# wvangansbeke/LaneDetection_End2End

Hardware: AMD Instinct MI355X
Metric: images/sec fwd+bwd, 256x512 2-lane bs32 (higher is better)
Workload: dtype f32; 1 GPU; BEV ERFNet + fused WLS fit + Area loss, 2 lanes, 256x512, batch 32 per GPU, fp32, train mode (BN batch stats, Dropout2d on), fwd+bwd, optimizer excluded; global_batch=32, parallelism=dp1, grad_allreduce=none

## Files before the change

lanedetection_end2end_amd/_lib.py:

```python
import ctypes
import os
from ctypes import c_char_p, c_double, c_int, c_long, c_size_t, c_void_p

import torch

_HERE = os.path.dirname(os.path.abspath(__file__))
LIB_PATH = os.path.join(_HERE, "liblanefit_hip.so")
_lib = None


class LaneFitLibraryError(RuntimeError):
    pass


def _declare(lib):
    P, I, L, D = c_void_p, c_int, c_long, c_double
    sig = {
        "lf_abi_version": (c_int, []),
        "lf_last_error": (c_char_p, []),
        "lf_wls_workspace_bytes": (c_size_t, [I, I, I]),
        "lf_wls_fwd": (I, [P, P, L, I, I, I, I, I, I, D, D, I, I, P, P, P, P, P, P]),
        "lf_wls_bwd": (I, [P, P, L, I, I, I, I, I, I, D, I, P, P, P, P, P]),
        "lf_gels_workspace_bytes": (c_size_t, [I, I]),
        "lf_gels_fwd": (I, [P, P, I, L, I, P, P, P, P, P]),
# ... 51 lines not shown
        "lf_adam_step": (I, [P, P, I, ctypes.c_float, ctypes.c_float, ctypes.c_float, ctypes.c_float, ctypes.c_float,
                             I, ctypes.c_float, P]),
        "lf_sgd_step": (I, [P, P, I, ctypes.c_float, ctypes.c_float, ctypes.c_float, ctypes.c_float, P]),
        "lf_rmsprop_step": (I, [P, P, I, ctypes.c_float, ctypes.c_float, ctypes.c_float, ctypes.c_float, ctypes.c_float,
                                ctypes.c_float, P]),
        "lf_conv1d_scratch_floats": (L, [I, I, I, I]),
        "lf_conv1d_fwd": (I, [P, P, P, P, I, I, I, I, I, I, I, P, P]),
        "lf_conv1d_bwd_data": (I, [P, P, P, P, I, I, I, I, I, I, P, P]),
        "lf_conv1d_bwd_weight": (I, [P, P, P, P, I, I, I, I, I, I, P, P]),
        "lf_erfnet_num_layers": (I, [P]),
        "lf_erfnet_range_workspace_bytes": (c_size_t, [P, I, I]),
        "lf_erfnet_layer_io": (I, [P, I, P]),
        "lf_erfnet_forward_range": (I, [P, I, I, I, P, P, P, P, P, I, P, P, c_size_t, P]),
        "lf_erfnet_backward_range": (I, [P, I, I, I, P, P, P, P, P, I, P, P, c_size_t, P]),
        "lf_linear_fwd": (I, [P, P, P, P, I, I, I, I, P]),
        "lf_linear_bwd": (I, [P, P, P, P, P, P, P, I, I, I, I, P]),
        "lf_seg_maps": (I, [P, P, P, I, I, I, I, I, I, P]),
        "lf_erfnet_set_precision": (I, [P, I]),
        "lf_erfnet_profile": (I, [P, I]),
        "lf_erfnet_profile_read": (I, [P, P, c_char_p]),
        "lf_erfnet_infer_workspace_bytes": (c_size_t, [P, I]),
        "lf_erfnet_infer_encoder_offset": (L, [P]),
        "lf_erfnet_infer": (I, [P, P, P, P, P, I, P, P, c_size_t, P]),
        "lf_erfnet_infer_range_workspace_bytes": (c_size_t, [P, I, I, I]),
        "lf_erfnet_infer_range": (I, [P, I, I, I, P, P, P, P, P, P, c_size_t, P]),
        "lf_convchain_infer_workspace_bytes": (c_size_t, [P, I]),
        "lf_convchain_infer": (I, [P, P, P, P, P, ctypes.c_float, P, P, c_size_t, P]),
        "lf_head_fit": (I, [P, I, P, P, P, L, I, I, I, I, I, I, D, D, I, I, P, P, P, P, P, P]),
        "lf_lane_infer_workspace_bytes": (c_size_t, [P, I, I, I]),
        "lf_lane_infer": (I, [P, P, P, P, P, P, L, I, I, D, D, I, I, P, P, P, P, c_size_t, P]),
        "lf_theta_grid": (I, [P, L, P, P, I, I, I, P, P]),
        "lf_theta_grid_bwd_workspace_bytes": (c_size_t, [I]),
        "lf_theta_grid_bwd": (I, [P, L, P, P, P, I, I, I, P, P, P]),
        "lf_wls_fwd_theta": (I, [P, P, L, P, P, I, I, I, I, I, I, D, D, I, I, P, P, P, P, P, P]),
        "lf_wls_bwd_theta_workspace_bytes": (c_size_t, [I, I]),
        "lf_wls_bwd_theta": (I, [P, P, L, P, P, I, I, I, I, I, I, D, I, P, P, P, P, P, P, P]),
        "lf_wls_bwd_grid": (I, [P, P, L, I, I, I, I, I, I, D, I, P, P, P, P, P]),
        "lf_lane_eval": (I, [P, P, P, P, P, P, L, P, I, I, I, I, I, D, D, P, P, P, P, P, P]),
        "lf_lane_decode_bev": (I, [P, I, P, P, P, P, L, P, P, I, D, P, P, I, I, I, I, I, I, I, I, I, I, P, P, P]),
        "lf_step_loss_workspace_bytes": (c_size_t, []),
        "lf_step_loss": (I, [I, I, I, I, I, I, I, P, L, I, P, P, L, I, P, P, P, P, P, P, P, I, D, D, P, P, P, P, P, P]),
        "lf_step_loss_bwd": (I, [P, I, L, L, P, P, P]),
        "lf_seg_step_workspace_bytes": (c_size_t, [I, I, I, I, I, I]),
        "lf_seg_step": (I, [P, P, P, P, L, P, I, I, I, I, I, I, I, D, D, I, P, P, P, P, P, P, P, P]),
        "lf_seg_step_bwd": (I, [P, L, P, P]),
        "lf_label_batch_bp": (I, [P, P, P, P, P, P, P, L, P, P, I, I, P, P, P, P, P, P, P, P, P]),
        "lf_label_batch_bev": (I, [P, P, P, P, P, L, P, P, I, P, P, P, P, P, P, P]),
        "lf_grad_norm_workspace_bytes": (c_size_t, [I]),
        "lf_grad_sumsq": (I, [P, P, I, I, P, P]),
        "lf_grad_norm_finish": (I, [P, I, ctypes.c_float, ctypes.c_float, P, P]),
        "lf_grad_scale_inplace": (I, [P, P, I, ctypes.c_float, P, P]),
        "lf_adam_step_clipped": (I, [P, P, I, ctypes.c_float, ctypes.c_float, ctypes.c_float, ctypes.c_float, ctypes.c_float,
                                     I, ctypes.c_float, P, P]),
        "lf_sgd_step_clipped": (I, [P, P, I, ctypes.c_float, ctypes.c_float, ctypes.c_float, ctypes.c_float, P, P]),
        "lf_rmsprop_step_clipped": (I, [P, P, I, ctypes.c_float, ctypes.c_float, ctypes.c_float, ctypes.c_float, ctypes.c_float,
                                        ctypes.c_float, P, P]),
        "lf_head_fit_seg": (I, [P, I, P, P, P, L, P, I, I, I, I, I, I, I, D, D, I, P, P, P, P, P, P]),
        "lf_lane_infer_seg_workspace_bytes": (c_size_t, [P, I, I, I]),
        "lf_lane_infer_seg": (I, [P, P, P, P, P, P, L, P, I, I, I, D, D, I, P, P, P, P, c_size_t, P]),
        "lf_stem_bwd_data": (I, [P, P, P, I, I, I, I, I, P, P]),
        "lf_erfnet_backward_input": (I, [P, P, P, P, P, P, P, I, I, P, P, c_size_t, P]),
        "lf_erfnet_infer_fold": (I, [P, P, P, P, P, c_size_t, P]),
        "lf_lane_infer_folded": (I, [P, P, P, P, P, P, L, I, I, D, D, I, I, P, P, P, P, c_size_t, I, P]),
        "lf_lane_infer_seg_folded": (I, [P, P, P, P, P, P, L, P, I, I, I, D, D, I, P, P, P, P, c_size_t, I, P]),
    }
    dbg = {
        "lf_debug_set_split_any_size": (None, [I]),
        "lf_debug_set_bf16_lds": (None, [I]),
        "lf_debug_set_bf16_no_partial_fast": (None, [I]),
        "lf_debug_stride2_epi": (I, [I, I, P, P, P, P, I, P, P, P, P, I, I, I, I, I, P, P]),
        "lf_debug_stride2_wgrad_scratch_floats": (L, [I, I, I, I, I, I, I]),
        "lf_debug_stride2_wgrad": (I, [I, I, P, P, P, P, I, I, I, I, I, P, P]),
        "lf_debug_stem_wgrad_scratch_floats": (L, [I, I, I, I]),
        "lf_debug_stem_wgrad": (I, [I, P, P, P, P, I, I, I, I, P, P]),
        "lf_debug_head_wgrad_scratch_floats": (L, [I, I, I, I]),
        "lf_debug_head_wgrad": (I, [I, P, P, P, P, I, I, I, I, P, P]),
        "lf_debug_set_ops_precision": (None, [I]),
        "lf_debug_conv1d_fwd_phases": (I, [P, P, P, P, I, I, I, I, I, I, P, P, P]),
        "lf_debug_conv1d_wgrad_phases": (I, [P, P, I, I, I, I, I, I, P, P, P]),
        "lf_debug_conv1d_fwd_pro": (I, [P, P, P, P, P, P, I, I, I, I, I, I, P, P]),
        "lf_debug_set_wgrad_ro": (None, [I, I, I]),
        "lf_debug_set_fp32_stream": (None, [I, I]),
        "lf_debug_set_bwd16_fused": (None, [I]),
        "lf_debug_set_fwd_pair": (None, [I, I]),
        "lf_debug_conv1d_fwd_pair": (I, [P, P, P, P, P, P, P, P, P, P, I, I, I, I, I, P, P]),
        "lf_debug_conv1d_bwd_pair_scratch_floats": (L, [I, I, I, I]),
        "lf_debug_conv1d_bwd_pair": (I, [P, P, P, I, P, P, P, P, P, P, P, P, P, P, I, I, I, I, I, I, P, P]),
        "lf_debug_conv1d_bwd_data_epi3": (I, [P, P, P, P, P, P, P, I, I, I, I, I, I, P, P]),
        "lf_debug_conv1d_epi": (I, [P, P, P, P, I, I, P, P, P, P, P, P, I, I, I, I, I, I, P, P]),
        "lf_debug_conv1d_wgrad_pro": (I, [P, P, P, P, P, P, I, I, I, I, I, I, P, P]),
        "lf_debug_bias_residual_launches": (L, []),
        "lf_debug_partial_fast_launches": (L, []),
        "lf_debug_bf16_ring_launches": (L, []),
        "lf_debug_set_bf16_max_workgroups": (None, [I]),
        "lf_debug_set_thin": (None, [I, I]),
        "lf_debug_thin_launches": (L, []),
        "lf_debug_fold_pack_launches": (L, []),
        "lf_debug_bn_finalize_fwd": (I, [P, I, I, I, I, I, I, L] * 2 + [I, D, P, P, P, P, ctypes.c_float, ctypes.c_float, I, P, P, P, P, P]),
        "lf_debug_bn_bwd_finalize": (I, [P, I, I, I, I, I, I, L] * 2 + [I, D, P, P, P, P, P, P, I, P]),
        "lf_debug_bn_act": (I, [P, P, P, P, P, P, L, I, L, I, P]),
        "lf_debug_bn_bwd_reduce": (I, [P, P, P, P, P, P, P, I, L, I, L, I, P]),
        "lf_debug_bn_bwd_apply": (I, [P, P, P, P, P, P, P, P, P, P, P, L, I, L, I, P]),
        "lf_debug_pool_concat_fwd": (I, [P, I, I, I, I, P, I, I, P, I, I, P]),
        "lf_debug_pool_affine_fwd": (I, [P, I, I, I, I, P, I, I, P, P, I, P]),
        "lf_debug_pool_bwd": (I, [P, P, I, I, I, I, I, I, P, I, P]),
        "lf_debug_stem_fwd": (I, [P, I, I, I, I, P, P, P, P, P, P, I, I, P]),
        "lf_debug_head_fwd": (I, [P, P, P, P, I, I, I, I, I, P]),
        "lf_debug_head_bwd_data": (I, [P, P, P, I, I, I, I, I, P]),
        "lf_debug_convchain_offset": (L, [P, I, I]),
    }
    for table in (sig, dbg):
        for name, (res, args) in table.items():
            fn = getattr(lib, name)
            fn.restype = res
            fn.argtypes = args
    return sig


def exported_symbols():
    return list(_declare(load()).keys()) + list(_extra_symbols)


_extra_symbols = ["lf_debug_set_thin", "lf_debug_thin_launches", "lf_debug_fold_pack_launches"]


def load():
    global _lib
    if _lib is None:
        if not os.path.exists(LIB_PATH):
            raise LaneFitLibraryError(
                "%s not found: build it with `python -m lanedetection_end2end_amd.build` "
                "(there is no fallback path)" % LIB_PATH)
        lib = ctypes.CDLL(LIB_PATH)
        _declare(lib)
        _lib = lib
    return _lib


def check(rc, what):
    if rc != 0:
        raise LaneFitLibraryError("%s failed: %s" % (what, load().lf_last_error().decode()))


def ptr(t, rows=False):
    if t is None:
        return None
    if not t.is_cuda:
        raise LaneFitLibraryError("lanefit ops need tensors on the MI355X (got a %s tensor); "
                                  "there is no CPU path" % t.device)
    if rows:
        assert t.dim() == 2 and t.stride(1) == 1, "internal: tensor rows must be contiguous"
    else:
        assert t.is_contiguous(), "internal: tensor must be contiguous"
    return c_void_p(t.data_ptr())


def stream():
    return c_void_p(torch.cuda.current_stream().cuda_stream)


class DeferredRead:

    def __init__(self, t):
        if t.is_cuda:
            self.host = torch.empty(t.shape, dtype=t.dtype, pin_memory=True)
            self.host.copy_(t, non_blocking=True)
            self.event = torch.cuda.Event()
            self.event.record()
        else:
            self.host = t.detach().clone()
            self.event = None

    def ready(self):
        return self.event is None or self.event.query()

    def get(self):
        if self.event is not None:
            self.event.synchronize()
        return self.host
```

lanedetection_end2end_amd/csrc/lf_bwd16.hip:

```cpp
#include "lf_conv_dev.h"
#include "lf_conv_epi.h"

namespace {

constexpr int B16_TILE = 1024;
template <int EPIC> struct B16Cfg {
    static constexpr bool ST_ADD = (EPIC & LF_EPI_ADD) != 0;
    static constexpr bool AUX_IS_X = (EPIC & LF_EPI_MASKBN) != 0;
    static constexpr bool ST_AUX = (EPIC & LF_EPI_STATS_XHAT) != 0 && !AUX_IS_X;
    static constexpr bool SUMS = (EPIC & LF_EPI_STATS_XHAT) != 0;
    static constexpr int T_ADD = 6, T_AUX = ST_AUX ? 6 + (ST_ADD ? 1 : 0) : 4;
    static constexpr int NTILE = 6 + (ST_ADD ? 1 : 0) + (ST_AUX ? 1 : 0);
    static constexpr int STAGES = NTILE == 6 ? 3 : 2;
    static constexpr int STAGE = NTILE * B16_TILE, WAVE_LDS = STAGES * STAGE;
    static_assert(WG_WAVES * WAVE_LDS + 1024 <= 80 * 1024, "two workgroups per CU");
    static_assert(WAVE_LDS >= 13 * 64 * 4, "the ring also stages the wave's weight-gradient sums");
};

typedef __attribute__((address_space(3))) float* lds_f32_p;
typedef __attribute__((address_space(3))) f32x4* lds_f32x4_p;
typedef __attribute__((address_space(3))) unsigned char* lds_u8_p;

template <bool PRO, int EPIC>
__global__ __launch_bounds__(256, 2) void tapbwd16_kernel(const LfTapGeom g, const LfWgradArgs wa, const LfTapArgs a, const long pps,
                                                          const int write_bias, const int wave_rows) {
    using Cfg = B16Cfg<EPIC>;
    constexpr int NTAPS = 3, NT = 1, epi = EPIC;
    constexpr bool S16 = false, HOISTV = true;
    const int lane = threadIdx.x & 63, wave = __builtin_amdgcn_readfirstlane((int)(threadIdx.x >> 6));
    const int pl = lane & 15, kq = lane >> 4;
    const long npix_l = (long)g.N * g.Hl * g.Wl;
    const unsigned npix = (unsigned)npix_l, bx = blockIdx.x;
    const int cob = 0;
    const long sub = (long)blockIdx.x * WG_WAVES + wave;
    const long p_begin = sub * pps;
    long p_end = p_begin + pps;
    if (p_end > npix_l) p_end = npix_l;
    const int niter = p_end > p_begin ? (int)((p_end - p_begin + 15) / 16) : 0;
    f32x4 acc[NTAPS];
#pragma unroll
    for (int t = 0; t < NTAPS; ++t) acc[t] = zero4();
    float bsum = 0.f;
    const unsigned tbytes = (unsigned)min((long)g.N * g.Hs * g.Ws * g.s_pix * 4, (long)LF_OOB);
    const i32x4s rx = make_rsrc_words(wa.x, tbytes), rg = make_rsrc_words(wa.g, tbytes),
                 radd = make_rsrc_words(a.add_src, Cfg::ST_ADD ? tbytes : 0u), raux = make_rsrc_words(a.aux, Cfg::ST_AUX ? tbytes : 0u);
    lds_u8_p const ring = (lds_u8_p)lf_tap_lds + wave * Cfg::WAVE_LDS;
    const unsigned lds0 = (unsigned)(size_t)ring;
    const int tdh0 = g.tdh[0], tdh1 = g.tdh[1], tdh2 = g.tdh[2], tdw0 = g.tdw[0], tdw1 = g.tdw[1], tdw2 = g.tdw[2];
    long p_ld = p_begin;
    int pj_, pi_, pn_;
    row1_coords(g, niter ? (unsigned)p_begin : 0u, pn_, pi_, pj_);
    int cj = pj_, ci = pi_, cn = pn_;
    const int px = lane >> 2, chunk = lane & 3;
    int slot_ld = 0;
    auto issue = [&]() __attribute__((always_inline)) {
        const bool ok = p_ld < p_end;
        const int j = pj_ + px;
        const unsigned dst = lds0 + (unsigned)(slot_ld * Cfg::STAGE);
#pragma unroll
        for (int t = 0; t < NTAPS; ++t) {
            const int dh = t == 0 ? tdh0 : t == 1 ? tdh1 : tdh2, dw = t == 0 ? tdw0 : t == 1 ? tdw1 : tdw2;
            const int sy = pi_ + dh, sx = j + dw;
            const bool in = ok && sy >= 0 && sy < g.Hs && sx >= 0 && sx < g.Ws;
            const unsigned o = in ? (unsigned)((((pn_ * g.Hs + sy) * g.Ws + sx) * g.s_pix + g.s_choff + chunk * 4) * 4) : LF_OOB;
            lds_dma16(rg, dst + (unsigned)(t * B16_TILE), o, 0u);
            lds_dma16(rx, dst + (unsigned)((3 + t) * B16_TILE), o, 0u);
        }
        if constexpr (Cfg::ST_ADD || Cfg::ST_AUX) {
            const unsigned o = ok ? (unsigned)((((pn_ * g.Hs + pi_) * g.Ws + j) * g.s_pix + g.s_choff + chunk * 4) * 4) : LF_OOB;
            if constexpr (Cfg::ST_ADD) lds_dma16(radd, dst + (unsigned)(Cfg::T_ADD * B16_TILE), o, 0u);
            if constexpr (Cfg::ST_AUX) lds_dma16(raux, dst + (unsigned)(Cfg::T_AUX * B16_TILE), o, 0u);
        }
        slot_ld = slot_ld == Cfg::STAGES - 1 ? 0 : slot_ld + 1;
        p_ld += 16;
        pj_ += 16;
        if (pj_ >= g.Wl) { pj_ = 0; if (++pi_ >= g.Hl) { pi_ = 0; ++pn_; } }
    };
    f32x4 w3[NTAPS];
    {
        const __amdgpu_buffer_rsrc_t rwl = make_rsrc(a.wp, (unsigned)(NTAPS * 16 * 16 * 4));
#pragma unroll
        for (int t = 0; t < NTAPS; ++t) w3[t] = ldb4(rwl, (unsigned)(kq * 16 + pl) * 16u, (unsigned)(t * 16 * 64));
    }
    float psc = 1.f, psh = 0.f;
    if constexpr (PRO) { psc = wa.pro_sc[pl]; psh = wa.pro_sh[pl]; }
#undef LF_EPI_ACC
#define LF_EPI_ACC(n, m) dacc
#undef LF_EPI_LDADD
#define LF_EPI_LDADD(o) (*(lds_f32x4_p)(epi_lane + Cfg::T_ADD * B16_TILE))
#undef LF_EPI_LDMSK
#define LF_EPI_LDMSK(o) (*(lds_f32x4_p)(epi_lane + 4 * B16_TILE))
#undef LF_EPI_LDAUX
#define LF_EPI_LDAUX(o) (*(lds_f32x4_p)(epi_lane + Cfg::T_AUX * B16_TILE))
#undef LF_EPI_HOIST_ALL
#define LF_EPI_HOIST_ALL true
#undef LF_EPI_ROW1
#define LF_EPI_ROW1 true
    LF_EPI_HEAD
    (void)r_add; (void)r_msk; (void)r_aux;
    if constexpr ((EPIC & LF_EPI_MASKBN) != 0) asm volatile("" ::"v"(hv[0][0]), "v"(hv[0][1]) : "memory");
    asm volatile("s_waitcnt vmcnt(0)" ::"v"(w3[0]), "v"(w3[1]), "v"(w3[2]), "v"(psc), "v"(psh) : "memory");
#pragma unroll
    for (int q = 0; q < Cfg::STAGES - 1; ++q) issue();
    int slot_c = 0;
    f32x4 row1 = zero4(), row2 = zero4();
    for (int it = 0; it < niter; ++it) {
        asm volatile("s_waitcnt lgkmcnt(0)" ::: "memory");
        issue();
        wait_vm_lgkm0<Cfg::NTILE * (Cfg::STAGES - 1)>();
        lds_u8_p const st = ring + slot_c * Cfg::STAGE;
        slot_c = slot_c == Cfg::STAGES - 1 ? 0 : slot_c + 1;
        lds_u8_p const epi_lane = st + pl * 64 + kq * 16;
        {
            lds_f32_p const frag = (lds_f32_p)(st + kq * 64 + pl * 4);
            float gv[4], xv[NTAPS][4];
#pragma unroll
            for (int u = 0; u < 4; ++u) {
                gv[u] = frag[(1 * B16_TILE + u * 256) / 4];
#pragma unroll
                for (int t = 0; t < NTAPS; ++t) xv[t][u] = frag[((3 + t) * B16_TILE + u * 256) / 4];
            }
            if constexpr (PRO) {
#pragma unroll
                for (int t = 0; t < NTAPS; ++t) {
                    const int dh = t == 0 ? tdh0 : t == 1 ? tdh1 : tdh2, dw = t == 0 ? tdw0 : t == 1 ? tdw1 : tdw2;
                    const bool rowok = (unsigned)(ci + dh) < (unsigned)g.Hs;
                    const int c0 = cj + dw;
                    const bool edge = c0 < 0 || c0 + 15 >= g.Ws;
#pragma unroll
                    for (int u = 0; u < 4; ++u) {
                        float v = fmaxf(xv[t][u] * psc + psh, 0.f);
                        if (edge) v = (unsigned)(c0 + 4 * u + kq) < (unsigned)g.Ws ? v : 0.f;
                        xv[t][u] = rowok ? v : 0.f;
                    }
                }
            }
#pragma unroll
            for (int u = 0; u < 4; ++u) {
#pragma unroll
                for (int t = 0; t < NTAPS; ++t) acc[t] = __builtin_amdgcn_mfma_f32_16x16x4f32(xv[t][u], gv[u], acc[t], 0, 0, 0);
                bsum += gv[u];
            }
        }
        f32x4 dacc;
#pragma unroll
        for (int t = 0; t < NTAPS; ++t) {
            const f32x4 x3 = *(lds_f32x4_p)(epi_lane + t * B16_TILE);
            f32x4 part;
#pragma unroll
            for (int s4 = 0; s4 < 4; ++s4) part = __builtin_amdgcn_mfma_f32_16x16x4f32(w3[t][s4], x3[s4], s4 ? part : zero4(), 0, 0, 0);
            dacc = t ? dacc + part : part;
        }
        {
            const int pn[1] = {cn}, pi[1] = {ci}, pj[1] = {cj + pl};
            const bool pv[1] = {true};
            LF_EPI_TILE(0)
        }
        if constexpr (Cfg::SUMS) {
            if (wave_rows && ((it & 3) == 3 || it == niter - 1)) {
                f32x4 q1, q2;
                q1.x = sum16(s1[0].x); q1.y = sum16(s1[0].y); q1.z = sum16(s1[0].z); q1.w = sum16(s1[0].w);
                q2.x = sum16(s2[0].x); q2.y = sum16(s2[0].y); q2.z = sum16(s2[0].z); q2.w = sum16(s2[0].w);
                const bool first = (it & 15) < 4;
                row1 = first ? q1 : row1 + q1;
                row2 = first ? q2 : row2 + q2;
                s1[0] = zero4(); s2[0] = zero4();
                if (((it & 15) == 15 || it == niter - 1) && pl == 0) {
                    const long row = (p_begin >> 8) + (it >> 4);
#pragma unroll
                    for (int e = 0; e < 4; ++e) {
                        a.stats[(long)(kq * 4 + e) * a.stats_ld + row] = row1[e];
                        a.stats[(long)(g.Cd + kq * 4 + e) * a.stats_ld + row] = row2[e];
                    }
                }
            }
        }
        cj += 16;
        if (cj >= g.Wl) { cj = 0; if (++ci >= g.Hl) { ci = 0; ++cn; } }
    }
    asm volatile("s_waitcnt vmcnt(0)" ::: "memory");
    if (!wave_rows) {
        const int pn[1] = {0};
        LF_EPI_TAIL
    }
#undef LF_EPI_ACC
#define LF_EPI_ACC(n, m) acc[n][m]
#undef LF_EPI_LDADD
#define LF_EPI_LDADD(o) epi_ld<S16>(r_add, o)
#undef LF_EPI_LDMSK
#define LF_EPI_LDMSK(o) epi_ld<S16>(r_msk, o)
#undef LF_EPI_LDAUX
#define LF_EPI_LDAUX(o) epi_ld<S16>(r_aux, o)
#undef LF_EPI_HOIST_ALL
#define LF_EPI_HOIST_ALL false
#undef LF_EPI_ROW1
#define LF_EPI_ROW1 false
    float* const red = reinterpret_cast<float*>(lf_tap_lds);
    constexpr int RW = Cfg::WAVE_LDS / 4;
    if (wave > 0) {
#pragma unroll
        for (int t = 0; t < NTAPS; ++t)
#pragma unroll
            for (int e = 0; e < 4; ++e) red[wave * RW + (t * 4 + e) * 64 + lane] = acc[t][e];
    }
    red[wave * RW + 12 * 64 + lane] = bsum;
    __syncthreads();
    if (wave == 0) {
#pragma unroll
        for (int t = 0; t < NTAPS; ++t) {
            float* out = wa.partial + ((long)blockIdx.x * NTAPS + t) * g.Cs * g.Cd;
#pragma unroll
            for (int e = 0; e < 4; ++e) {
                float v = acc[t][e];
#pragma unroll
                for (int w = 1; w < WG_WAVES; ++w) v += red[w * RW + (t * 4 + e) * 64 + lane];
                out[(long)(4 * kq + e) * g.Cd + pl] = v;
            }
        }
        if (write_bias && wa.bias_partial) {
            float v = red[12 * 64 + lane] + red[RW + 12 * 64 + lane] + red[2 * RW + 12 * 64 + lane] + red[3 * RW + 12 * 64 + lane];
            v += __shfl_xor(v, 16, 64);
            v += __shfl_xor(v, 32, 64);
            if (kq == 0) wa.bias_partial[(long)blockIdx.x * g.Cd + pl] = v;
        }
    }
}

std::atomic<int> g_bwd16_mode{1};
enum { B16_MASK = 1, B16_MASKBN = 2, B16_EPI3 = 4, B16_ADD = 8 };
constexpr int g_bwd16_routed = B16_MASK | B16_MASKBN | B16_EPI3 | B16_ADD;

int form_of(int pro, int epi) {
    if (pro == LF_PRO_NONE && epi == LF_EPI_MASK) return B16_MASK;
    if (pro == LF_PRO_BNRELU && epi == (LF_EPI_MASKBN | LF_EPI_STATS_XHAT)) return B16_MASKBN;
    if (pro == LF_PRO_NONE && epi == (LF_EPI_ADD | LF_EPI_MASK | LF_EPI_STATS_XHAT)) return B16_EPI3;
    if (pro == LF_PRO_NONE && epi == LF_EPI_ADD) return B16_ADD;
    return 0;
}
template <typename F>
auto with_form(int form, F&& f) {
    switch (form) {
        case B16_MASK: return f(tapbwd16_kernel<false, LF_EPI_MASK>, B16Cfg<LF_EPI_MASK>{});
        case B16_MASKBN: return f(tapbwd16_kernel<true, LF_EPI_MASKBN | LF_EPI_STATS_XHAT>, B16Cfg<LF_EPI_MASKBN | LF_EPI_STATS_XHAT>{});
        case B16_EPI3: return f(tapbwd16_kernel<false, LF_EPI_ADD | LF_EPI_MASK | LF_EPI_STATS_XHAT>, B16Cfg<LF_EPI_ADD | LF_EPI_MASK | LF_EPI_STATS_XHAT>{});
        default: return f(tapbwd16_kernel<false, LF_EPI_ADD>, B16Cfg<LF_EPI_ADD>{});
    }
}

}

void lf_tapbwd16_set(int mode) { g_bwd16_mode = mode < 0 ? 0 : mode; }
bool lf_tapbwd16_routed(int pro, int epi) {
    const int mode = g_bwd16_mode.load();
    const int forms = mode == 0 ? 0 : mode == 1 ? g_bwd16_routed : mode >> 1;
    return (forms & form_of(pro, epi)) != 0;
}

bool lf_tapbwd16_ok(const LfTapGeom& gf, const LfTapGeom& gd, const LfWgradArgs& w, const LfTapArgs& a, int pro, int epi) {
    const int form = form_of(pro, epi);
    if (!form) return false;
    const LfTapGeom& g = gf;
    bool same = gf.N == gd.N && gf.Hl == gd.Hl && gf.Wl == gd.Wl && gf.Hs == gd.Hs && gf.Ws == gd.Ws && gf.s_pix == gd.s_pix && gf.s_choff == gd.s_choff &&
                gf.ssh == gd.ssh && gf.ssw == gd.ssw && gf.Hd == gd.Hd && gf.Wd == gd.Wd && gf.d_pix == gd.d_pix && gf.d_choff == gd.d_choff &&
                gf.dsh == gd.dsh && gf.dsw == gd.dsw && gf.dah == gd.dah && gf.daw == gd.daw && gf.Cs == gd.Cs && gf.Cd == gd.Cd && gf.ntaps == gd.ntaps;
    for (int t = 0; same && t < 3 && t < gf.ntaps; ++t) same = gf.tdh[t] == gd.tdh[t] && gf.tdw[t] == gd.tdw[t];
    if (!same) return false;
    if (!(g.Cs == 16 && g.Cd == 16 && g.ntaps == 3 && g.ssh == 1 && g.ssw == 1 && g.dsh == 1 && g.dsw == 1 && g.dah == 0 && g.daw == 0 &&
          g.Hs == g.Hl && g.Hd == g.Hl && g.Ws == g.Wl && g.Wd == g.Wl && g.s_pix == 16 && g.d_pix == 16 && g.s_choff == 0 && g.d_choff == 0 &&
          g.tdh[1] == 0 && g.tdw[1] == 0))
        return false;
    if (g.N < 1 || g.Hl < 1 || g.Wl < 64 || g.Wl % 64 != 0) return false;
    const long npix = (long)g.N * g.Hl * g.Wl;
    if (npix * 64 >= (long)LF_OOB) return false;
    if (lf_tapgemm_bf16_lds() < 3) return false;
    if (w.s16 || a.s16 || a.wp16 || w.dbg || a.dbg || a.bias || a.dm) return false;
    if (!w.x || !w.g || !w.partial || !w.bias_partial || !a.wp || !a.dst || a.src != w.g) return false;
    if (a.dst == w.x || a.dst == w.g) return false;
    if ((pro == LF_PRO_BNRELU) != (w.pro_sc != nullptr) || (w.pro_sc != nullptr) != (w.pro_sh != nullptr)) return false;
    if ((epi & LF_EPI_MASK) && a.mask_src != w.x) return false;
    if ((epi & LF_EPI_MASKBN) && (a.aux != w.x || !a.msc || !a.msh)) return false;
    if ((epi & LF_EPI_ADD) && (!a.add_src || a.add_src == a.dst)) return false;
    if ((epi & LF_EPI_STATS_XHAT) && (!a.aux || a.aux == a.dst || !a.stats)) return false;
    if (epi & LF_EPI_STATS_XHAT) {
        const long pps = lf_tapwgrad_wave_pixels(g);
        if (!(pps % 256 == 0 || pps == 64 || (lf_tapwgrad_splits(g) == 1 && npix <= 256))) return false;
        if (a.stats_ld < lf_tapgemm_stat_rows(g)) return false;
    }
    return with_form(form, [&](auto kern, auto cfg) {
        return allow_big_lds(reinterpret_cast<const void*>(kern), 128 * 1024);
    });
}

int lf_tapbwd16_launch(const LfTapGeom& gf, const LfTapGeom& gd, const LfWgradArgs& w, const LfTapArgs& a, int pro, int epi, hipStream_t st) {
    LF_REQUIRE(lf_tapbwd16_ok(gf, gd, w, a, pro, epi), "tapbwd16: the fused kernel does not take this launch (pro %d, epi %d, %d x %d x %d x %d -> %d)",
               pro, epi, gf.N, gf.Hl, gf.Wl, gf.Cs, gf.Cd);
    const long pps = lf_tapwgrad_wave_pixels(gf);
    const int gx = lf_tapwgrad_splits(gf);
    const int wave_rows = pps % 256 == 0;
    with_form(form_of(pro, epi), [&](auto kern, auto cfg) {
        hipLaunchKernelGGL(kern, dim3(gx), dim3(256), (size_t)WG_WAVES * decltype(cfg)::WAVE_LDS, st, gf, w, a, pps, 1, wave_rows);
        return true;
    });
    LF_CHECK_LAUNCH("tapbwd16");
    return 0;
}
```

lanedetection_end2end_amd/csrc/lf_conv.h:

```cpp
#pragma once
#include <atomic>

#include "lf_common.h"

#define LF_MAX_TAPS 9
struct TapIdx { int v[LF_MAX_TAPS]; };

struct LfTapGeom {
    int N, Hl, Wl;
    int Hs, Ws, s_pix, s_choff;
    int ssh, ssw;
    int Hd, Wd, d_pix, d_choff;
    int dsh, dsw, dah, daw;
    int Cs, Cd;
    int ntaps;
    int tdh[LF_MAX_TAPS], tdw[LF_MAX_TAPS];
};

enum { LF_PRO_NONE = 0, LF_PRO_BNRELU = 1 };
enum {
    LF_EPI_RELU = 1,
    LF_EPI_MASK = 2,
    LF_EPI_ADD = 4,
    LF_EPI_STATS_SQ = 8,
    LF_EPI_MASKBN = 16,
    LF_EPI_STATS_XHAT = 32,
    LF_EPI_BIAS = 64
};

struct LfTapArgs {
    const float* src;
    const float* wp;
    int s16;
    const void* wp16;
    int split;
    const void* wp48;
    const float* bias;
    float* dst;
    const float* pro_sc;
    const float* pro_sh;
    const float* mask_src;
    const float* add_src;
    const float* aux;
    const float* msc;
    const float* msh;
    const float* asc;
    const float* ash;
    const float* dm;
    float* stats;
    int stats_ld;
    unsigned long long* dbg;
    int thin;
};

void lf_tapgemm_set_split_any_size(int v);
void lf_tapgemm_set_fp32_stream(int mode, int max_workgroups);
void lf_tapgemm_set_thin(int mode, int nt);
long lf_tapgemm_thin_launches();
int lf_tapgemm_stat_rows(const LfTapGeom& g);
int lf_tapgemm_stat_rows_for(const LfTapGeom& g, const LfTapArgs& a);
int lf_tapgemm_launch(const LfTapGeom& g, const LfTapArgs& a, int pro, int epi, hipStream_t st);
int lf_tapgemm_launch_unordered(const LfTapGeom& g, const LfTapArgs& a, int pro, int epi, hipStream_t st);
bool lf_tapgemm_split_ok(const LfTapGeom& g);
long lf_tapgemm_bias_residual_launches();
extern std::atomic<long> g_bres_launches;

bool lf_tappair_ok(const LfTapGeom& ga, const LfTapGeom& gb, const LfTapArgs& aa, const LfTapArgs& ab, int pro, int epi_a, int epi_b);
int lf_tappair_launch(const LfTapGeom& ga, const LfTapGeom& gb, const LfTapArgs& aa, const LfTapArgs& ab, int pro, hipStream_t st);
void lf_tappair_set(int mode, int max_workgroups);
bool lf_tappair_routed(int C, int pro);

int lf_tapgemm_bf16_route(const LfTapGeom& g, const LfTapArgs& a, int pro, int epi, int epis, long npix, int nt, dim3 grid, hipStream_t st);
void lf_tapgemm_set_bf16_lds(int v);
int lf_tapgemm_bf16_lds();
void lf_tapgemm_set_bf16_no_partial_fast(int v);
long lf_tapgemm_partial_fast_launches();
long lf_tapgemm_bf16_ring_launches();
void lf_tapgemm_set_bf16_max_workgroups(int v);

struct LfWgradArgs {
    const float* x;
    const float* g;
    const float* pro_sc;
    const float* pro_sh;
    int s16;
    int split;
    float* partial;
    float* bias_partial;
    unsigned long long* dbg = nullptr;
};
int lf_tapwgrad_splits(const LfTapGeom& g);
int lf_tapwgrad_splits_bound(const LfTapGeom& g, int s16);
long lf_tapwgrad_wave_pixels(const LfTapGeom& g);
int lf_tapwgrad_splits_for(const LfTapGeom& g, const LfWgradArgs& a, int pro);
int lf_tapwgrad_launch(const LfTapGeom& g, const LfWgradArgs& a, int pro, hipStream_t st);

bool lf_tapbwd16_ok(const LfTapGeom& gf, const LfTapGeom& gd, const LfWgradArgs& w, const LfTapArgs& a, int pro, int epi);
int lf_tapbwd16_launch(const LfTapGeom& gf, const LfTapGeom& gd, const LfWgradArgs& w, const LfTapArgs& a, int pro, int epi, hipStream_t st);
void lf_tapbwd16_set(int mode);
bool lf_tapbwd16_routed(int pro, int epi);

bool lf_tapwgrad_ro_ok(const LfTapGeom& g, int s16);
int lf_tapwgrad_ro_rows_bound(const LfTapGeom& g);
int lf_tapwgrad_ro_rows(const LfTapGeom& g);
int lf_tapwgrad_ro_launch(const LfTapGeom& g, const LfWgradArgs& a, int pro, hipStream_t st);
void lf_tapwgrad_ro_set(int mode, int cap64, int cap128);

int lf_wgrad_reduce_launch(const float* partial, int splits, int ntaps, int Cs, int Cd, float* grad, long sk, long sn,
                           const int* tapidx_host, const float* bias_rows, int n_bias_rows, float* bias_grad,
                           int bias_accumulate, hipStream_t st);
#define LF_REDUCE_BATCH 32
struct LfReduceJob {
    const float* partial; float* grad; const float* bias_rows; float* bias_grad;
    long sk, sn;
    int splits, ntaps, Cs, Cd, n_bias_rows;
    int tapidx[LF_MAX_TAPS];
};
int lf_wgrad_reduce_batch_launch(const LfReduceJob* jobs_host, int njobs, hipStream_t st);
int lf_rows_reduce_launch(const float* rows, int nrows, int C, float* dst, int accumulate, hipStream_t st);

struct LfPackEntry {
    long src_off;
    long dst_off;
    int Kc, Nc, ntaps;
    long sk, sn;
    int tapidx[LF_MAX_TAPS];
    int param;
    long dst16_off;
};
int lf_pack_weights_launch(const LfPackEntry* entries_dev, int nentries, const float* const* params_dev, float* arena,
                           hipStream_t st);
long lf_pack_bf16_elems(int Kc, int Nc, int ntaps);
int lf_pack_weights_split_launch(const LfPackEntry* entries_dev, int nentries, const float* const* params_dev, void* arena48,
                                 hipStream_t st);

struct LfFoldEntry {
    LfPackEntry pk;
    int ch_off, C;
    const float* gamma;
    const float* beta;
    const float* mean;
    const float* var;
    const float* bias;
    long out_off;
};
int lf_fold_pack_launch(const LfFoldEntry* entries_dev, int nentries, const float* const* params_dev, float eps, float* vec, float* arena,
                        void* arena16, void* arena48, hipStream_t st);
long lf_fold_pack_launches();
int lf_pack_weights_bf16_launch(const LfPackEntry* entries_dev, int nentries, const float* const* params_dev, void* arena16,
                                hipStream_t st);
```

lanedetection_end2end_amd/csrc/lf_debug.h:

```cpp
#pragma once
#ifdef __cplusplus
extern "C" {
#endif
void lf_debug_set_split_any_size(int v);
void lf_debug_set_bf16_lds(int v);
void lf_debug_set_bf16_no_partial_fast(int v);
long lf_debug_partial_fast_launches(void);
long lf_debug_bf16_ring_launches(void);
void lf_debug_set_bf16_max_workgroups(int v);
void lf_debug_set_ops_precision(int mode);
int lf_debug_conv1d_fwd_phases(const float* x, const float* w, const float* bias, float* y, int N, int H, int W, int C,
                               int axis, int dilation, float* scratch, unsigned long long* dbg, void* stream);
int lf_debug_conv1d_fwd_pro(const float* x, const float* w, const float* bias, const float* sc, const float* sh, float* y, int N, int H,
                            int W, int C, int axis, int dilation, float* scratch, void* stream);
void lf_debug_set_wgrad_ro(int mode, int cap64, int cap128);
void lf_debug_set_fp32_stream(int mode, int max_workgroups);
void lf_debug_set_fwd_pair(int mode, int max_workgroups);
int lf_debug_conv1d_fwd_pair(const float* x, const float* wa, const float* ba, const float* wb, const float* bb, const float* sc,
                             const float* sh, float* t, float* y, float* stats, int N, int H, int W, int C, int dilation, float* scratch,
                             void* stream);
void lf_debug_set_bwd16_fused(int mode);
long lf_debug_conv1d_bwd_pair_scratch_floats(int N, int H, int W, int C);
int lf_debug_conv1d_bwd_pair(const float* x, const float* gy, const float* w, int epi, const float* add_src, const float* aux,
                             const float* msc, const float* msh, const float* pro_sc, const float* pro_sh, float* gx, float* gw, float* gb,
                             float* stats, int N, int H, int W, int C, int axis, int dilation, float* scratch, void* stream);
int lf_debug_conv1d_wgrad_pro(const float* x, const float* gy, const float* sc, const float* sh, float* gw, float* gb, int N, int H, int W,
                              int C, int axis, int dilation, float* scratch, void* stream);
int lf_debug_conv1d_bwd_data_epi3(const float* gy, const float* w, const float* mask_src, const float* add_src, const float* aux,
                                  float* gx, float* stats, int N, int H, int W, int C, int axis, int dilation, float* scratch, void* stream);
int lf_debug_conv1d_epi(const float* src, const float* w, const float* bias, float* dst, int transposed, int epi, const float* mask_src,
                        const float* add_src, const float* aux, const float* msc, const float* msh, float* stats, int N, int H, int W, int C,
                        int axis, int dilation, float* scratch, void* stream);
int lf_debug_stride2_epi(int kind, int phase, const float* src, const float* w, const float* bias, float* dst, int epi, const float* mask_src,
                         const float* add_src, const float* aux, float* stats, int N, int H, int W, int Cin, int Cout, float* scratch,
                         void* stream);
long lf_debug_stride2_wgrad_scratch_floats(int kind, int reduce, int N, int H, int W, int Cin, int Cout);
int lf_debug_stride2_wgrad(int kind, int reduce, const float* x, const float* g, float* gw, float* gb, int N, int H, int W, int Cin,
                           int Cout, float* scratch, void* stream);
long lf_debug_stem_wgrad_scratch_floats(int N, int Cin, int H, int W);
int lf_debug_stem_wgrad(int reduce, const float* img, const float* gcat, float* gw, float* gb, int N, int Cin, int H, int W, float* scratch,
                        void* stream);
long lf_debug_head_wgrad_scratch_floats(int N, int h, int w, int K);
int lf_debug_head_wgrad(int reduce, const float* x, const float* gout, float* gw, float* gb, int N, int h, int w, int K, float* scratch,
                        void* stream);
int lf_debug_bn_finalize_fwd(const float* rows0, int nrows0, int ld0, int C0, int ch_off0, int tile_pix0, int seg_rows0, long seg_pix0,
                             const float* rows1, int nrows1, int ld1, int C1, int ch_off1, int tile_pix1, int seg_rows1, long seg_pix1,
                             int C, double count, const float* gamma, const float* beta, float* running_mean, float* running_var,
                             float momentum, float eps, int training, float* scale, float* shift, float* asc, float* ash, void* stream);
int lf_debug_bn_bwd_finalize(const float* rows0, int nrows0, int ld0, int C0, int ch_off0, int tile_pix0, int seg_rows0, long seg_pix0,
                             const float* rows1, int nrows1, int ld1, int C1, int ch_off1, int tile_pix1, int seg_rows1, long seg_pix1,
                             int C, double count, const float* asc, const float* ash, float* c1, float* c2, float* ggamma, float* gbeta,
                             int training, void* stream);
int lf_debug_bn_act(const float* x, const float* sc, const float* sh, const float* dm, const float* res, float* y, long npix, int C,
                    long pix_per_image, int s16, void* stream);
int lf_debug_bn_bwd_reduce(const float* g, const float* y, const float* t, const float* asc, const float* ash, const float* dm, float* rows,
                           int ld, long npix, int C, long pix_per_image, int s16, void* stream);
int lf_debug_bn_bwd_apply(const float* g, const float* y, const float* t, const float* asc, const float* ash, const float* gamma,
                          const float* c1, const float* c2, const float* dm, float* g_t, float* g_z, long npix, int C, long pix_per_image,
                          int s16, void* stream);
int lf_debug_pool_concat_fwd(const float* x, int N, int H, int W, int Cin, float* cat, int cat_pix, int choff, float* rows, int ld, int s16,
                             void* stream);
int lf_debug_pool_affine_fwd(const float* x, int N, int H, int W, int Cin, float* cat, int cat_pix, int choff, const float* sc, const float* sh,
                             int s16, void* stream);
int lf_debug_pool_bwd(const float* x, const float* gcat, int N, int H, int W, int Cin, int cat_pix, int choff, float* gx, int s16, void* stream);
int lf_debug_stem_fwd(const float* img, int N, int Cin, int H, int W, const float* w, const float* b, const float* sc, const float* sh, float* cat,
                      float* rows, int ld, int s16, void* stream);
int lf_debug_head_fwd(const float* x, const float* w, const float* b, float* out, int N, int h, int w_, int K, int s16, void* stream);
int lf_debug_head_bwd_data(const float* gout, const float* w, float* gx, int N, int h, int w_, int K, int s16, void* stream);
long lf_debug_bias_residual_launches(void);
void lf_debug_set_thin(int mode, int nt);
long lf_debug_thin_launches(void);
long lf_debug_fold_pack_launches(void);
int lf_debug_conv1d_wgrad_phases(const float* x, const float* gy, int N, int H, int W, int C, int axis, int dilation,
                                 float* scratch, unsigned long long* dbg, void* stream);
struct lf_convchain_plan;
long lf_debug_convchain_offset(const struct lf_convchain_plan* plan, int block, int which);
#ifdef __cplusplus
}
#endif
```

lanedetection_end2end_amd/csrc/lf_eltwise.h:

```cpp
#pragma once
#include "lf_common.h"

struct LfStatPart {
    const float* rows; int nrows; int C; int ch_off; int ld;
    int tile_pix = 0; int seg_rows = 0; long seg_pix = 0;
};
inline int lf_stat_ld(int nrows) { return (nrows + 3) / 4 * 4; }
inline LfStatPart lf_stat_part_tiles(const float* rows, int nrows, int ld, int C, int ch_off, int seg_rows, long seg_pix, int tile_pix = 256) {
    LfStatPart p = {rows, nrows, C, ch_off, ld};
    p.tile_pix = tile_pix; p.seg_rows = seg_rows; p.seg_pix = seg_pix;
    return p;
}

int lf_bn_finalize_fwd(const LfStatPart* parts, int nparts, int C, double count, const float* gamma, const float* beta,
                       float* running_mean, float* running_var, float momentum, float eps, int training,
                       float* scale, float* shift, float* asc , float* ash , hipStream_t st);
int lf_bn_act(const float* x, const float* sc, const float* sh, const float* dm, const float* res, float* y,
              long npix, int C, long pix_per_image, int s16, hipStream_t st);
int lf_bn_bwd_reduce_rows(long npix);
int lf_bn_bwd_reduce(const float* g, const float* y, const float* t, const float* asc, const float* ash, const float* dm,
                     float* rows, int ld, long npix, int C, long pix_per_image, int s16, hipStream_t st);
int lf_bn_bwd_finalize(const LfStatPart* parts, int nparts, int C, double count, const float* asc, const float* ash, float* c1,
                       float* c2, float* ggamma, float* gbeta, int training, hipStream_t st);
int lf_bn_bwd_apply(const float* g, const float* y, const float* t, const float* asc, const float* ash, const float* gamma,
                    const float* c1, const float* c2, const float* dm, float* g_t, float* g_z, long npix, int C,
                    long pix_per_image, int s16, hipStream_t st);

int lf_pool_rows(long npix_out);
int lf_pool_concat_fwd(const float* x, int N, int H, int W, int Cin, float* cat, int cat_pix, int choff, float* rows, int ld,
                       int s16, hipStream_t st);
int lf_pool_affine_fwd(const float* x, int N, int H, int W, int Cin, float* cat, int cat_pix, int choff, const float* sc,
                       const float* sh, int s16, hipStream_t st);
int lf_pool_bwd(const float* x, const float* gcat, int N, int H, int W, int Cin, int cat_pix, int choff, float* gx,
                int s16, hipStream_t st);

int lf_stem_rows(int N, int H, int W);
int lf_stem_fwd(const float* img, int N, int Cin, int H, int W, const float* w, const float* b, float* cat, float* rows, int ld,
                int s16, hipStream_t st);
int lf_stem_fwd_infer(const float* img, int N, int Cin, int H, int W, const float* w, const float* b, const float* sc, const float* sh,
                      float* cat, int s16, hipStream_t st);
int lf_stem_wgrad_rows(int N, int H, int W);
int lf_stem_wgrad(const float* img, const float* gcat, int N, int Cin, int H, int W, float* wrows, float* brows,
                  int s16, hipStream_t st);

int lf_head_fwd(const float* x, const float* w, const float* b, float* out, int N, int h, int w_, int K, int s16,
                hipStream_t st);
int lf_head_bwd_data(const float* gout, const float* w, float* gx, int N, int h, int w_, int K, int s16, hipStream_t st);
int lf_head_wgrad_rows(int N, int h, int w_);
int lf_head_wgrad(const float* x, const float* gout, float* wrows, float* brows, int N, int h, int w_, int K,
                  int s16, hipStream_t st);
```

lanedetection_end2end_amd/csrc/lf_eltwise.hip:

```cpp
#include "lf_eltwise.h"
#include "lf_types.h"
#include "lf_plan.h"

typedef float f32x4 __attribute__((ext_vector_type(4)));

namespace {

__device__ __forceinline__ f32x4 ld4(const float* p) { return *reinterpret_cast<const f32x4*>(p); }
__device__ __forceinline__ void st4(float* p, f32x4 v) { *reinterpret_cast<f32x4*>(p) = v; }
__device__ __forceinline__ f32x4 z4() { f32x4 z = {0.f, 0.f, 0.f, 0.f}; return z; }
__device__ __forceinline__ f32x4 relu4(f32x4 v) {
    v.x = fmaxf(v.x, 0.f); v.y = fmaxf(v.y, 0.f); v.z = fmaxf(v.z, 0.f); v.w = fmaxf(v.w, 0.f); return v;
}
__device__ __forceinline__ f32x4 pos4(f32x4 v, f32x4 m) {
    v.x = m.x > 0.f ? v.x : 0.f; v.y = m.y > 0.f ? v.y : 0.f; v.z = m.z > 0.f ? v.z : 0.f; v.w = m.w > 0.f ? v.w : 0.f; return v;
}

template <int NQ>
__device__ __forceinline__ void block_reduce_quads(f32x4 (&a1)[NQ], f32x4 (&a2)[NQ], int U, float (*sm)[8 * NQ]) {
    const int tid = threadIdx.x;
#pragma unroll
    for (int q = 0; q < NQ; ++q) {
        sm[tid][8 * q + 0] = a1[q].x; sm[tid][8 * q + 1] = a1[q].y; sm[tid][8 * q + 2] = a1[q].z; sm[tid][8 * q + 3] = a1[q].w;
        sm[tid][8 * q + 4] = a2[q].x; sm[tid][8 * q + 5] = a2[q].y; sm[tid][8 * q + 6] = a2[q].z; sm[tid][8 * q + 7] = a2[q].w;
// ... 49 lines not shown
                    s1 += v ? av : 0.0;
                    s2 += v ? (double)b[u][e] + av * av * inv : 0.0;
                }
        }
    }
    constexpr int NWV = FIN_THREADS / 64;
    __shared__ double sm[NWV][2];
#pragma unroll
    for (int o = 32; o > 0; o >>= 1) { s1 += __shfl_xor(s1, o, 64); s2 += __shfl_xor(s2, o, 64); }
    const int w = threadIdx.x >> 6;
    if ((threadIdx.x & 63) == 0) { sm[w][0] = s1; sm[w][1] = s2; }
    __syncthreads();
    double t1 = 0.0, t2 = 0.0;
#pragma unroll
    for (int k = 0; k < NWV; ++k) { t1 += sm[k][0]; t2 += sm[k][1]; }
    s1 = t1; s2 = t2;
}

__global__ __launch_bounds__(FIN_THREADS) void bn_finalize_fwd_kernel(StatParts sp, int C, double count,
                                                            const float* __restrict__ gamma, const float* __restrict__ beta,
                                                            float* __restrict__ rmean, float* __restrict__ rvar,
                                                            float momentum, float eps, int training,
                                                            float* __restrict__ scale, float* __restrict__ shift,
                                                            float* __restrict__ asc, float* __restrict__ ash) {
    const int c = blockIdx.x;
    double s1 = 0.0, s2 = 0.0;
    if (training) stat_channel_sums(sp, c, s1, s2);
    if (threadIdx.x == 0 && c < C) {
        double mean, var;
        if (training) {
            mean = s1 / count;
            var = s2 / count - mean * mean;
            if (var < 0.0) var = 0.0;
            rmean[c] = (float)((1.0 - momentum) * (double)rmean[c] + momentum * mean);
            const double unb = count > 1.0 ? var * count / (count - 1.0) : var;
            rvar[c] = (float)((1.0 - momentum) * (double)rvar[c] + momentum * unb);
        } else {
            mean = (double)rmean[c];
            var = (double)rvar[c];
        }
        const double rstd = 1.0 / sqrt(var + (double)eps);
        const double sc = (double)gamma[c] * rstd;
        scale[c] = (float)sc;
        shift[c] = (float)((double)beta[c] - mean * sc);
        asc[c] = (float)rstd;
        ash[c] = (float)(-mean * rstd);
    }
}

template <typename T, int NQ>
__global__ __launch_bounds__(256) void bn_act_kernel(const T* __restrict__ x, const float* __restrict__ sc,
                                                    const float* __restrict__ sh, const float* __restrict__ dm,
                                                    const T* __restrict__ res, T* __restrict__ y, long units,
                                                    int U, long pix_per_image) {
    constexpr int V = 4 * NQ;
    const int C = U * V;
    for (long u = (long)blockIdx.x * 256 + threadIdx.x; u < units; u += (long)gridDim.x * 256) {
        const int c = (int)(u % U) * V;
        f32x4 v[NQ];
        lf_ldq<T, NQ>(x + u * V, v);
#pragma unroll
        for (int q = 0; q < NQ; ++q) v[q] = v[q] * ld4(sc + c + 4 * q) + ld4(sh + c + 4 * q);
        if (dm) {
            const float* d = dm + ((u / U) / pix_per_image) * C + c;
#pragma unroll
            for (int q = 0; q < NQ; ++q) v[q] *= ld4(d + 4 * q);
        }
        if (res) {
            f32x4 r[NQ];
            lf_ldq<T, NQ>(res + u * V, r);
#pragma unroll
            for (int q = 0; q < NQ; ++q) v[q] += r[q];
        }
#pragma unroll
        for (int q = 0; q < NQ; ++q) v[q] = relu4(v[q]);
        lf_stq<T, NQ>(y + u * V, v);
    }
}

template <typename T, int NQ>
__global__ __launch_bounds__(256) void bn_bwd_reduce_kernel(const T* __restrict__ g, const T* __restrict__ y,
                                                           const T* __restrict__ t, const float* __restrict__ asc,
                                                           const float* __restrict__ ash, const float* __restrict__ dm,
                                                           float* __restrict__ rows, int ld, long npix, int U, long pix_per_image) {
    constexpr int V = 4 * NQ;
    const int C = U * V, ppi = 256 / U;
    const int cq = threadIdx.x % U, pr = threadIdx.x / U;
    const int c = cq * V;
    (void)asc; (void)ash;
    f32x4 a1[NQ], a2[NQ];
#pragma unroll
    for (int q = 0; q < NQ; ++q) { a1[q] = z4(); a2[q] = z4(); }
    const long per_block = ((npix + gridDim.x - 1) / gridDim.x + ppi - 1) / ppi * ppi;
    const long p0 = (long)blockIdx.x * per_block;
    long p1 = p0 + per_block;
    if (p1 > npix) p1 = npix;
    for (long p = p0 + pr; p < p1; p += ppi) {
        const long off = p * C + c;
        f32x4 gm[NQ], tv[NQ];
        lf_ldq<T, NQ>(g + off, gm);
        lf_ldq<T, NQ>(t + off, tv);
        if (y) {
            f32x4 yv[NQ];
            lf_ldq<T, NQ>(y + off, yv);
#pragma unroll
            for (int q = 0; q < NQ; ++q) gm[q] = pos4(gm[q], yv[q]);
        }
        if (dm) {
            const float* d = dm + (p / pix_per_image) * C + c;
#pragma unroll
            for (int q = 0; q < NQ; ++q) gm[q] *= ld4(d + 4 * q);
        }
#pragma unroll
        for (int q = 0; q < NQ; ++q) {
            a1[q] += gm[q];
            a2[q] += gm[q] * tv[q];
        }
    }
    __shared__ float sm[256][8 * NQ];
    block_reduce_quads<NQ>(a1, a2, U, sm);
    if (threadIdx.x < U) {
#pragma unroll
        for (int q = 0; q < NQ; ++q)
#pragma unroll
            for (int e = 0; e < 4; ++e) {
                rows[(long)(c + 4 * q + e) * ld + blockIdx.x] = a1[q][e];
                rows[((long)C + c + 4 * q + e) * ld + blockIdx.x] = a2[q][e];
            }
    }
}

__global__ __launch_bounds__(FIN_THREADS) void bn_bwd_finalize_kernel(StatParts sp, int C, double mean_scale, const float* __restrict__ asc,
                                                            const float* __restrict__ ash, float* __restrict__ c1,
                                                            float* __restrict__ c2, float* __restrict__ ggamma,
                                                            float* __restrict__ gbeta) {
    const int c = blockIdx.x;
    double t1, t2;
    stat_channel_sums(sp, c, t1, t2);
    if (threadIdx.x == 0 && c < C) {
        const double rstd = (double)asc[c], mr = (double)ash[c];
        t2 = rstd * t2 + mr * t1;
        c1[c] = (float)(t1 * mean_scale);
        c2[c] = (float)(t2 * mean_scale);
        ggamma[c] = (float)t2;
        gbeta[c] = (float)t1;
    }
}

template <typename T, int NQ>
__global__ __launch_bounds__(256) void bn_bwd_apply_kernel(const T* __restrict__ g, const T* __restrict__ y,
                                                          const T* __restrict__ t, const float* __restrict__ asc,
                                                          const float* __restrict__ ash, const float* __restrict__ gamma,
                                                          const float* __restrict__ c1, const float* __restrict__ c2,
                                                          const float* __restrict__ dm, T* __restrict__ g_t,
                                                          T* __restrict__ g_z, long units, int U, long pix_per_image) {
    constexpr int V = 4 * NQ;
    const int C = U * V;
    for (long u = (long)blockIdx.x * 256 + threadIdx.x; u < units; u += (long)gridDim.x * 256) {
        const int c = (int)(u % U) * V;
        f32x4 gm[NQ], tv[NQ];
        lf_ldq<T, NQ>(g + u * V, gm);
        lf_ldq<T, NQ>(t + u * V, tv);
        if (y) {
            f32x4 yv[NQ];
            lf_ldq<T, NQ>(y + u * V, yv);
#pragma unroll
            for (int q = 0; q < NQ; ++q) gm[q] = pos4(gm[q], yv[q]);
        }
        if (g_z) lf_stq<T, NQ>(g_z + u * V, gm);
        if (dm) {
            const float* d = dm + ((u / U) / pix_per_image) * C + c;
#pragma unroll
            for (int q = 0; q < NQ; ++q) gm[q] *= ld4(d + 4 * q);
        }
        f32x4 o[NQ];
#pragma unroll
        for (int q = 0; q < NQ; ++q) {
            const f32x4 rstd = ld4(asc + c + 4 * q);
            const f32x4 xh = tv[q] * rstd + ld4(ash + c + 4 * q);
            o[q] = ld4(gamma + c + 4 * q) * rstd * (gm[q] - ld4(c1 + c + 4 * q) - xh * ld4(c2 + c + 4 * q));
        }
        lf_stq<T, NQ>(g_t + u * V, o);
    }
}

template <typename T, int NQ>
__global__ __launch_bounds__(256) void pool_concat_fwd_kernel(const T* __restrict__ x, int N, int H, int W, int U,
                                                             T* __restrict__ cat, int cat_pix, int choff,
                                                             float* __restrict__ rows, int ld) {
    constexpr int V = 4 * NQ;
// ... 141 lines not shown
                                                           T* __restrict__ gx, int N, int h, int wd, int K) {
    __shared__ float sw[16 * HEAD_MAXK * 4];
    for (int i = threadIdx.x; i < 16 * K * 4; i += 256) sw[i] = w[i];
    __syncthreads();
    const long npix = (long)N * h * wd;
    for (long p = (long)blockIdx.x * 256 + threadIdx.x; p < npix; p += (long)gridDim.x * 256) {
        const int j = (int)(p % wd);
        const long r = p / wd;
        const int i = (int)(r % h), n = (int)(r / h);
        float acc[16];
#pragma unroll
        for (int ci = 0; ci < 16; ++ci) acc[ci] = 0.f;
        for (int k = 0; k < K; ++k) {
            const float* gp = gout + (((long)n * K + k) * (2 * h) + 2 * i) * (2 * wd) + 2 * j;
            const float2 g0 = *reinterpret_cast<const float2*>(gp);
            const float2 g1 = *reinterpret_cast<const float2*>(gp + 2 * wd);
#pragma unroll
            for (int ci = 0; ci < 16; ++ci) {
                const float* wk = sw + (ci * K + k) * 4;
                acc[ci] = fmaf(g0.x, wk[0], fmaf(g0.y, wk[1], fmaf(g1.x, wk[2], fmaf(g1.y, wk[3], acc[ci]))));
            }
        }
#pragma unroll
        for (int q = 0; q < 4; ++q) {
            f32x4 v = {acc[q * 4], acc[q * 4 + 1], acc[q * 4 + 2], acc[q * 4 + 3]};
            lf_stv(gx + p * 16 + q * 4, v);
        }
    }
}

constexpr int LF_STREAM_BLOCKS = 16384;
inline int grid_for(long units, int cap) {
    long g = (units + 255) / 256;
    if (g > cap) g = cap;
    if (g < 1) g = 1;
    return (int)g;
}
inline bool quad_ok(int C) { return C % 4 == 0 && 256 % (C / 4) == 0; }
inline bool oct_ok(int s16, int C) { return s16 && C % 8 == 0 && 256 % (C / 8) == 0; }
template <typename T> inline const T* as(const float* p) { return reinterpret_cast<const T*>(p); }
template <typename T> inline T* as(float* p) { return reinterpret_cast<T*>(p); }
#define LF_BY_STORAGE(s16, CALL_BF16, CALL_F32) do { if (s16) { CALL_BF16; } else { CALL_F32; } } while (0)
#define LF_BY_STORAGE3(s16, oct, CALL_BF16X8, CALL_BF16, CALL_F32) do { if (oct) { CALL_BF16X8; } else if (s16) { CALL_BF16; } else { CALL_F32; } } while (0)

}

int lf_bn_finalize_fwd(const LfStatPart* parts, int nparts, int C, double count, const float* gamma, const float* beta,
                       float* running_mean, float* running_var, float momentum, float eps, int training, float* scale,
                       float* shift, float* asc, float* ash, hipStream_t st) {
    LF_REQUIRE(nparts >= 0 && nparts <= 2, "bn_finalize: at most 2 partial sources");
    StatParts sp;
    sp.n = nparts;
    for (int i = 0; i < nparts; ++i) sp.p[i] = parts[i];
    for (int i = 0; i < nparts; ++i) LF_REQUIRE(parts[i].C % 4 == 0 && parts[i].ch_off % 4 == 0, "bn_finalize: channel ranges must be multiples of 4");
    for (int i = 0; i < nparts; ++i)
        LF_REQUIRE(parts[i].tile_pix == 0 || (parts[i].seg_rows > 0 && parts[i].seg_pix > 0 && parts[i].nrows % parts[i].seg_rows == 0),
                   "bn_finalize: centred rows need the launch geometry (seg_rows, seg_pix)");
    for (int i = 0; i < nparts; ++i)
        LF_REQUIRE(parts[i].ld >= parts[i].nrows && parts[i].ld % 4 == 0 && ((size_t)parts[i].rows & 15) == 0,
                   "bn_finalize: channel-major rows need a 16-byte aligned base and a leading dimension >= nrows, multiple of 4 (ld=%d nrows=%d)", parts[i].ld, parts[i].nrows);
    hipLaunchKernelGGL(bn_finalize_fwd_kernel, dim3(C), dim3(FIN_THREADS), 0, st, sp, C, count, gamma, beta,
                       running_mean, running_var, momentum, eps, training, scale, shift, asc, ash);
    LF_CHECK_LAUNCH("bn_finalize_fwd");
    return 0;
}

int lf_bn_act(const float* x, const float* sc, const float* sh, const float* dm, const float* res, float* y, long npix,
              int C, long pix_per_image, int s16, hipStream_t st) {
    LF_REQUIRE(C % 4 == 0, "bn_act: C %% 4");
    const bool oct = oct_ok(s16, C);
    const int V = oct ? 8 : 4;
    const long units = npix * (C / V);
    const dim3 grid(grid_for(units, LF_STREAM_BLOCKS));
    LF_BY_STORAGE3(s16, oct,
        hipLaunchKernelGGL((bn_act_kernel<lf_bf16, 2>), grid, dim3(256), 0, st, as<lf_bf16>(x), sc, sh, dm, as<lf_bf16>(res), as<lf_bf16>(y), units, C / V, pix_per_image),
        hipLaunchKernelGGL((bn_act_kernel<lf_bf16, 1>), grid, dim3(256), 0, st, as<lf_bf16>(x), sc, sh, dm, as<lf_bf16>(res), as<lf_bf16>(y), units, C / V, pix_per_image),
        hipLaunchKernelGGL((bn_act_kernel<float, 1>), grid, dim3(256), 0, st, x, sc, sh, dm, res, y, units, C / V, pix_per_image));
    LF_CHECK_LAUNCH("bn_act");
    return 0;
}

int lf_bn_bwd_reduce_rows(long npix) { return grid_for(npix * 4, 1024); }

int lf_bn_bwd_reduce(const float* g, const float* y, const float* t, const float* asc, const float* ash, const float* dm,
                     float* rows, int ld, long npix, int C, long pix_per_image, int s16, hipStream_t st) {
    LF_REQUIRE(quad_ok(C), "bn_bwd_reduce: unsupported channel count %d", C);
    const dim3 grid(lf_bn_bwd_reduce_rows(npix));
    const bool oct = oct_ok(s16, C);
    const int V = oct ? 8 : 4;
    LF_BY_STORAGE3(s16, oct,
        hipLaunchKernelGGL((bn_bwd_reduce_kernel<lf_bf16, 2>), grid, dim3(256), 0, st, as<lf_bf16>(g), as<lf_bf16>(y), as<lf_bf16>(t), asc, ash, dm, rows, ld, npix, C / V, pix_per_image),
        hipLaunchKernelGGL((bn_bwd_reduce_kernel<lf_bf16, 1>), grid, dim3(256), 0, st, as<lf_bf16>(g), as<lf_bf16>(y), as<lf_bf16>(t), asc, ash, dm, rows, ld, npix, C / V, pix_per_image),
        hipLaunchKernelGGL((bn_bwd_reduce_kernel<float, 1>), grid, dim3(256), 0, st, g, y, t, asc, ash, dm, rows, ld, npix, C / V, pix_per_image));
    LF_CHECK_LAUNCH("bn_bwd_reduce");
    return 0;
}

int lf_bn_bwd_finalize(const LfStatPart* parts, int nparts, int C, double count, const float* asc, const float* ash, float* c1,
                       float* c2, float* ggamma, float* gbeta, int training, hipStream_t st) {
    LF_REQUIRE(nparts >= 1 && nparts <= 2, "bn_bwd_finalize: 1..2 partial sources");
    StatParts sp;
    sp.n = nparts;
    for (int i = 0; i < nparts; ++i) sp.p[i] = parts[i];
    for (int i = 0; i < nparts; ++i) LF_REQUIRE(parts[i].C % 4 == 0 && parts[i].ch_off % 4 == 0, "bn_bwd_finalize: channel ranges must be multiples of 4");
    for (int i = 0; i < nparts; ++i)
        LF_REQUIRE(parts[i].ld >= parts[i].nrows && parts[i].ld % 4 == 0 && ((size_t)parts[i].rows & 15) == 0,
                   "bn_bwd_finalize: channel-major rows need a 16-byte aligned base and a leading dimension >= nrows, multiple of 4 (ld=%d nrows=%d)", parts[i].ld, parts[i].nrows);
    hipLaunchKernelGGL(bn_bwd_finalize_kernel, dim3(C), dim3(FIN_THREADS), 0, st, sp, C, training ? 1.0 / count : 0.0, asc, ash,
                       c1, c2, ggamma, gbeta);
    LF_CHECK_LAUNCH("bn_bwd_finalize");
    return 0;
}

int lf_bn_bwd_apply(const float* g, const float* y, const float* t, const float* asc, const float* ash, const float* gamma,
                    const float* c1, const float* c2, const float* dm, float* g_t, float* g_z, long npix, int C,
                    long pix_per_image, int s16, hipStream_t st) {
    LF_REQUIRE(C % 4 == 0, "bn_bwd_apply: C %% 4");
    const bool oct = oct_ok(s16, C);
    const int V = oct ? 8 : 4;
    const long units = npix * (C / V);
    const dim3 grid(grid_for(units, LF_STREAM_BLOCKS));
    LF_BY_STORAGE3(s16, oct,
        hipLaunchKernelGGL((bn_bwd_apply_kernel<lf_bf16, 2>), grid, dim3(256), 0, st, as<lf_bf16>(g), as<lf_bf16>(y), as<lf_bf16>(t), asc, ash, gamma, c1, c2, dm, as<lf_bf16>(g_t), as<lf_bf16>(g_z), units, C / V, pix_per_image),
        hipLaunchKernelGGL((bn_bwd_apply_kernel<lf_bf16, 1>), grid, dim3(256), 0, st, as<lf_bf16>(g), as<lf_bf16>(y), as<lf_bf16>(t), asc, ash, gamma, c1, c2, dm, as<lf_bf16>(g_t), as<lf_bf16>(g_z), units, C / V, pix_per_image),
        hipLaunchKernelGGL((bn_bwd_apply_kernel<float, 1>), grid, dim3(256), 0, st, g, y, t, asc, ash, gamma, c1, c2, dm, g_t, g_z, units, C / V, pix_per_image));
    LF_CHECK_LAUNCH("bn_bwd_apply");
    return 0;
}

int lf_pool_rows(long npix_out) { return grid_for(npix_out * 4, 1024); }

int lf_pool_concat_fwd(const float* x, int N, int H, int W, int Cin, float* cat, int cat_pix, int choff, float* rows, int ld,
                       int s16, hipStream_t st) {
    LF_REQUIRE(quad_ok(Cin) && H % 2 == 0 && W % 2 == 0, "pool_concat: unsupported shape");
    const long npo = (long)N * (H / 2) * (W / 2);
    const dim3 grid(lf_pool_rows(npo));
    const bool oct = oct_ok(s16, Cin) && cat_pix % 8 == 0 && choff % 8 == 0;
    const int V = oct ? 8 : 4;
    LF_BY_STORAGE3(s16, oct,
        hipLaunchKernelGGL((pool_concat_fwd_kernel<lf_bf16, 2>), grid, dim3(256), 0, st, as<lf_bf16>(x), N, H, W, Cin / V, as<lf_bf16>(cat), cat_pix, choff, rows, ld),
        hipLaunchKernelGGL((pool_concat_fwd_kernel<lf_bf16, 1>), grid, dim3(256), 0, st, as<lf_bf16>(x), N, H, W, Cin / V, as<lf_bf16>(cat), cat_pix, choff, rows, ld),
        hipLaunchKernelGGL((pool_concat_fwd_kernel<float, 1>), grid, dim3(256), 0, st, x, N, H, W, Cin / V, cat, cat_pix, choff, rows, ld));
    LF_CHECK_LAUNCH("pool_concat_fwd");
    return 0;
}

int lf_pool_affine_fwd(const float* x, int N, int H, int W, int Cin, float* cat, int cat_pix, int choff, const float* sc,
                       const float* sh, int s16, hipStream_t st) {
    LF_REQUIRE(quad_ok(Cin) && H % 2 == 0 && W % 2 == 0 && sc && sh, "pool_affine: unsupported shape");
    const long npo = (long)N * (H / 2) * (W / 2);
    const bool oct = oct_ok(s16, Cin) && cat_pix % 8 == 0 && choff % 8 == 0;
    const int V = oct ? 8 : 4;
    const long units = npo * (Cin / V);
    const dim3 grid(grid_for(units, LF_STREAM_BLOCKS));
    LF_BY_STORAGE3(s16, oct,
        hipLaunchKernelGGL((pool_affine_fwd_kernel<lf_bf16, 2>), grid, dim3(256), 0, st, as<lf_bf16>(x), N, H, W, Cin / V, as<lf_bf16>(cat), cat_pix, choff, sc, sh, units),
        hipLaunchKernelGGL((pool_affine_fwd_kernel<lf_bf16, 1>), grid, dim3(256), 0, st, as<lf_bf16>(x), N, H, W, Cin / V, as<lf_bf16>(cat), cat_pix, choff, sc, sh, units),
        hipLaunchKernelGGL((pool_affine_fwd_kernel<float, 1>), grid, dim3(256), 0, st, x, N, H, W, Cin / V, cat, cat_pix, choff, sc, sh, units));
    LF_CHECK_LAUNCH("pool_affine_fwd");
    return 0;
}

int lf_pool_bwd(const float* x, const float* gcat, int N, int H, int W, int Cin, int cat_pix, int choff, float* gx,
                int s16, hipStream_t st) {
    const bool oct = oct_ok(s16, Cin) && cat_pix % 8 == 0 && choff % 8 == 0;
    const int V = oct ? 8 : 4;
    const long units = (long)N * (H / 2) * (W / 2) * (Cin / V);
    const dim3 grid(grid_for(units, 4096));
    LF_BY_STORAGE3(s16, oct,
        hipLaunchKernelGGL((pool_bwd_kernel<lf_bf16, 2>), grid, dim3(256), 0, st, as<lf_bf16>(x), as<lf_bf16>(gcat), N, H, W, Cin / V, cat_pix, choff, as<lf_bf16>(gx)),
        hipLaunchKernelGGL((pool_bwd_kernel<lf_bf16, 1>), grid, dim3(256), 0, st, as<lf_bf16>(x), as<lf_bf16>(gcat), N, H, W, Cin / V, cat_pix, choff, as<lf_bf16>(gx)),
        hipLaunchKernelGGL((pool_bwd_kernel<float, 1>), grid, dim3(256), 0, st, x, gcat, N, H, W, Cin / V, cat_pix, choff, gx));
    LF_CHECK_LAUNCH("pool_bwd");
    return 0;
}

int lf_head_fwd(const float* x, const float* w, const float* b, float* out, int N, int h, int w_, int K, int s16,
                hipStream_t st) {
    LF_REQUIRE(K >= 1 && K <= HEAD_MAXK, "head: out_channels %d not in 1..%d", K, HEAD_MAXK);
    const dim3 grid(grid_for((long)N * h * w_, 4096));
    LF_BY_STORAGE(s16,
        hipLaunchKernelGGL(head_fwd_kernel<lf_bf16>, grid, dim3(256), 0, st, as<lf_bf16>(x), w, b, out, N, h, w_, K),
        hipLaunchKernelGGL(head_fwd_kernel<float>, grid, dim3(256), 0, st, x, w, b, out, N, h, w_, K));
    LF_CHECK_LAUNCH("head_fwd");
    return 0;
}

int lf_head_bwd_data(const float* gout, const float* w, float* gx, int N, int h, int w_, int K, int s16, hipStream_t st) {
    LF_REQUIRE(K >= 1 && K <= HEAD_MAXK, "head: out_channels %d not in 1..%d", K, HEAD_MAXK);
    const dim3 grid(grid_for((long)N * h * w_, 4096));
    LF_BY_STORAGE(s16,
        hipLaunchKernelGGL(head_bwd_data_kernel<lf_bf16>, grid, dim3(256), 0, st, gout, w, as<lf_bf16>(gx), N, h, w_, K),
        hipLaunchKernelGGL(head_bwd_data_kernel<float>, grid, dim3(256), 0, st, gout, w, gx, N, h, w_, K));
    LF_CHECK_LAUNCH("head_bwd_data");
    return 0;
}

namespace {
constexpr int PW_MAXK = 8, PW_MAXC = 256;

template <typename T>
__global__ __launch_bounds__(256) void pointwise_fwd_kernel(const T* __restrict__ x, const float* __restrict__ w,
                                                           const float* __restrict__ b, float* __restrict__ y, long npix,
                                                           long pix_per_image, int C, int K) {
    __shared__ float sw[PW_MAXK * PW_MAXC];
    for (int i = threadIdx.x; i < K * C; i += 256) sw[i] = w[i];
    __syncthreads();
    for (long p = (long)blockIdx.x * 256 + threadIdx.x; p < npix; p += (long)gridDim.x * 256) {
        float acc[PW_MAXK];
// ... 129 lines not shown
```

lanedetection_end2end_amd/csrc/lf_erfnet.hip:

```cpp
#include <stdlib.h>

#include <vector>

#include "lf_conv.h"
#include "lf_eltwise.h"
#include "lf_plan.h"
#include "lf_types.h"

namespace {

constexpr float BN_EPS = 1e-3f, BN_MOM = 0.1f;
enum { K_DOWN = 0, K_NB = 1, K_UP = 2 };

struct GemmOp {
    LfTapGeom geom;
    int pack;
};
struct BNRef {
    int p_g, p_b, idx, C;
    long sc, sh, asc, ash, c1, c2;
};
struct ConvRef {
    int p_w, p_b;
    GemmOp fwd;
// ... 445 lines not shown

int bn_finalize(const Ctx& c, const BNRef& b, const LfStatPart* parts, int nparts, double count) {
    return lf_bn_finalize_fwd(parts, nparts, b.C, count, c.params[b.p_g], c.params[b.p_b], c.running[2 * b.idx],
                              c.running[2 * b.idx + 1], BN_MOM, BN_EPS, c.training, c.at(b.sc), c.at(b.sh), c.at(b.asc),
                              c.at(b.ash), c.st);
}

int encoder_layers(const lf_erfnet_plan* P) {
    int n = 0;
    for (const Layer& L : P->layers) { if (L.kind == K_UP) break; ++n; }
    return n;
}

int forward_layers(const Ctx& c, const float* img, int nlayers, int first = 0) {
    const lf_erfnet_plan* P = c.P;
    const int N = P->N;
    float* stat0 = c.at(P->off_stat0);
    float* stat1 = c.at(P->off_stat1);
    int layer_idx = 0;
    for (const Layer& L : P->layers) {
        if (layer_idx >= nlayers) break;
        if (layer_idx < first) { ++layer_idx; continue; }
        P->prof_layer = layer_idx++;
        const long npo = (long)N * L.Hout * L.Wout;
        if (L.kind == K_DOWN) {
            LfStatPart parts[2];
            int np = 0;
            if (L.x < 0) {
                const int srows = lf_stem_rows(N, L.Hin, L.Win);
                LF_TRY(lf_stem_fwd(img, N, L.Cin, L.Hin, L.Win, c.params[L.cv[0].p_w], c.params[L.cv[0].p_b], c.at(L.b[0]),
                                   c.training ? stat0 : nullptr, lf_stat_ld(srows), c.s16, c.st));
                parts[np++] = {stat0, srows, 16, 0, lf_stat_ld(srows)};
            } else {
                LfTapArgs a = lf_no_args();
                a.stats = stat0; a.stats_ld = lf_stat_ld(lf_tapgemm_stat_rows(L.cv[0].fwd.geom));
                LF_TRY(run_gemm(c, L.cv[0].fwd, c.at(L.x), c.at(L.b[0]), c.params[L.cv[0].p_b], LF_PRO_NONE,
                                c.training ? LF_EPI_STATS_SQ : 0, a));
                parts[np++] = lf_stat_part_tiles(stat0, c.last_rows, a.stats_ld, L.Cout - L.Cin, 0, c.last_rows, npo);
                const int prows = lf_pool_rows(npo);
                LF_TRY(lf_pool_concat_fwd(c.at(L.x), N, L.Hin, L.Win, L.Cin, c.at(L.b[0]), L.Cout, L.Cout - L.Cin,
                                          c.training ? stat1 : nullptr, lf_stat_ld(prows), c.s16, c.st));
                parts[np++] = {stat1, prows, L.Cin, L.Cout - L.Cin, lf_stat_ld(prows)};
            }
            LF_TRY(bn_finalize(c, L.bn[0], parts, np, (double)npo));
            LF_TRY(lf_bn_act(c.at(L.b[0]), c.at(L.bn[0].sc), c.at(L.bn[0].sh), nullptr, nullptr, c.at(L.b[1]), npo, L.Cout,
                             (long)L.Hout * L.Wout, c.s16, c.st));
        } else if (L.kind == K_NB) {
            LfTapArgs a = lf_no_args(), ap = lf_no_args();
            a.stats = stat0; a.stats_ld = lf_stat_ld(lf_tapgemm_stat_rows(L.cv[1].fwd.geom));
            LF_TRY(run_gemm_pair(c, L.cv[0], L.cv[1], c.at(L.x), c.at(L.b[0]), c.at(L.b[1]), LF_PRO_NONE, ap, a));
            LfStatPart p0 = lf_stat_part_tiles(stat0, c.last_rows, a.stats_ld, L.Cout, 0, c.last_rows, npo);
            LF_TRY(bn_finalize(c, L.bn[0], &p0, 1, (double)npo));
            ap.pro_sc = c.at(L.bn[0].sc); ap.pro_sh = c.at(L.bn[0].sh);
            a = lf_no_args();
            a.stats = stat0; a.stats_ld = lf_stat_ld(lf_tapgemm_stat_rows(L.cv[3].fwd.geom));
            LF_TRY(run_gemm_pair(c, L.cv[2], L.cv[3], c.at(L.b[1]), c.at(L.b[2]), c.at(L.b[3]), LF_PRO_BNRELU, ap, a));
            p0.nrows = p0.seg_rows = c.last_rows; p0.ld = a.stats_ld;
            LF_TRY(bn_finalize(c, L.bn[1], &p0, 1, (double)npo));
            const float* dm = (c.training && L.drop_idx >= 0 && c.dropmask) ? c.dropmask + P->drop_off[L.drop_idx] : nullptr;
            LF_TRY(lf_bn_act(c.at(L.b[3]), c.at(L.bn[1].sc), c.at(L.bn[1].sh), dm, c.at(L.x), c.at(L.b[4]), npo, L.Cout,
                             (long)L.Hout * L.Wout, c.s16, c.st));
        } else {
            LfStatPart parts[1];
            int rows = 0, rows4 = 0;
            for (int ph = 0; ph < 4; ++ph) rows4 += lf_tapgemm_stat_rows(L.cv[0].fph[ph].geom);
            for (int ph = 0; ph < 4; ++ph) {
                LfTapArgs a = lf_no_args();
                a.stats = stat0 + rows; a.stats_ld = lf_stat_ld(rows4);
                LF_TRY(run_gemm(c, L.cv[0].fph[ph], c.at(L.x), c.at(L.b[0]), c.params[L.cv[0].p_b], LF_PRO_NONE,
                                c.training ? LF_EPI_STATS_SQ : 0, a));
                rows += c.last_rows;
            }
            parts[0] = lf_stat_part_tiles(stat0, rows, lf_stat_ld(rows4), L.Cout, 0, rows / 4, npo / 4);
            LF_TRY(bn_finalize(c, L.bn[0], parts, 1, (double)npo));
            LF_TRY(lf_bn_act(c.at(L.b[0]), c.at(L.bn[0].sc), c.at(L.bn[0].sh), nullptr, nullptr, c.at(L.b[1]), npo, L.Cout,
                             (long)L.Hout * L.Wout, c.s16, c.st));
        }
    }
    return 0;
}

typedef LfBiasChain BiasChain;

struct PairDg { const GemmOp* op; float* dst; int epi; LfTapArgs extra; };

int run_wgrad(const Ctx& c, const GemmOp& op, const ConvRef& cv, const float* x, const float* g, const float* pro_sc,
              const float* pro_sh, int bias_accumulate, bool batch_off = false, BiasChain* chain = nullptr, const PairDg* pair = nullptr) {
    const lf_erfnet_plan* P = c.P;
    c.wgrad_launched = false;
    c.pair_fused = false;
    if (!c.grads[cv.p_w]) return 0;
    hipStream_t ws = c.st;
    LfWgradArgs a;
    a.x = x; a.g = g; a.pro_sc = pro_sc; a.pro_sh = pro_sh; a.s16 = c.s16;
    a.split = 0;
    const long wneed = (wneed_of(op.geom, c.s16) + 63) / 64 * 64, bneed = (bneed_of(op.geom, c.s16) + 63) / 64 * 64;
    const bool batched = !bias_accumulate && !batch_off && !c.no_batch &&
                         c.wpart_used + wneed <= P->wpart_all_floats[c.s16] && c.bpart_used + bneed <= P->bpart_all_floats[c.s16];
    const long off_bpart_all = P->off_wpart_all + P->wpart_all_floats[c.s16];
    a.partial = batched ? c.at(P->off_wpart_all + c.wpart_used) : c.at(P->off_wpart);
    a.bias_partial = c.grads[cv.p_b] ? (batched ? c.at(off_bpart_all + c.bpart_used) : c.at(P->off_bpart)) : nullptr;
    if (chain) {
        if (!batched) return lf_fail("erfnet backward: a chained weight gradient does not fit its partial-row regions");
        float* rows = lf_bias_chain_rows(*chain, c.at(off_bpart_all + c.bpart_used), op.geom.Cd);
        if (a.bias_partial) a.bias_partial = rows;
    }
    const int wpro = pro_sc ? LF_PRO_BNRELU : LF_PRO_NONE;
    if (pair && !chain && !c.s16 && (P->precision == 0 || P->precision == 3) && lf_tapbwd16_routed(wpro, pair->epi)) {
        LfTapArgs d = pair->extra;
        d.src = g; d.dst = pair->dst; d.bias = nullptr; d.wp = c.packed(pair->op->pack); d.s16 = 0;
        if (lf_tapbwd16_ok(op.geom, pair->op->geom, a, d, wpro, pair->epi)) {
            c.last_rows = lf_tapgemm_stat_rows_for(pair->op->geom, d);
            ProfScope ps(c, 0, pair->op->geom, pair->epi, ws, 2);
            LF_TRY(lf_tapbwd16_launch(op.geom, pair->op->geom, a, d, wpro, pair->epi, ws));
            c.pair_fused = true;
        }
    }
    if (!c.pair_fused) {
        ProfScope ps(c, 1, op.geom, 0, ws);
        LF_TRY(lf_tapwgrad_launch(op.geom, a, wpro, ws));
    }
    c.wgrad_launched = true;
    const LfPackEntry& e = P->packs[op.pack];
    const int nsplit = lf_tapwgrad_splits_for(op.geom, a, pro_sc ? LF_PRO_BNRELU : LF_PRO_NONE);
    if (batched) {
        c.wpart_used += wneed; c.bpart_used += bneed;
        LfReduceJob j = lf_wgrad_reduce_job(op.geom, a.partial, nsplit, c.grads[cv.p_w], e.sk, e.sn, e.tapidx, a.bias_partial, c.grads[cv.p_b]);
        if (chain) lf_bias_chain_job(*chain, j, nsplit, a.bias_partial != nullptr);
        c.reduce_jobs.push_back(j);
        return 0;
    }
    LF_TRY(lf_wgrad_reduce_launch(a.partial, nsplit, op.geom.ntaps, op.geom.Cs, op.geom.Cd,
                                  c.grads[cv.p_w], e.sk, e.sn, e.tapidx, a.bias_partial, nsplit,
                                  c.grads[cv.p_b], bias_accumulate, ws));
    return 0;
}

int run_bwd_pair(const Ctx& c, const ConvRef& cv, const float* x, const float* g, const float* pro_sc, const float* pro_sh, float* dst,
                 int epi, const LfTapArgs& extra) {
    const PairDg pair = {&cv.dg[0], dst, epi, extra};
    LF_TRY(run_wgrad(c, cv.fwd, cv, x, g, pro_sc, pro_sh, 0, false, nullptr, &pair));
    if (c.pair_fused) return 0;
    return run_gemm(c, cv.dg[0], g, dst, nullptr, LF_PRO_NONE, epi, extra, true);
}

struct RowSums { float* wrows; float* brows; bool batched; };
RowSums row_sum_regions(const Ctx& c, long wneed, long bneed) {
    const lf_erfnet_plan* P = c.P;
    wneed = (wneed + 63) / 64 * 64; bneed = (bneed + 63) / 64 * 64;
    const bool batched = !c.no_batch && c.wpart_used + wneed <= P->wpart_all_floats[c.s16] && c.bpart_used + bneed <= P->bpart_all_floats[c.s16];
    RowSums r;
    r.batched = batched;
    r.wrows = batched ? c.at(P->off_wpart_all + c.wpart_used) : c.at(P->off_wpart);
    r.brows = batched ? c.at(P->off_wpart_all + P->wpart_all_floats[c.s16] + c.bpart_used) : c.at(P->off_bpart);
    if (batched) { c.wpart_used += wneed; c.bpart_used += bneed; }
    return r;
}
int row_sums_finish(const Ctx& c, const RowSums& r, int rows, int nw, float* gw, int nb, float* gb) {
    if (!r.batched) {
        LF_TRY(lf_rows_reduce_launch(r.wrows, rows, nw, gw, 0, c.st));
        if (gb) LF_TRY(lf_rows_reduce_launch(r.brows, rows, nb, gb, 0, c.st));
        return 0;
    }
    c.reduce_jobs.push_back(lf_row_sum_job(r.wrows, rows, nw, gw));
    if (gb) c.reduce_jobs.push_back(lf_row_sum_job(r.brows, rows, nb, gb));
    return 0;
}

int bn_bwd_finalize(const Ctx& c, const BNRef& b, const LfStatPart* parts, int nparts, double count) {
    if (!c.grads[b.p_g] || !c.grads[b.p_b]) return lf_fail("erfnet backward: BatchNorm weight/bias must both require grad");
    return lf_bn_bwd_finalize(parts, nparts, b.C, count, c.at(b.asc), c.at(b.ash), c.at(b.c1), c.at(b.c2), c.grads[b.p_g],
                              c.grads[b.p_b], c.training, c.st);
}

struct Prep {
    const float* y = nullptr;
    const float* pre = nullptr;
    const BNRef* bn = nullptr;
    const float* dm = nullptr;
};

Prep prep_for(const Ctx& c, const Layer& Lp) {
    Prep p;
    if (Lp.kind == K_NB) {
        p.y = c.at(Lp.b[4]); p.pre = c.at(Lp.b[3]); p.bn = &Lp.bn[1];
        p.dm = (Lp.drop_idx >= 0 && c.dropmask) ? c.dropmask + c.P->drop_off[Lp.drop_idx] : nullptr;
    } else {
        p.y = c.at(Lp.b[1]); p.pre = c.at(Lp.b[0]); p.bn = &Lp.bn[0];
    }
    return p;
}

int backward_layers(const Ctx& c, const float* img, float* g0, float* g1, float* g2, int nlayers, int first = 0,
                    float** gin = nullptr) {
    const lf_erfnet_plan* P = c.P;
    const int N = P->N;
    float* stat0 = c.at(P->off_stat0);
    float* bufs[3] = {g0, g1, g2};
    float* in = g0;
    bool prepped = false;
    int prep_rows = 0, prep_ld = 0;
    for (int li = nlayers - 1; li >= first; --li) {
        const Layer& L = P->layers[li];
        P->prof_layer = 100 + li;
        const long npo = (long)N * L.Hout * L.Wout;
        const long ppi = (long)L.Hout * L.Wout;
        const int iin = in == bufs[0] ? 0 : (in == bufs[1] ? 1 : 2);
        float* X = bufs[(iin + 1) % 3];
        float* Y = bufs[(iin + 2) % 3];
        Prep nx;
        const bool can_prep = li > first && (L.kind == K_NB || L.kind == K_UP);
        if (can_prep) nx = prep_for(c, P->layers[li - 1]);
        auto add_prep = [&](LfTapArgs& a, int& epi, const LfTapGeom& dg) {
            if (!can_prep) return;
            a.mask_src = nx.y; a.aux = nx.pre; a.asc = c.at(nx.bn->asc); a.ash = c.at(nx.bn->ash); a.dm = nx.dm;
            a.stats = stat0; a.stats_ld = lf_stat_ld(lf_tapgemm_stat_rows(dg));
            epi |= LF_EPI_MASK | LF_EPI_STATS_XHAT;
        };
        const BNRef& blast = L.kind == K_NB ? L.bn[1] : L.bn[0];
        const float* ylast = c.at(L.kind == K_NB ? L.b[4] : L.b[1]);
        const float* prelast = c.at(L.kind == K_NB ? L.b[3] : L.b[0]);
        const float* dm = (L.kind == K_NB && L.drop_idx >= 0 && c.dropmask) ? c.dropmask + P->drop_off[L.drop_idx] : nullptr;
        const float* gz;
        if (!prepped) {
            const int rrows = lf_bn_bwd_reduce_rows(npo);
            LF_TRY(lf_bn_bwd_reduce(in, ylast, prelast, c.at(blast.asc), c.at(blast.ash), dm, stat0, lf_stat_ld(rrows), npo, L.Cout, ppi, c.s16, c.st));
            LfStatPart rp = {stat0, rrows, L.Cout, 0, lf_stat_ld(rrows)};
            LF_TRY(bn_bwd_finalize(c, blast, &rp, 1, (double)npo));
            LF_TRY(lf_bn_bwd_apply(in, ylast, prelast, c.at(blast.asc), c.at(blast.ash), c.params[blast.p_g], c.at(blast.c1),
                                   c.at(blast.c2), dm, X, L.kind == K_NB ? Y : nullptr, npo, L.Cout, ppi, c.s16, c.st));
            gz = Y;
        } else {
            LfStatPart rp = {stat0, prep_rows, L.Cout, 0, prep_ld};
            LF_TRY(bn_bwd_finalize(c, blast, &rp, 1, (double)npo));
            LF_TRY(lf_bn_bwd_apply(in, nullptr, prelast, c.at(blast.asc), c.at(blast.ash), c.params[blast.p_g], c.at(blast.c1),
                                   c.at(blast.c2), dm, X, nullptr, npo, L.Cout, ppi, c.s16, c.st));
            gz = in;
        }
        float* F = prepped ? Y : in;
        float* out = nullptr;
        prepped = false;
        if (L.kind == K_NB) {
            const float* x = c.at(L.x);
            const float *t1 = c.at(L.b[0]), *t2 = c.at(L.b[1]), *t3 = c.at(L.b[2]);
            const BNRef& b1 = L.bn[0];
            LfTapArgs a = lf_no_args();
            a.mask_src = t3;
            LF_TRY(run_bwd_pair(c, L.cv[3], t3, X, nullptr, nullptr, F, LF_EPI_MASK, a));
            a = lf_no_args();
            a.aux = t2; a.msc = c.at(b1.sc); a.msh = c.at(b1.sh); a.asc = c.at(b1.asc); a.ash = c.at(b1.ash);
            a.stats = stat0; a.stats_ld = lf_stat_ld(lf_tapgemm_stat_rows(L.cv[2].dg[0].geom));
            LF_TRY(run_bwd_pair(c, L.cv[2], t2, F, c.at(b1.sc), c.at(b1.sh), X, LF_EPI_MASKBN | LF_EPI_STATS_XHAT, a));
            LfStatPart sp = {stat0, c.last_rows, L.Cout, 0, a.stats_ld};
            LF_TRY(bn_bwd_finalize(c, b1, &sp, 1, (double)npo));
            LF_TRY(lf_bn_bwd_apply(X, nullptr, t2, c.at(b1.asc), c.at(b1.ash), c.params[b1.p_g], c.at(b1.c1), c.at(b1.c2),
                                   nullptr, F , nullptr, npo, L.Cout, ppi, c.s16, c.st));
            a = lf_no_args();
            a.mask_src = t1;
            LF_TRY(run_bwd_pair(c, L.cv[1], t1, F, nullptr, nullptr, X, LF_EPI_MASK, a));
            a = lf_no_args();
            a.add_src = gz;
            int epi = LF_EPI_ADD;
            add_prep(a, epi, L.cv[0].dg[0].geom);
            LF_TRY(run_bwd_pair(c, L.cv[0], x, X, nullptr, nullptr, F, epi, a));
            out = F;
            if (can_prep) { prepped = true; prep_rows = c.last_rows; prep_ld = a.stats_ld; }
        } else if (L.kind == K_UP) {
            long wsum = 0, bsum = 0;
            for (int ph = 0; ph < 4; ++ph) {
                wsum += (wneed_of(L.cv[0].fph[ph].geom, c.s16) + 63) / 64 * 64;
                bsum += (bneed_of(L.cv[0].fph[ph].geom, c.s16) + 63) / 64 * 64;
            }
            const bool chained = !c.no_batch && c.wpart_used + wsum <= P->wpart_all_floats[c.s16] && c.bpart_used + bsum <= P->bpart_all_floats[c.s16];
            BiasChain bc;
            for (int ph = 0; ph < 4; ++ph) {
                if (chained) LF_TRY(run_wgrad(c, L.cv[0].fph[ph], L.cv[0], c.at(L.x), X, nullptr, nullptr, 0, false, &bc));
                else LF_TRY(run_wgrad(c, L.cv[0].fph[ph], L.cv[0], c.at(L.x), X, nullptr, nullptr, ph > 0, true));
            }
            LfTapArgs a = lf_no_args();
            int epi = 0;
            if (c.g_enc && L.x == lf_erfnet_encoder_offset(P)) {
                a.add_src = c.g_enc;
                epi |= LF_EPI_ADD;
            }
            add_prep(a, epi, L.cv[0].dg[0].geom);
            LF_TRY(run_gemm(c, L.cv[0].dg[0], X, F, nullptr, LF_PRO_NONE, epi, a));
            out = F;
            if (can_prep) { prepped = true; prep_rows = c.last_rows; prep_ld = a.stats_ld; }
        } else if (L.x < 0) {
            const int Cc = 16 - L.Cin, rows = lf_stem_wgrad_rows(N, L.Hin, L.Win);
            if (c.grads[L.cv[0].p_w]) {
                const RowSums rs = row_sum_regions(c, (long)rows * Cc * L.Cin * 9, (long)rows * Cc);
                LF_TRY(lf_stem_wgrad(img, X, N, L.Cin, L.Hin, L.Win, rs.wrows, rs.brows, c.s16, c.st));
                LF_TRY(row_sums_finish(c, rs, rows, Cc * L.Cin * 9, c.grads[L.cv[0].p_w], Cc, c.grads[L.cv[0].p_b]));
            }
            if (c.g_img) LF_TRY(lf_stem_bwd_data(X, img, c.params[L.cv[0].p_w], N, L.Cin, L.Hin, L.Win, c.s16, c.g_img, c.st));
            out = F;
        } else {
            LF_TRY(run_wgrad(c, L.cv[0].fwd, L.cv[0], c.at(L.x), X, nullptr, nullptr, 0));
            LF_TRY(lf_pool_bwd(c.at(L.x), X, N, L.Hin, L.Win, L.Cin, L.Cout, L.Cout - L.Cin, F, c.s16, c.st));
            for (int ph = 0; ph < 4; ++ph) {
                LfTapArgs a = lf_no_args();
                a.add_src = F;
                LF_TRY(run_gemm(c, L.cv[0].dg[ph], X, F, nullptr, LF_PRO_NONE, LF_EPI_ADD, a));
            }
            out = F;
        }
        in = out;
    }
    if (gin) *gin = in;
    return 0;
}

int upload_and_pack(const Ctx& c, const float* const* params_dev) {
    const lf_erfnet_plan* P = c.P;
    LfPackEntry* ent = reinterpret_cast<LfPackEntry*>(c.at(P->off_entries));
    if (hipMemcpyAsync(ent, P->packs.data(), P->packs.size() * sizeof(LfPackEntry), hipMemcpyHostToDevice, c.st) != hipSuccess)
        return lf_fail("erfnet: upload of the pack table failed");
    LF_TRY(lf_pack_weights_launch(ent, (int)P->packs.size(), params_dev, c.at(P->off_packed), c.st));
    if (P->precision == 2)
        LF_TRY(lf_pack_weights_bf16_launch(ent, (int)P->packs.size(), params_dev, c.at(P->off_packed16), c.st));
    if (P->precision == 3)
        LF_TRY(lf_pack_weights_split_launch(ent, (int)P->packs.size(), params_dev, c.at(P->off_packed48), c.st));
    return 0;
}

}

extern "C" {


int lf_erfnet_forward(const lf_erfnet_plan* P, const float* img, const float* const* params_host,
                      const float* const* params_dev, float* const* running_host, const float* dropmask, int training,
                      int head, float* logits, void* workspace, size_t workspace_bytes, void* stream) {
    LF_REQUIRE(P && img && params_host && params_dev && running_host && (logits || head < 0) && workspace, "lf_erfnet_forward: null pointer");
    LF_REQUIRE(workspace_bytes >= lf_erfnet_workspace_bytes(P), "lf_erfnet_forward: workspace too small");
    LF_REQUIRE(head >= -1 && head < P->n_heads, "lf_erfnet_forward: head %d out of range", head);
    Ctx c{P, (float*)workspace, params_host, nullptr, running_host, dropmask, training, (hipStream_t)stream};
    c.s16 = P->precision == 2;
    LF_TRY(upload_and_pack(c, params_dev));
    if (head < 0) return forward_layers(c, img, encoder_layers(P));
    LF_TRY(forward_layers(c, img, (int)P->layers.size()));
    return lf_head_fwd(c.at(P->head_in), params_host[P->p_head_w[head]], params_host[P->p_head_b[head]], logits, P->N, P->H / 2,
                       P->W / 2, P->Cout + head, c.s16, c.st);
}

int lf_erfnet_backward_input(const lf_erfnet_plan* P, const float* img, const float* grad_logits,
                             const float* grad_encoder, const float* const* params_host, float* const* grads_host,
// ... 502 lines not shown
```

lanedetection_end2end_amd/csrc/lf_ops.hip:

```cpp
#include "lf_conv.h"
#include "lf_debug.h"
#include "lf_eltwise.h"
#include "lf_plan.h"

namespace {

TapIdx conv1d_taps(int flip) {
    TapIdx ti;
    memset(&ti, 0, sizeof(ti));
    for (int t = 0; t < 3; ++t) ti.v[t] = flip ? 2 - t : t;
    return ti;
}

__global__ __launch_bounds__(256) void pack_one_kernel(const float* __restrict__ w, float* __restrict__ dst, int Kc, int Nc,
                                                      int ntaps, long sk, long sn, const TapIdx ti) {
    const long total = (long)ntaps * Kc * Nc;
    for (long i = (long)blockIdx.x * 256 + threadIdx.x; i < total; i += (long)gridDim.x * 256) {
        const int k4 = (int)(i & 3);
        long r = i >> 2;
        const int n = (int)(r % Nc);
        r /= Nc;
        const int kb = (int)(r % (Kc >> 2));
        const int t = (int)(r / (Kc >> 2));
        dst[i] = w[(kb * 4 + k4) * sk + n * sn + ti.v[t]];
    }
}

__global__ __launch_bounds__(256) void pack_one_bf16_kernel(const float* __restrict__ w, __bf16* __restrict__ dst, int Kc, int Nc,
                                                           int ntaps, long sk, long sn, const TapIdx ti) {
    const int kb_per_tap = ((Kc + 31) >> 5) * 4;
    const long total = (long)ntaps * kb_per_tap * Nc * 8;
    for (long i = (long)blockIdx.x * 256 + threadIdx.x; i < total; i += (long)gridDim.x * 256) {
        const int k8 = (int)(i & 7);
        long r = i >> 3;
        const int n = (int)(r % Nc);
        r /= Nc;
        const int kb = (int)(r % kb_per_tap);
        const int t = (int)(r / kb_per_tap);
        const int k = kb * 8 + k8;
        dst[i] = (__bf16)(k < Kc ? w[k * sk + n * sn + ti.v[t]] : 0.f);
    }
}

__global__ __launch_bounds__(256) void pack_one_split_kernel(const float* __restrict__ w, __bf16* __restrict__ dst, int Kc, int Nc,
                                                            int ntaps, long sk, long sn, const TapIdx ti) {
    const int kb_per_tap = Kc >> 3;
    const long total = (long)ntaps * kb_per_tap * Nc * 8;
    for (long i = (long)blockIdx.x * 256 + threadIdx.x; i < total; i += (long)gridDim.x * 256) {
        const int k8 = (int)(i & 7);
        const long row = i >> 3;
        long r = row;
        const int n = (int)(r % Nc);
        r /= Nc;
        const int kb = (int)(r % kb_per_tap);
        const int t = (int)(r / kb_per_tap);
        const float v = w[(kb * 8 + k8) * sk + n * sn + ti.v[t]];
        const __bf16 vh = (__bf16)v;
        const float r1 = v - (float)vh;
        const __bf16 vm = (__bf16)r1;
        dst[row * 24 + k8] = vh; dst[row * 24 + 8 + k8] = vm; dst[row * 24 + 16 + k8] = (__bf16)(r1 - (float)vm);
    }
}

int g_ops_bf16 = 0;

void pack_conv1d(LfTapArgs& a, const float* w, float* scratch, int C, long sk, long sn, int flip, hipStream_t st) {
    if (g_ops_bf16 == 9) {
        hipLaunchKernelGGL(pack_one_kernel, dim3(64), dim3(256), 0, st, w, scratch, C, C, 3, sk, sn, conv1d_taps(flip));
        if (C % 32 == 0) {
            hipLaunchKernelGGL(pack_one_split_kernel, dim3(64), dim3(256), 0, st, w, reinterpret_cast<__bf16*>(scratch + 3L * C * C),
                               C, C, 3, sk, sn, conv1d_taps(flip));
            a.split = g_ops_bf16;
            a.wp48 = scratch + 3L * C * C;
        }
    } else if (g_ops_bf16 == 2) {
        hipLaunchKernelGGL(pack_one_bf16_kernel, dim3(64), dim3(256), 0, st, w, reinterpret_cast<__bf16*>(scratch), C, C, 3, sk, sn, conv1d_taps(flip));
        a.wp16 = scratch;
        a.s16 = 1;
    } else {
        hipLaunchKernelGGL(pack_one_kernel, dim3(64), dim3(256), 0, st, w, scratch, C, C, 3, sk, sn, conv1d_taps(flip));
    }
    a.wp = scratch;
}

LfTapGeom conv1d_geom(int N, int H, int W, int C, int axis, int d) {
    LfTapGeom g;
    memset(&g, 0, sizeof(g));
    g.N = N; g.Hl = H; g.Wl = W; g.Hs = H; g.Ws = W; g.s_pix = C; g.ssh = 1; g.ssw = 1;
    g.Hd = H; g.Wd = W; g.d_pix = C; g.dsh = 1; g.dsw = 1; g.Cs = C; g.Cd = C; g.ntaps = 3;
    for (int t = 0; t < 3; ++t) { g.tdh[t] = axis == 0 ? (t - 1) * d : 0; g.tdw[t] = axis == 1 ? (t - 1) * d : 0; }
    return g;
}

}

extern "C" {

void lf_debug_set_split_any_size(int v) { lf_tapgemm_set_split_any_size(v); }
void lf_debug_set_bf16_lds(int v) { lf_tapgemm_set_bf16_lds(v); }
void lf_debug_set_bf16_no_partial_fast(int v) { lf_tapgemm_set_bf16_no_partial_fast(v); }
void lf_debug_set_ops_precision(int mode) { g_ops_bf16 = (mode == 2 || mode == 9) ? mode : 0; }

void lf_debug_set_wgrad_ro(int mode, int cap64, int cap128) { lf_tapwgrad_ro_set(mode, cap64, cap128); }
void lf_debug_set_fp32_stream(int mode, int max_workgroups) { lf_tapgemm_set_fp32_stream(mode, max_workgroups); }
void lf_debug_set_bwd16_fused(int mode) { lf_tapbwd16_set(mode); }
void lf_debug_set_fwd_pair(int mode, int max_workgroups) { lf_tappair_set(mode, max_workgroups); }
long lf_debug_bias_residual_launches(void) { return lf_tapgemm_bias_residual_launches(); }
void lf_debug_set_thin(int mode, int nt) { lf_tapgemm_set_thin(mode, nt); }
long lf_debug_thin_launches(void) { return lf_tapgemm_thin_launches(); }
long lf_debug_fold_pack_launches(void) { return lf_fold_pack_launches(); }
long lf_debug_partial_fast_launches(void) { return lf_tapgemm_partial_fast_launches(); }
long lf_debug_bf16_ring_launches(void) { return lf_tapgemm_bf16_ring_launches(); }
void lf_debug_set_bf16_max_workgroups(int v) { lf_tapgemm_set_bf16_max_workgroups(v); }

int lf_debug_conv1d_fwd_phases(const float* x, const float* w, const float* bias, float* y, int N, int H, int W, int C,
                               int axis, int dilation, float* scratch, unsigned long long* dbg, void* stream) {
    hipStream_t st = (hipStream_t)stream;
    const LfTapGeom g = conv1d_geom(N, H, W, C, axis, dilation);
    LfTapArgs a;
    memset(&a, 0, sizeof(a));
    pack_conv1d(a, w, scratch, C, 3L, 3L * C, 0, st);
    a.src = x; a.bias = bias; a.dst = y; a.dbg = dbg;
    return lf_tapgemm_launch(g, a, LF_PRO_NONE, 0, st);
}

int lf_debug_conv1d_fwd_pro(const float* x, const float* w, const float* bias, const float* sc, const float* sh, float* y, int N, int H,
                            int W, int C, int axis, int dilation, float* scratch, void* stream) {
    LF_REQUIRE(x && w && y && sc && sh && scratch, "lf_debug_conv1d_fwd_pro: null pointer");
    hipStream_t st = (hipStream_t)stream;
    const LfTapGeom g = conv1d_geom(N, H, W, C, axis, dilation);
    LfTapArgs a;
    memset(&a, 0, sizeof(a));
    pack_conv1d(a, w, scratch, C, 3L, 3L * C, 0, st);
    a.src = x; a.bias = bias; a.dst = y; a.pro_sc = sc; a.pro_sh = sh;
    return lf_tapgemm_launch(g, a, LF_PRO_BNRELU, LF_EPI_RELU, st);
}

int lf_debug_conv1d_fwd_pair(const float* x, const float* wa, const float* ba, const float* wb, const float* bb, const float* sc,
                             const float* sh, float* t, float* y, float* stats, int N, int H, int W, int C, int dilation, float* scratch,
                             void* stream) {
    if (!(x && wa && wb && t && y && stats && scratch) || (sc != nullptr) != (sh != nullptr)) { lf_fail("lf_debug_conv1d_fwd_pair: null pointer"); return -1; }
    if (N < 1 || H < 1 || W < 1 || C < 16 || C % 16 != 0 || dilation < 1) { lf_fail("lf_debug_conv1d_fwd_pair: bad arguments"); return -1; }
    if (g_ops_bf16 != 0) { lf_fail("lf_debug_conv1d_fwd_pair: fp32 tensors in precision mode 0 only"); return -1; }
    hipStream_t st = (hipStream_t)stream;
    const LfTapGeom ga = conv1d_geom(N, H, W, C, 0, dilation), gb = conv1d_geom(N, H, W, C, 1, dilation);
    LfTapArgs aa, ab;
    memset(&aa, 0, sizeof(aa));
    memset(&ab, 0, sizeof(ab));
    pack_conv1d(aa, wa, scratch, C, 3L, 3L * C, 0, st);
    pack_conv1d(ab, wb, scratch + 3L * C * C, C, 3L, 3L * C, 0, st);
    aa.src = x; aa.bias = ba; aa.dst = t; aa.pro_sc = sc; aa.pro_sh = sh;
    ab.src = t; ab.bias = bb; ab.dst = y; ab.stats = stats;
    ab.stats_ld = lf_tapgemm_stat_rows(gb);
    const int pro = sc ? LF_PRO_BNRELU : LF_PRO_NONE;
    if (lf_tappair_routed(C, pro) && lf_tappair_ok(ga, gb, aa, ab, pro, LF_EPI_RELU, LF_EPI_STATS_SQ))
        return lf_tappair_launch(ga, gb, aa, ab, pro, st) ? -1 : 1;
    if (lf_tapgemm_launch(ga, aa, pro, LF_EPI_RELU, st) || lf_tapgemm_launch(gb, ab, LF_PRO_NONE, LF_EPI_STATS_SQ, st)) return -1;
    return 0;
}

int lf_debug_conv1d_wgrad_phases(const float* x, const float* gy, int N, int H, int W, int C, int axis, int dilation,
                                 float* scratch, unsigned long long* dbg, void* stream) {
    const LfTapGeom g = conv1d_geom(N, H, W, C, axis, dilation);
    LfWgradArgs a;
    a.x = x; a.g = gy; a.pro_sc = nullptr; a.pro_sh = nullptr; a.s16 = 0; a.split = 0;
    a.partial = scratch; a.bias_partial = nullptr; a.dbg = dbg;
    const int rc = lf_tapwgrad_launch(g, a, LF_PRO_NONE, (hipStream_t)stream);
    return rc ? -1 : lf_tapwgrad_splits_for(g, a, LF_PRO_NONE) * 3 * (C / 64) * (C / 64) * 4;
}

long lf_conv1d_scratch_floats(int N, int H, int W, int C) {
    const LfTapGeom g = conv1d_geom(N, H, W, C, 0, 1);
    long a = 8L * C * C;
    const long rows = lf_tapwgrad_splits_bound(g, 1);
    long b = rows * 3 * C * C + rows * C;
    return a > b ? a : b;
}

int lf_conv1d_fwd(const float* x, const float* w, const float* bias, float* y, int N, int H, int W, int C, int axis,
                  int dilation, int relu, float* scratch, void* stream) {
    LF_REQUIRE(x && w && y && scratch, "lf_conv1d_fwd: null pointer");
    hipStream_t st = (hipStream_t)stream;
    const LfTapGeom g = conv1d_geom(N, H, W, C, axis, dilation);
    LfTapArgs a;
    memset(&a, 0, sizeof(a));
    pack_conv1d(a, w, scratch, C, 3L, 3L * C, 0, st);
    a.src = x; a.bias = bias; a.dst = y;
    return lf_tapgemm_launch(g, a, LF_PRO_NONE, relu ? LF_EPI_RELU : 0, st);
// ... 225 lines not shown
        }
        if (tile_pix[i] < 0 || (tile_pix[i] > 0 && (seg_rows[i] < 1 || nrows[i] % seg_rows[i] != 0 || seg_pix[i] > (long)seg_rows[i] * tile_pix[i] ||
                                                    seg_pix[i] <= (long)(seg_rows[i] - 1) * tile_pix[i]))) {
            lf_fail("%s: source %d: centred rows need the launch geometry (nrows=%d seg_rows=%d seg_pix=%ld tile_pix=%d)", who, i, nrows[i],
                    seg_rows[i], seg_pix[i], tile_pix[i]);
            return -1;
        }
        parts[n] = {rows[i], nrows[i], Cs[i], ch_off[i], ld[i]};
        parts[n].tile_pix = tile_pix[i]; parts[n].seg_rows = seg_rows[i]; parts[n].seg_pix = seg_pix[i];
        ++n;
    }
    return n;
}
bool stream_ok(const char* who, long npix, int C, long pix_per_image, const float* dm) {
    if (npix < 1 || C < 4 || C % 4 != 0 || pix_per_image < 1 || (dm && npix % pix_per_image != 0)) {
        lf_fail("%s: bad arguments (npix %ld C %d pix_per_image %ld)", who, npix, C, pix_per_image);
        return false;
    }
    return true;
}
bool pool_ok(const char* who, int N, int H, int W, int Cin, int cat_pix, int choff) {
    if (N < 1 || H < 2 || W < 2 || (H & 1) || (W & 1) || !quads_ok(Cin) || choff < 0 || choff % 4 != 0 || cat_pix % 4 != 0 || choff + Cin > cat_pix) {
        lf_fail("%s: bad arguments (N %d H %d W %d Cin %d cat_pix %d choff %d)", who, N, H, W, Cin, cat_pix, choff);
        return false;
    }
    return true;
}
}

int lf_debug_bn_finalize_fwd(const float* rows0, int nrows0, int ld0, int C0, int ch_off0, int tile_pix0, int seg_rows0, long seg_pix0,
                             const float* rows1, int nrows1, int ld1, int C1, int ch_off1, int tile_pix1, int seg_rows1, long seg_pix1,
                             int C, double count, const float* gamma, const float* beta, float* running_mean, float* running_var,
                             float momentum, float eps, int training, float* scale, float* shift, float* asc, float* ash, void* stream) {
    if (!(gamma && beta && running_mean && running_var && scale && shift && asc && ash)) { lf_fail("lf_debug_bn_finalize_fwd: null pointer"); return -1; }
    if (C < 4 || C % 4 != 0 || !(count >= 1.0)) { lf_fail("lf_debug_bn_finalize_fwd: bad arguments (C %d count %g)", C, count); return -1; }
    const float* const rows[2] = {rows0, rows1};
    const int nrows[2] = {nrows0, nrows1}, ld[2] = {ld0, ld1}, Cs[2] = {C0, C1}, ch_off[2] = {ch_off0, ch_off1}, tile_pix[2] = {tile_pix0, tile_pix1},
              seg_rows[2] = {seg_rows0, seg_rows1};
    const long seg_pix[2] = {seg_pix0, seg_pix1};
    LfStatPart parts[2];
    const int n = debug_stat_parts("lf_debug_bn_finalize_fwd", rows, nrows, ld, Cs, ch_off, tile_pix, seg_rows, seg_pix, C, parts);
    if (n < 0) return -1;
    if (training && n == 0) { lf_fail("lf_debug_bn_finalize_fwd: training mode needs a source of partial rows"); return -1; }
    return lf_bn_finalize_fwd(parts, n, C, count, gamma, beta, running_mean, running_var, momentum, eps, training, scale, shift, asc, ash,
                              (hipStream_t)stream) ? -1 : 0;
}

int lf_debug_bn_bwd_finalize(const float* rows0, int nrows0, int ld0, int C0, int ch_off0, int tile_pix0, int seg_rows0, long seg_pix0,
                             const float* rows1, int nrows1, int ld1, int C1, int ch_off1, int tile_pix1, int seg_rows1, long seg_pix1,
                             int C, double count, const float* asc, const float* ash, float* c1, float* c2, float* ggamma, float* gbeta,
                             int training, void* stream) {
    if (!(asc && ash && c1 && c2 && ggamma && gbeta)) { lf_fail("lf_debug_bn_bwd_finalize: null pointer"); return -1; }
    if (C < 4 || C % 4 != 0 || !(count >= 1.0)) { lf_fail("lf_debug_bn_bwd_finalize: bad arguments (C %d count %g)", C, count); return -1; }
    const float* const rows[2] = {rows0, rows1};
    const int nrows[2] = {nrows0, nrows1}, ld[2] = {ld0, ld1}, Cs[2] = {C0, C1}, ch_off[2] = {ch_off0, ch_off1}, tile_pix[2] = {tile_pix0, tile_pix1},
              seg_rows[2] = {seg_rows0, seg_rows1};
    const long seg_pix[2] = {seg_pix0, seg_pix1};
    LfStatPart parts[2];
    const int n = debug_stat_parts("lf_debug_bn_bwd_finalize", rows, nrows, ld, Cs, ch_off, tile_pix, seg_rows, seg_pix, C, parts);
    if (n < 0) return -1;
    if (n == 0) { lf_fail("lf_debug_bn_bwd_finalize: no source of partial rows"); return -1; }
    return lf_bn_bwd_finalize(parts, n, C, count, asc, ash, c1, c2, ggamma, gbeta, training, (hipStream_t)stream) ? -1 : 0;
}

int lf_debug_bn_act(const float* x, const float* sc, const float* sh, const float* dm, const float* res, float* y, long npix, int C,
                    long pix_per_image, int s16, void* stream) {
    if (!(x && sc && sh && y)) { lf_fail("lf_debug_bn_act: null pointer"); return -1; }
    if (!(al16(x) && al16(sc) && al16(sh) && al16(dm) && al16(res) && al16(y))) { lf_fail("lf_debug_bn_act: pointers must be 16-byte aligned"); return -1; }
    if (!stream_ok("lf_debug_bn_act", npix, C, pix_per_image, dm)) return -1;
    return lf_bn_act(x, sc, sh, dm, res, y, npix, C, pix_per_image, s16 != 0, (hipStream_t)stream) ? -1 : 0;
}

int lf_debug_bn_bwd_reduce(const float* g, const float* y, const float* t, const float* asc, const float* ash, const float* dm, float* rows,
                           int ld, long npix, int C, long pix_per_image, int s16, void* stream) {
    if (!(g && t && asc && ash && rows)) { lf_fail("lf_debug_bn_bwd_reduce: null pointer"); return -1; }
    if (!(al16(g) && al16(y) && al16(t) && al16(dm))) { lf_fail("lf_debug_bn_bwd_reduce: pointers must be 16-byte aligned"); return -1; }
    if (!stream_ok("lf_debug_bn_bwd_reduce", npix, C, pix_per_image, dm)) return -1;
    if (!quads_ok(C)) { lf_fail("lf_debug_bn_bwd_reduce: unsupported channel count %d", C); return -1; }
    const int nrows = lf_bn_bwd_reduce_rows(npix);
    if (ld < nrows) { lf_fail("lf_debug_bn_bwd_reduce: ld %d below the %d rows of the launch", ld, nrows); return -1; }
    return lf_bn_bwd_reduce(g, y, t, asc, ash, dm, rows, ld, npix, C, pix_per_image, s16 != 0, (hipStream_t)stream) ? -1 : nrows;
}

int lf_debug_bn_bwd_apply(const float* g, const float* y, const float* t, const float* asc, const float* ash, const float* gamma,
                          const float* c1, const float* c2, const float* dm, float* g_t, float* g_z, long npix, int C, long pix_per_image,
                          int s16, void* stream) {
    if (!(g && t && asc && ash && gamma && c1 && c2 && g_t)) { lf_fail("lf_debug_bn_bwd_apply: null pointer"); return -1; }
    if (!(al16(g) && al16(y) && al16(t) && al16(asc) && al16(ash) && al16(gamma) && al16(c1) && al16(c2) && al16(dm) && al16(g_t) && al16(g_z))) {
        lf_fail("lf_debug_bn_bwd_apply: pointers must be 16-byte aligned");
        return -1;
    }
    if (!stream_ok("lf_debug_bn_bwd_apply", npix, C, pix_per_image, dm)) return -1;
    return lf_bn_bwd_apply(g, y, t, asc, ash, gamma, c1, c2, dm, g_t, g_z, npix, C, pix_per_image, s16 != 0, (hipStream_t)stream) ? -1 : 0;
}

int lf_debug_pool_concat_fwd(const float* x, int N, int H, int W, int Cin, float* cat, int cat_pix, int choff, float* rows, int ld, int s16,
                             void* stream) {
    if (!(x && cat) || !al16(x) || !al16(cat)) { lf_fail("lf_debug_pool_concat_fwd: null or misaligned pointer"); return -1; }
    if (!pool_ok("lf_debug_pool_concat_fwd", N, H, W, Cin, cat_pix, choff)) return -1;
    const int nrows = lf_pool_rows((long)N * (H / 2) * (W / 2));
    if (rows && ld < nrows) { lf_fail("lf_debug_pool_concat_fwd: ld %d below the %d rows of the launch", ld, nrows); return -1; }
    return lf_pool_concat_fwd(x, N, H, W, Cin, cat, cat_pix, choff, rows, ld, s16 != 0, (hipStream_t)stream) ? -1 : nrows;
}

int lf_debug_pool_affine_fwd(const float* x, int N, int H, int W, int Cin, float* cat, int cat_pix, int choff, const float* sc, const float* sh,
                             int s16, void* stream) {
    if (!(x && cat && sc && sh) || !al16(x) || !al16(cat) || !al16(sc) || !al16(sh)) { lf_fail("lf_debug_pool_affine_fwd: null or misaligned pointer"); return -1; }
    if (!pool_ok("lf_debug_pool_affine_fwd", N, H, W, Cin, cat_pix, choff)) return -1;
    return lf_pool_affine_fwd(x, N, H, W, Cin, cat, cat_pix, choff, sc, sh, s16 != 0, (hipStream_t)stream) ? -1 : 0;
}

int lf_debug_pool_bwd(const float* x, const float* gcat, int N, int H, int W, int Cin, int cat_pix, int choff, float* gx, int s16, void* stream) {
    if (!(x && gcat && gx) || !al16(x) || !al16(gcat) || !al16(gx)) { lf_fail("lf_debug_pool_bwd: null or misaligned pointer"); return -1; }
    if (!pool_ok("lf_debug_pool_bwd", N, H, W, Cin, cat_pix, choff)) return -1;
    return lf_pool_bwd(x, gcat, N, H, W, Cin, cat_pix, choff, gx, s16 != 0, (hipStream_t)stream) ? -1 : 0;
}

int lf_debug_stem_fwd(const float* img, int N, int Cin, int H, int W, const float* w, const float* b, const float* sc, const float* sh, float* cat,
                      float* rows, int ld, int s16, void* stream) {
    if (!(img && w && b && cat) || !al16(cat)) { lf_fail("lf_debug_stem_fwd: null or misaligned pointer"); return -1; }
    if (N < 1 || Cin < 1 || Cin > 4 || H < 2 || W < 2 || (H & 1) || (W & 1)) {
        lf_fail("lf_debug_stem_fwd: bad arguments (N %d Cin %d H %d W %d)", N, Cin, H, W);
        return -1;
    }
    if ((sc == nullptr) != (sh == nullptr)) { lf_fail("lf_debug_stem_fwd: scale and shift come together"); return -1; }
    hipStream_t st = (hipStream_t)stream;
    if (sc) return lf_stem_fwd_infer(img, N, Cin, H, W, w, b, sc, sh, cat, s16 != 0, st) ? -1 : 0;
    const int nrows = lf_stem_rows(N, H, W);
    if (rows && ld < nrows) { lf_fail("lf_debug_stem_fwd: ld %d below the %d rows of the launch", ld, nrows); return -1; }
    return lf_stem_fwd(img, N, Cin, H, W, w, b, cat, rows, ld, s16 != 0, st) ? -1 : nrows;
}

int lf_debug_head_fwd(const float* x, const float* w, const float* b, float* out, int N, int h, int w_, int K, int s16, void* stream) {
    if (!(x && w && b && out) || !al16(x) || ((size_t)out & 7)) { lf_fail("lf_debug_head_fwd: null or misaligned pointer"); return -1; }
    if (N < 1 || h < 1 || w_ < 1 || K < 1 || K > 8) { lf_fail("lf_debug_head_fwd: bad arguments (N %d h %d w %d K %d)", N, h, w_, K); return -1; }
    return lf_head_fwd(x, w, b, out, N, h, w_, K, s16 != 0, (hipStream_t)stream) ? -1 : 0;
}

int lf_debug_head_bwd_data(const float* gout, const float* w, float* gx, int N, int h, int w_, int K, int s16, void* stream) {
    if (!(gout && w && gx) || !al16(gx) || ((size_t)gout & 7)) { lf_fail("lf_debug_head_bwd_data: null or misaligned pointer"); return -1; }
    if (N < 1 || h < 1 || w_ < 1 || K < 1 || K > 8) { lf_fail("lf_debug_head_bwd_data: bad arguments (N %d h %d w %d K %d)", N, h, w_, K); return -1; }
    return lf_head_bwd_data(gout, w, gx, N, h, w_, K, s16 != 0, (hipStream_t)stream) ? -1 : 0;
}

namespace {
int conv1d_bwd_weight(const float* x, const float* gy, const float* sc, const float* sh, float* gw, float* gb, int N, int H, int W, int C,
                      int axis, int dilation, float* scratch, hipStream_t st) {
    const LfTapGeom g = conv1d_geom(N, H, W, C, axis, dilation);
    const int pro = sc ? LF_PRO_BNRELU : LF_PRO_NONE;
    LfWgradArgs a;
    a.x = x; a.g = gy; a.pro_sc = sc; a.pro_sh = sh; a.s16 = g_ops_bf16 == 2;
    a.split = 0;
    a.partial = scratch;
    a.bias_partial = gb ? scratch + (long)lf_tapwgrad_splits_bound(g, 1) * 3 * C * C : nullptr;
    int rc = lf_tapwgrad_launch(g, a, pro, st);
    if (rc) return rc;
    const int idx[3] = {0, 1, 2};
    const int nsplit = lf_tapwgrad_splits_for(g, a, pro);
    return lf_wgrad_reduce_launch(a.partial, nsplit, 3, C, C, gw, 3L, 3L * C, idx, a.bias_partial, nsplit, gb, 0, st);
}
}

int lf_conv1d_bwd_weight(const float* x, const float* gy, float* gw, float* gb, int N, int H, int W, int C, int axis,
                         int dilation, float* scratch, void* stream) {
    LF_REQUIRE(x && gy && gw && scratch, "lf_conv1d_bwd_weight: null pointer");
    return conv1d_bwd_weight(x, gy, nullptr, nullptr, gw, gb, N, H, W, C, axis, dilation, scratch, (hipStream_t)stream);
}

long lf_debug_conv1d_bwd_pair_scratch_floats(int N, int H, int W, int C) {
    if (N < 1 || H < 1 || W < 1 || C < 1) return -1;
    const long rows = lf_tapwgrad_splits(conv1d_geom(N, H, W, C, 0, 1));
    return 3L * C * C + rows * (3L * C * C + C);
}

int lf_debug_conv1d_bwd_pair(const float* x, const float* gy, const float* w, int epi, const float* add_src, const float* aux,
                             const float* msc, const float* msh, const float* pro_sc, const float* pro_sh, float* gx, float* gw, float* gb,
                             float* stats, int N, int H, int W, int C, int axis, int dilation, float* scratch, void* stream) {
    if (!(x && gy && w && gx && gw && gb && scratch)) { lf_fail("lf_debug_conv1d_bwd_pair: null pointer"); return -1; }
    if (N < 1 || H < 1 || W < 1 || C < 1 || dilation < 1 || (axis != 0 && axis != 1)) { lf_fail("lf_debug_conv1d_bwd_pair: bad arguments"); return -1; }
    if (g_ops_bf16 == 2) { lf_fail("lf_debug_conv1d_bwd_pair: fp32 tensors only"); return -1; }
    hipStream_t st = (hipStream_t)stream;
    const LfTapGeom g = conv1d_geom(N, H, W, C, axis, dilation);
    const long rows = lf_tapwgrad_splits(g);
    LfTapArgs a;
    memset(&a, 0, sizeof(a));
    LfWgradArgs wa;
    wa.x = x; wa.g = gy; wa.pro_sc = pro_sc; wa.pro_sh = pro_sh; wa.s16 = 0; wa.split = 0;
    wa.partial = scratch + 3L * C * C;
    wa.bias_partial = wa.partial + rows * 3L * C * C;
    a.wp = scratch;
    a.src = gy; a.dst = gx; a.add_src = add_src; a.msc = msc; a.msh = msh; a.stats = stats;
    a.mask_src = (epi & LF_EPI_MASK) ? x : nullptr;
    a.aux = (epi & LF_EPI_MASKBN) ? x : aux;
    a.stats_ld = lf_tapgemm_stat_rows(g);
    const int pro = pro_sc ? LF_PRO_BNRELU : LF_PRO_NONE;
    if (!lf_tapbwd16_ok(g, g, wa, a, pro, epi)) {
        lf_fail("lf_debug_conv1d_bwd_pair: the fused kernel does not take this launch (epi %d, prologue %d, %d x %d x %d x %d)", epi, pro, N, H, W, C);
        return -1;
    }
    hipLaunchKernelGGL(pack_one_kernel, dim3(64), dim3(256), 0, st, w, scratch, C, C, 3, 3L * C, 3L, conv1d_taps(1));
    if (lf_tapbwd16_launch(g, g, wa, a, pro, epi, st)) return -1;
    const int idx[3] = {0, 1, 2};
    const int nsplit = lf_tapwgrad_splits_for(g, wa, pro);
    if (lf_wgrad_reduce_launch(wa.partial, nsplit, 3, C, C, gw, 3L, 3L * C, idx, wa.bias_partial, nsplit, gb, 0, st)) return -1;
    return (epi & LF_EPI_STATS_XHAT) ? lf_tapgemm_stat_rows_for(g, a) : 0;
}

int lf_debug_conv1d_wgrad_pro(const float* x, const float* gy, const float* sc, const float* sh, float* gw, float* gb, int N, int H, int W,
                              int C, int axis, int dilation, float* scratch, void* stream) {
    LF_REQUIRE(x && gy && sc && sh && gw && scratch, "lf_debug_conv1d_wgrad_pro: null pointer");
    return conv1d_bwd_weight(x, gy, sc, sh, gw, gb, N, H, W, C, axis, dilation, scratch, (hipStream_t)stream);
}

}
```

Baseline: 2065 images/sec.

## Fold BatchNorm-backward apply into the fused tap backward kernel

Adds a BN-fold variant of the fused conv1d backward kernel. It computes the BatchNorm input gradient (gamma·rstd·(g − c1 − x̂·c2)) while the tiles are being staged, so the separate lf_bn_bwd_apply pass over the activation is removed from the non-bottleneck block backward. The ERFNet block backward is rewired to route through this kernel and to ping-pong its output buffers. It also adds an optional g_z output to the BN backward reduce. The cost is three extra LDS tiles per stage, which means fewer pipeline stages, plus a new kernel instantiation.

Result: no change. 2073 images/sec (median of 6 runs) (+0.4%).

```diff
diff --git a/lanedetection_end2end_amd/_lib.py b/lanedetection_end2end_amd/_lib.py
--- a/lanedetection_end2end_amd/_lib.py
+++ b/lanedetection_end2end_amd/_lib.py
@@ -157,10 +157,12 @@
         "lf_debug_set_wgrad_ro": (None, [I, I, I]),
         "lf_debug_set_fp32_stream": (None, [I, I]),
         "lf_debug_set_bwd16_fused": (None, [I]),
+        "lf_debug_bn_bwd_launches": (L, [I]),
         "lf_debug_set_fwd_pair": (None, [I, I]),
         "lf_debug_conv1d_fwd_pair": (I, [P, P, P, P, P, P, P, P, P, P, I, I, I, I, I, P, P]),
         "lf_debug_conv1d_bwd_pair_scratch_floats": (L, [I, I, I, I]),
         "lf_debug_conv1d_bwd_pair": (I, [P, P, P, I, P, P, P, P, P, P, P, P, P, P, I, I, I, I, I, I, P, P]),
+        "lf_debug_conv1d_bwd_pair_bn": (I, [P, P, P, I, P, P, P, P, P, P, P, P, P, P, I, I, I, I, I, I, P, P, P, P, P, P, P, P, P]),
         "lf_debug_conv1d_bwd_data_epi3": (I, [P, P, P, P, P, P, P, I, I, I, I, I, I, P, P]),
         "lf_debug_conv1d_epi": (I, [P, P, P, P, I, I, P, P, P, P, P, P, I, I, I, I, I, I, P, P]),
         "lf_debug_conv1d_wgrad_pro": (I, [P, P, P, P, P, P, I, I, I, I, I, I, P, P]),
@@ -175,6 +177,7 @@
         "lf_debug_bn_bwd_finalize": (I, [P, I, I, I, I, I, I, L] * 2 + [I, D, P, P, P, P, P, P, I, P]),
         "lf_debug_bn_act": (I, [P, P, P, P, P, P, L, I, L, I, P]),
         "lf_debug_bn_bwd_reduce": (I, [P, P, P, P, P, P, P, I, L, I, L, I, P]),
+        "lf_debug_bn_bwd_reduce_gz": (I, [P, P, P, P, P, P, P, I, L, I, L, I, P, P]),
         "lf_debug_bn_bwd_apply": (I, [P, P, P, P, P, P, P, P, P, P, P, L, I, L, I, P]),
         "lf_debug_pool_concat_fwd": (I, [P, I, I, I, I, P, I, I, P, I, I, P]),
         "lf_debug_pool_affine_fwd": (I, [P, I, I, I, I, P, I, I, P, P, I, P]),
diff --git a/lanedetection_end2end_amd/csrc/lf_bwd16.hip b/lanedetection_end2end_amd/csrc/lf_bwd16.hip
--- a/lanedetection_end2end_amd/csrc/lf_bwd16.hip
+++ b/lanedetection_end2end_amd/csrc/lf_bwd16.hip
@@ -4,13 +4,15 @@
 namespace {
 
 constexpr int B16_TILE = 1024;
-template <int EPIC> struct B16Cfg {
+template <int EPIC, bool BNF = false> struct B16Cfg {
     static constexpr bool ST_ADD = (EPIC & LF_EPI_ADD) != 0;
     static constexpr bool AUX_IS_X = (EPIC & LF_EPI_MASKBN) != 0;
     static constexpr bool ST_AUX = (EPIC & LF_EPI_STATS_XHAT) != 0 && !AUX_IS_X;
     static constexpr bool SUMS = (EPIC & LF_EPI_STATS_XHAT) != 0;
     static constexpr int T_ADD = 6, T_AUX = ST_AUX ? 6 + (ST_ADD ? 1 : 0) : 4;
-    static constexpr int NTILE = 6 + (ST_ADD ? 1 : 0) + (ST_AUX ? 1 : 0);
+    static constexpr int T_BNT = 6;
+    static constexpr int NTILE = 6 + (ST_ADD ? 1 : 0) + (ST_AUX ? 1 : 0) + (BNF ? 3 : 0);
+    static_assert(!BNF || (!ST_ADD && !ST_AUX), "the BatchNorm-backward fold is a form of the mask epilogue");
     static constexpr int STAGES = NTILE == 6 ? 3 : 2;
     static constexpr int STAGE = NTILE * B16_TILE, WAVE_LDS = STAGES * STAGE;
     static_assert(WG_WAVES * WAVE_LDS + 1024 <= 80 * 1024, "two workgroups per CU");
@@ -21,214 +23,33 @@
 typedef __attribute__((address_space(3))) f32x4* lds_f32x4_p;
 typedef __attribute__((address_space(3))) unsigned char* lds_u8_p;
 
+__device__ __forceinline__ float bn_fold_dt(float gv, float tv, float gr, float rs, float sh, float c1, float c2) {
+    const float xh = __fmaf_rn(tv, rs, sh);
+    return __fmul_rn(gr, __fmaf_rn(-xh, c2, __fsub_rn(gv, c1)));
+}
+
 template <bool PRO, int EPIC>
 __global__ __launch_bounds__(256, 2) void tapbwd16_kernel(const LfTapGeom g, const LfWgradArgs wa, const LfTapArgs a, const long pps,
                                                           const int write_bias, const int wave_rows) {
-    using Cfg = B16Cfg<EPIC>;
-    constexpr int NTAPS = 3, NT = 1, epi = EPIC;
-    constexpr bool S16 = false, HOISTV = true;
-    const int lane = threadIdx.x & 63, wave = __builtin_amdgcn_readfirstlane((int)(threadIdx.x >> 6));
-    const int pl = lane & 15, kq = lane >> 4;
-    const long npix_l = (long)g.N * g.Hl * g.Wl;
-    const unsigned npix = (unsigned)npix_l, bx = blockIdx.x;
-    const int cob = 0;
-    const long sub = (long)blockIdx.x * WG_WAVES + wave;
-    const long p_begin = sub * pps;
-    long p_end = p_begin + pps;
-    if (p_end > npix_l) p_end = npix_l;
-    const int niter = p_end > p_begin ? (int)((p_end - p_begin + 15) / 16) : 0;
-    f32x4 acc[NTAPS];
-#pragma unroll
-    for (int t = 0; t < NTAPS; ++t) acc[t] = zero4();
-    float bsum = 0.f;
-    const unsigned tbytes = (unsigned)min((long)g.N * g.Hs * g.Ws * g.s_pix * 4, (long)LF_OOB);
-    const i32x4s rx = make_rsrc_words(wa.x, tbytes), rg = make_rsrc_words(wa.g, tbytes),
-                 radd = make_rsrc_words(a.add_src, Cfg::ST_ADD ? tbytes : 0u), raux = make_rsrc_words(a.aux, Cfg::ST_AUX ? tbytes : 0u);
-    lds_u8_p const ring = (lds_u8_p)lf_tap_lds + wave * Cfg::WAVE_LDS;
-    const unsigned lds0 = (unsigned)(size_t)ring;
-    const int tdh0 = g.tdh[0], tdh1 = g.tdh[1], tdh2 = g.tdh[2], tdw0 = g.tdw[0], tdw1 = g.tdw[1], tdw2 = g.tdw[2];
-    long p_ld = p_begin;
-    int pj_, pi_, pn_;
-    row1_coords(g, niter ? (unsigned)p_begin : 0u, pn_, pi_, pj_);
-    int cj = pj_, ci = pi_, cn = pn_;
-    const int px = lane >> 2, chunk = lane & 3;
-    int slot_ld = 0;
-    auto issue = [&]() __attribute__((always_inline)) {
-        const bool ok = p_ld < p_end;
-        const int j = pj_ + px;
-        const unsigned dst = lds0 + (unsigned)(slot_ld * Cfg::STAGE);
-#pragma unroll
-        for (int t = 0; t < NTAPS; ++t) {
-            const int dh = t == 0 ? tdh0 : t == 1 ? tdh1 : tdh2, dw = t == 0 ? tdw0 : t == 1 ? tdw1 : tdw2;
-            const int sy = pi_ + dh, sx = j + dw;
-            const bool in = ok && sy >= 0 && sy < g.Hs && sx >= 0 && sx < g.Ws;
-            const unsigned o = in ? (unsigned)((((pn_ * g.Hs + sy) * g.Ws + sx) * g.s_pix + g.s_choff + chunk * 4) * 4) : LF_OOB;
-            lds_dma16(rg, dst + (unsigned)(t * B16_TILE), o, 0u);
-            lds_dma16(rx, dst + (unsigned)((3 + t) * B16_TILE), o, 0u);
-        }
-        if constexpr (Cfg::ST_ADD || Cfg::ST_AUX) {
-            const unsigned o = ok ? (unsigned)((((pn_ * g.Hs + pi_) * g.Ws + j) * g.s_pix + g.s_choff + chunk * 4) * 4) : LF_OOB;
-            if constexpr (Cfg::ST_ADD) lds_dma16(radd, dst + (unsigned)(Cfg::T_ADD * B16_TILE), o, 0u);
-            if constexpr (Cfg::ST_AUX) lds_dma16(raux, dst + (unsigned)(Cfg::T_AUX * B16_TILE), o, 0u);
-        }
-        slot_ld = slot_ld == Cfg::STAGES - 1 ? 0 : slot_ld + 1;
-        p_ld += 16;
-        pj_ += 16;
-        if (pj_ >= g.Wl) { pj_ = 0; if (++pi_ >= g.Hl) { pi_ = 0; ++pn_; } }
-    };
-    f32x4 w3[NTAPS];
-    {
-        const __amdgpu_buffer_rsrc_t rwl = make_rsrc(a.wp, (unsigned)(NTAPS * 16 * 16 * 4));
-#pragma unroll
-        for (int t = 0; t < NTAPS; ++t) w3[t] = ldb4(rwl, (unsigned)(kq * 16 + pl) * 16u, (unsigned)(t * 16 * 64));
-    }
-    float psc = 1.f, psh = 0.f;
-    if constexpr (PRO) { psc = wa.pro_sc[pl]; psh = wa.pro_sh[pl]; }
-#undef LF_EPI_ACC
-#define LF_EPI_ACC(n, m) dacc
-#undef LF_EPI_LDADD
-#define LF_EPI_LDADD(o) (*(lds_f32x4_p)(epi_lane + Cfg::T_ADD * B16_TILE))
-#undef LF_EPI_LDMSK
-#define LF_EPI_LDMSK(o) (*(lds_f32x4_p)(epi_lane + 4 * B16_TILE))
-#undef LF_EPI_LDAUX
-#define LF_EPI_LDAUX(o) (*(lds_f32x4_p)(epi_lane + Cfg::T_AUX * B16_TILE))
-#undef LF_EPI_HOIST_ALL
-#define LF_EPI_HOIST_ALL true
-#undef LF_EPI_ROW1
-#define LF_EPI_ROW1 true
-    LF_EPI_HEAD
-    (void)r_add; (void)r_msk; (void)r_aux;
-    if constexpr ((EPIC & LF_EPI_MASKBN) != 0) asm volatile("" ::"v"(hv[0][0]), "v"(hv[0][1]) : "memory");
-    asm volatile("s_waitcnt vmcnt(0)" ::"v"(w3[0]), "v"(w3[1]), "v"(w3[2]), "v"(psc), "v"(psh) : "memory");
-#pragma unroll
-    for (int q = 0; q < Cfg::STAGES - 1; ++q) issue();
-    int slot_c = 0;
-    f32x4 row1 = zero4(), row2 = zero4();
-    for (int it = 0; it < niter; ++it) {
-        asm volatile("s_waitcnt lgkmcnt(0)" ::: "memory");
-        issue();
-        wait_vm_lgkm0<Cfg::NTILE * (Cfg::STAGES - 1)>();
-        lds_u8_p const st = ring + slot_c * Cfg::STAGE;
-        slot_c = slot_c == Cfg::STAGES - 1 ? 0 : slot_c + 1;
-        lds_u8_p const epi_lane = st + pl * 64 + kq * 16;
-        {
-            lds_f32_p const frag = (lds_f32_p)(st + kq * 64 + pl * 4);
-            float gv[4], xv[NTAPS][4];
-#pragma unroll
-            for (int u = 0; u < 4; ++u) {
-                gv[u] = frag[(1 * B16_TILE + u * 256) / 4];
-#pragma unroll
-                for (int t = 0; t < NTAPS; ++t) xv[t][u] = frag[((3 + t) * B16_TILE + u * 256) / 4];
-            }
-            if constexpr (PRO) {
-#pragma unroll
-                for (int t = 0; t < NTAPS; ++t) {
-                    const int dh = t == 0 ? tdh0 : t == 1 ? tdh1 : tdh2, dw = t == 0 ? tdw0 : t == 1 ? tdw1 : tdw2;
-                    const bool rowok = (unsigned)(ci + dh) < (unsigned)g.Hs;
-                    const int c0 = cj + dw;
-                    const bool edge = c0 < 0 || c0 + 15 >= g.Ws;
-#pragma unroll
-                    for (int u = 0; u < 4; ++u) {
-                        float v = fmaxf(xv[t][u] * psc + psh, 0.f);
-                        if (edge) v = (unsigned)(c0 + 4 * u + kq) < (unsigned)g.Ws ? v : 0.f;
-                        xv[t][u] = rowok ? v : 0.f;
-                    }
-                }
-            }
-#pragma unroll
-            for (int u = 0; u < 4; ++u) {
-#pragma unroll
-                for (int t = 0; t < NTAPS; ++t) acc[t] = __builtin_amdgcn_mfma_f32_16x16x4f32(xv[t][u], gv[u], acc[t], 0, 0, 0);
-                bsum += gv[u];
-            }
-        }
-        f32x4 dacc;
-#pragma unroll
-        for (int t = 0; t < NTAPS; ++t) {
-            const f32x4 x3 = *(lds_f32x4_p)(epi_lane + t * B16_TILE);
-            f32x4 part;
-#pragma unroll
-            for (int s4 = 0; s4 < 4; ++s4) part = __builtin_amdgcn_mfma_f32_16x16x4f32(w3[t][s4], x3[s4], s4 ? part : zero4(), 0, 0, 0);
-            dacc = t ? dacc + part : part;
-        }
-        {
-            const int pn[1] = {cn}, pi[1] = {ci}, pj[1] = {cj + pl};
-            const bool pv[1] = {true};
-            LF_EPI_TILE(0)
-        }
-        if constexpr (Cfg::SUMS) {
-            if (wave_rows && ((it & 3) == 3 || it == niter - 1)) {
-                f32x4 q1, q2;
-                q1.x = sum16(s1[0].x); q1.y = sum16(s1[0].y); q1.z = sum16(s1[0].z); q1.w = sum16(s1[0].w);
-                q2.x = sum16(s2[0].x); q2.y = sum16(s2[0].y); q2.z = sum16(s2[0].z); q2.w = sum16(s2[0].w);
-                const bool first = (it & 15) < 4;
-                row1 = first ? q1 : row1 + q1;
-                row2 = first ? q2 : row2 + q2;
-                s1[0] = zero4(); s2[0] = zero4();
-                if (((it & 15) == 15 || it == niter - 1) && pl == 0) {
-                    const long row = (p_begin >> 8) + (it >> 4);
-#pragma unroll
-                    for (int e = 0; e < 4; ++e) {
-                        a.stats[(long)(kq * 4 + e) * a.stats_ld + row] = row1[e];
-                        a.stats[(long)(g.Cd + kq * 4 + e) * a.stats_ld + row] = row2[e];
-                    }
-                }
-            }
-        }
-        cj += 16;
-        if (cj >= g.Wl) { cj = 0; if (++ci >= g.Hl) { ci = 0; ++cn; } }
-    }
-    asm volatile("s_waitcnt vmcnt(0)" ::: "memory");
-    if (!wave_rows) {
-        const int pn[1] = {0};
-        LF_EPI_TAIL
-    }
-#undef LF_EPI_ACC
-#define LF_EPI_ACC(n, m) acc[n][m]
-#undef LF_EPI_LDADD
-#define LF_EPI_LDADD(o) epi_ld<S16>(r_add, o)
-#undef LF_EPI_LDMSK
-#define LF_EPI_LDMSK(o) epi_ld<S16>(r_msk, o)
-#undef LF_EPI_LDAUX
-#define LF_EPI_LDAUX(o) epi_ld<S16>(r_aux, o)
-#undef LF_EPI_HOIST_ALL
-#define LF_EPI_HOIST_ALL false
-#undef LF_EPI_ROW1
-#define LF_EPI_ROW1 false
-    float* const red = reinterpret_cast<float*>(lf_tap_lds);
-    constexpr int RW = Cfg::WAVE_LDS / 4;
-    if (wave > 0) {
-#pragma unroll
-        for (int t = 0; t < NTAPS; ++t)
-#pragma unroll
-            for (int e = 0; e < 4; ++e) red[wave * RW + (t * 4 + e) * 64 + lane] = acc[t][e];
-    }
-    red[wave * RW + 12 * 64 + lane] = bsum;
-    __syncthreads();
-    if (wave == 0) {
-#pragma unroll
-        for (int t = 0; t < NTAPS; ++t) {
-            float* out = wa.partial + ((long)blockIdx.x * NTAPS + t) * g.Cs * g.Cd;
-#pragma unroll
-            for (int e = 0; e < 4; ++e) {
-                float v = acc[t][e];
-#pragma unroll
-                for (int w = 1; w < WG_WAVES; ++w) v += red[w * RW + (t * 4 + e) * 64 + lane];
-                out[(long)(4 * kq + e) * g.Cd + pl] = v;
-            }
-        }
-        if (write_bias && wa.bias_partial) {
-            float v = red[12 * 64 + lane] + red[RW + 12 * 64 + lane] + red[2 * RW + 12 * 64 + lane] + red[3 * RW + 12 * 64 + lane];
-            v += __shfl_xor(v, 16, 64);
-            v += __shfl_xor(v, 32, 64);
-            if (kq == 0) wa.bias_partial[(long)blockIdx.x * g.Cd + pl] = v;
-        }
-    }
+    constexpr bool BNF = false;
+    const LfBnFold bn = {};
+#include "lf_bwd16_body.h"
+}
+
+__global__ __launch_bounds__(256, 2) void tapbwd16_bn_kernel(const LfTapGeom g, const LfWgradArgs wa, const LfTapArgs a, const LfBnFold bn,
+                                                             const long pps, const int write_bias, const int wave_rows) {
+    constexpr bool PRO = false, BNF = true;
+    constexpr int EPIC = LF_EPI_MASK;
+#include "lf_bwd16_body.h"
 }
 
 std::atomic<int> g_bwd16_mode{1};
-enum { B16_MASK = 1, B16_MASKBN = 2, B16_EPI3 = 4, B16_ADD = 8 };
-constexpr int g_bwd16_routed = B16_MASK | B16_MASKBN | B16_EPI3 | B16_ADD;
+enum { B16_MASK = 1, B16_MASKBN = 2, B16_EPI3 = 4, B16_ADD = 8, B16_BNFOLD = 16, B16_GZ = 32 };
+constexpr int g_bwd16_routed = B16_MASK | B16_MASKBN | B16_EPI3 | B16_ADD | B16_BNFOLD;
+int routed_forms() {
+    const int mode = g_bwd16_mode.load();
+    return mode == 0 ? 0 : mode == 1 ? g_bwd16_routed : mode >> 1;
+}
 
 int form_of(int pro, int epi) {
     if (pro == LF_PRO_NONE && epi == LF_EPI_MASK) return B16_MASK;
@@ -250,15 +71,24 @@
 }
 
 void lf_tapbwd16_set(int mode) { g_bwd16_mode = mode < 0 ? 0 : mode; }
-bool lf_tapbwd16_routed(int pro, int epi) {
-    const int mode = g_bwd16_mode.load();
-    const int forms = mode == 0 ? 0 : mode == 1 ? g_bwd16_routed : mode >> 1;
+bool lf_tapbwd16_routed(int pro, int epi, bool bnfold) {
+    const int forms = routed_forms();
+    if (bnfold && !(forms & B16_BNFOLD)) return false;
     return (forms & form_of(pro, epi)) != 0;
 }
+static std::atomic<long> g_bwd16_bn_launches{0};
+long lf_tapbwd16_bn_launches() { return g_bwd16_bn_launches.load(); }
+bool lf_tapbwd16_reduce_gz() { return (routed_forms() & B16_GZ) != 0; }
 
-bool lf_tapbwd16_ok(const LfTapGeom& gf, const LfTapGeom& gd, const LfWgradArgs& w, const LfTapArgs& a, int pro, int epi) {
+bool lf_tapbwd16_ok(const LfTapGeom& gf, const LfTapGeom& gd, const LfWgradArgs& w, const LfTapArgs& a, int pro, int epi, const LfBnFold* bn) {
     const int form = form_of(pro, epi);
     if (!form) return false;
+    if (bn) {
+        if (form != B16_MASK) return false;
+        if (!bn->t || !bn->asc || !bn->ash || !bn->gamma || !bn->c1 || !bn->c2 || bn->t == a.dst) return false;
+        for (const float* v : {bn->asc, bn->ash, bn->gamma, bn->c1, bn->c2})
+            if (reinterpret_cast<size_t>(v) % 16) return false;
+    }
     const LfTapGeom& g = gf;
     bool same = gf.N == gd.N && gf.Hl == gd.Hl && gf.Wl == gd.Wl && gf.Hs == gd.Hs && gf.Ws == gd.Ws && gf.s_pix == gd.s_pix && gf.s_choff == gd.s_choff &&
                 gf.ssh == gd.ssh && gf.ssw == gd.ssw && gf.Hd == gd.Hd && gf.Wd == gd.Wd && gf.d_pix == gd.d_pix && gf.d_choff == gd.d_choff &&
@@ -286,21 +116,29 @@
         if (!(pps % 256 == 0 || pps == 64 || (lf_tapwgrad_splits(g) == 1 && npix <= 256))) return false;
         if (a.stats_ld < lf_tapgemm_stat_rows(g)) return false;
     }
+    if (bn) return allow_big_lds(reinterpret_cast<const void*>(tapbwd16_bn_kernel), 128 * 1024);
     return with_form(form, [&](auto kern, auto cfg) {
         return allow_big_lds(reinterpret_cast<const void*>(kern), 128 * 1024);
     });
 }
 
-int lf_tapbwd16_launch(const LfTapGeom& gf, const LfTapGeom& gd, const LfWgradArgs& w, const LfTapArgs& a, int pro, int epi, hipStream_t st) {
-    LF_REQUIRE(lf_tapbwd16_ok(gf, gd, w, a, pro, epi), "tapbwd16: the fused kernel does not take this launch (pro %d, epi %d, %d x %d x %d x %d -> %d)",
+int lf_tapbwd16_launch(const LfTapGeom& gf, const LfTapGeom& gd, const LfWgradArgs& w, const LfTapArgs& a, int pro, int epi, hipStream_t st,
+                       const LfBnFold* bn) {
+    LF_REQUIRE(lf_tapbwd16_ok(gf, gd, w, a, pro, epi, bn), "tapbwd16: the fused kernel does not take this launch (pro %d, epi %d, %d x %d x %d x %d -> %d)",
                pro, epi, gf.N, gf.Hl, gf.Wl, gf.Cs, gf.Cd);
     const long pps = lf_tapwgrad_wave_pixels(gf);
     const int gx = lf_tapwgrad_splits(gf);
     const int wave_rows = pps % 256 == 0;
-    with_form(form_of(pro, epi), [&](auto kern, auto cfg) {
-        hipLaunchKernelGGL(kern, dim3(gx), dim3(256), (size_t)WG_WAVES * decltype(cfg)::WAVE_LDS, st, gf, w, a, pps, 1, wave_rows);
-        return true;
-    });
+    if (bn) {
+        using CfgBn = B16Cfg<LF_EPI_MASK, true>;
+        hipLaunchKernelGGL(tapbwd16_bn_kernel, dim3(gx), dim3(256), (size_t)WG_WAVES * CfgBn::WAVE_LDS, st, gf, w, a, *bn, pps, 1, wave_rows);
+    } else {
+        with_form(form_of(pro, epi), [&](auto kern, auto cfg) {
+            hipLaunchKernelGGL(kern, dim3(gx), dim3(256), (size_t)WG_WAVES * decltype(cfg)::WAVE_LDS, st, gf, w, a, pps, 1, wave_rows);
+            return true;
+        });
+    }
     LF_CHECK_LAUNCH("tapbwd16");
+    if (bn) ++g_bwd16_bn_launches;
     return 0;
 }
diff --git a/lanedetection_end2end_amd/csrc/lf_bwd16_body.h b/lanedetection_end2end_amd/csrc/lf_bwd16_body.h
--- /dev/null
+++ b/lanedetection_end2end_amd/csrc/lf_bwd16_body.h
@@ -0,0 +1,234 @@
+    using Cfg = B16Cfg<EPIC, BNF>;
+    constexpr int NTAPS = 3, NT = 1, epi = EPIC;
+    constexpr bool S16 = false, HOISTV = true;
+    const int lane = threadIdx.x & 63, wave = __builtin_amdgcn_readfirstlane((int)(threadIdx.x >> 6));
+    const int pl = lane & 15, kq = lane >> 4;
+    const long npix_l = (long)g.N * g.Hl * g.Wl;
+    const unsigned npix = (unsigned)npix_l, bx = blockIdx.x;
+    const int cob = 0;
+    const long sub = (long)blockIdx.x * WG_WAVES + wave;
+    const long p_begin = sub * pps;
+    long p_end = p_begin + pps;
+    if (p_end > npix_l) p_end = npix_l;
+    const int niter = p_end > p_begin ? (int)((p_end - p_begin + 15) / 16) : 0;
+    f32x4 acc[NTAPS];
+#pragma unroll
+    for (int t = 0; t < NTAPS; ++t) acc[t] = zero4();
+    float bsum = 0.f;
+    const unsigned tbytes = (unsigned)min((long)g.N * g.Hs * g.Ws * g.s_pix * 4, (long)LF_OOB);
+    const i32x4s rx = make_rsrc_words(wa.x, tbytes), rg = make_rsrc_words(wa.g, tbytes),
+                 radd = make_rsrc_words(a.add_src, Cfg::ST_ADD ? tbytes : 0u), raux = make_rsrc_words(a.aux, Cfg::ST_AUX ? tbytes : 0u),
+                 rbnt = make_rsrc_words(BNF ? bn.t : nullptr, BNF ? tbytes : 0u);
+    lds_u8_p const ring = (lds_u8_p)lf_tap_lds + wave * Cfg::WAVE_LDS;
+    const unsigned lds0 = (unsigned)(size_t)ring;
+    const int tdh0 = g.tdh[0], tdh1 = g.tdh[1], tdh2 = g.tdh[2], tdw0 = g.tdw[0], tdw1 = g.tdw[1], tdw2 = g.tdw[2];
+    long p_ld = p_begin;
+    int pj_, pi_, pn_;
+    row1_coords(g, niter ? (unsigned)p_begin : 0u, pn_, pi_, pj_);
+    int cj = pj_, ci = pi_, cn = pn_;
+    const int px = lane >> 2, chunk = lane & 3;
+    int slot_ld = 0;
+    auto issue = [&]() __attribute__((always_inline)) {
+        const bool ok = p_ld < p_end;
+        const int j = pj_ + px;
+        const unsigned dst = lds0 + (unsigned)(slot_ld * Cfg::STAGE);
+#pragma unroll
+        for (int t = 0; t < NTAPS; ++t) {
+            const int dh = t == 0 ? tdh0 : t == 1 ? tdh1 : tdh2, dw = t == 0 ? tdw0 : t == 1 ? tdw1 : tdw2;
+            const int sy = pi_ + dh, sx = j + dw;
+            const bool in = ok && sy >= 0 && sy < g.Hs && sx >= 0 && sx < g.Ws;
+            const unsigned o = in ? (unsigned)((((pn_ * g.Hs + sy) * g.Ws + sx) * g.s_pix + g.s_choff + chunk * 4) * 4) : LF_OOB;
+            lds_dma16(rg, dst + (unsigned)(t * B16_TILE), o, 0u);
+            lds_dma16(rx, dst + (unsigned)((3 + t) * B16_TILE), o, 0u);
+            if constexpr (BNF) lds_dma16(rbnt, dst + (unsigned)((Cfg::T_BNT + t) * B16_TILE), o, 0u);
+        }
+        if constexpr (Cfg::ST_ADD || Cfg::ST_AUX) {
+            const unsigned o = ok ? (unsigned)((((pn_ * g.Hs + pi_) * g.Ws + j) * g.s_pix + g.s_choff + chunk * 4) * 4) : LF_OOB;
+            if constexpr (Cfg::ST_ADD) lds_dma16(radd, dst + (unsigned)(Cfg::T_ADD * B16_TILE), o, 0u);
+            if constexpr (Cfg::ST_AUX) lds_dma16(raux, dst + (unsigned)(Cfg::T_AUX * B16_TILE), o, 0u);
+        }
+        slot_ld = slot_ld == Cfg::STAGES - 1 ? 0 : slot_ld + 1;
+        p_ld += 16;
+        pj_ += 16;
+        if (pj_ >= g.Wl) { pj_ = 0; if (++pi_ >= g.Hl) { pi_ = 0; ++pn_; } }
+    };
+    f32x4 w3[NTAPS];
+    {
+        const __amdgpu_buffer_rsrc_t rwl = make_rsrc(a.wp, (unsigned)(NTAPS * 16 * 16 * 4));
+#pragma unroll
+        for (int t = 0; t < NTAPS; ++t) w3[t] = ldb4(rwl, (unsigned)(kq * 16 + pl) * 16u, (unsigned)(t * 16 * 64));
+    }
+    float psc = 1.f, psh = 0.f;
+    if constexpr (PRO) { psc = wa.pro_sc[pl]; psh = wa.pro_sh[pl]; }
+    float bw_gr = 0.f, bw_rs = 0.f, bw_sh = 0.f, bw_c1 = 0.f, bw_c2 = 0.f;
+    f32x4 bd_gr = zero4(), bd_rs = zero4(), bd_sh = zero4(), bd_c1 = zero4(), bd_c2 = zero4();
+    if constexpr (BNF) {
+        bw_rs = bn.asc[pl]; bw_sh = bn.ash[pl]; bw_c1 = bn.c1[pl]; bw_c2 = bn.c2[pl];
+        bw_gr = __fmul_rn(bn.gamma[pl], bw_rs);
+        bd_rs = *reinterpret_cast<const f32x4*>(bn.asc + 4 * kq); bd_sh = *reinterpret_cast<const f32x4*>(bn.ash + 4 * kq);
+        bd_c1 = *reinterpret_cast<const f32x4*>(bn.c1 + 4 * kq); bd_c2 = *reinterpret_cast<const f32x4*>(bn.c2 + 4 * kq);
+        const f32x4 gm = *reinterpret_cast<const f32x4*>(bn.gamma + 4 * kq);
+#pragma unroll
+        for (int e = 0; e < 4; ++e) bd_gr[e] = __fmul_rn(gm[e], bd_rs[e]);
+    }
+#undef LF_EPI_ACC
+#define LF_EPI_ACC(n, m) dacc
+#undef LF_EPI_LDADD
+#define LF_EPI_LDADD(o) (*(lds_f32x4_p)(epi_lane + Cfg::T_ADD * B16_TILE))
+#undef LF_EPI_LDMSK
+#define LF_EPI_LDMSK(o) (*(lds_f32x4_p)(epi_lane + 4 * B16_TILE))
+#undef LF_EPI_LDAUX
+#define LF_EPI_LDAUX(o) (*(lds_f32x4_p)(epi_lane + Cfg::T_AUX * B16_TILE))
+#undef LF_EPI_HOIST_ALL
+#define LF_EPI_HOIST_ALL true
+#undef LF_EPI_ROW1
+#define LF_EPI_ROW1 true
+    LF_EPI_HEAD
+    (void)r_add; (void)r_msk; (void)r_aux;
+    if constexpr ((EPIC & LF_EPI_MASKBN) != 0) asm volatile("" ::"v"(hv[0][0]), "v"(hv[0][1]) : "memory");
+    if constexpr (BNF)
+        asm volatile("" ::"v"(bw_gr), "v"(bw_rs), "v"(bw_sh), "v"(bw_c1), "v"(bw_c2), "v"(bd_gr), "v"(bd_rs), "v"(bd_sh), "v"(bd_c1), "v"(bd_c2) : "memory");
+    asm volatile("s_waitcnt vmcnt(0)" ::"v"(w3[0]), "v"(w3[1]), "v"(w3[2]), "v"(psc), "v"(psh) : "memory");
+#pragma unroll
+    for (int q = 0; q < Cfg::STAGES - 1; ++q) issue();
+    int slot_c = 0;
+    f32x4 row1 = zero4(), row2 = zero4();
+    for (int it = 0; it < niter; ++it) {
+        asm volatile("s_waitcnt lgkmcnt(0)" ::: "memory");
+        issue();
+        wait_vm_lgkm0<Cfg::NTILE * (Cfg::STAGES - 1)>();
+        lds_u8_p const st = ring + slot_c * Cfg::STAGE;
+        slot_c = slot_c == Cfg::STAGES - 1 ? 0 : slot_c + 1;
+        lds_u8_p const epi_lane = st + pl * 64 + kq * 16;
+        const int left = BNF ? (int)min(p_end - p_begin - 16L * it, 16L) : 16;
+        (void)left;
+        {
+            lds_f32_p const frag = (lds_f32_p)(st + kq * 64 + pl * 4);
+            float gv[4], xv[NTAPS][4];
+#pragma unroll
+            for (int u = 0; u < 4; ++u) {
+                gv[u] = frag[(1 * B16_TILE + u * 256) / 4];
+#pragma unroll
+                for (int t = 0; t < NTAPS; ++t) xv[t][u] = frag[((3 + t) * B16_TILE + u * 256) / 4];
+            }
+            if constexpr (BNF) {
+#pragma unroll
+                for (int u = 0; u < 4; ++u) {
+                    const float v = bn_fold_dt(gv[u], frag[((Cfg::T_BNT + 1) * B16_TILE + u * 256) / 4], bw_gr, bw_rs, bw_sh, bw_c1, bw_c2);
+                    gv[u] = 4 * u + kq < left ? v : 0.f;
+                }
+            }
+            if constexpr (PRO) {
+#pragma unroll
+                for (int t = 0; t < NTAPS; ++t) {
+                    const int dh = t == 0 ? tdh0 : t == 1 ? tdh1 : tdh2, dw = t == 0 ? tdw0 : t == 1 ? tdw1 : tdw2;
+                    const bool rowok = (unsigned)(ci + dh) < (unsigned)g.Hs;
+                    const int c0 = cj + dw;
+                    const bool edge = c0 < 0 || c0 + 15 >= g.Ws;
+#pragma unroll
+                    for (int u = 0; u < 4; ++u) {
+                        float v = fmaxf(xv[t][u] * psc + psh, 0.f);
+                        if (edge) v = (unsigned)(c0 + 4 * u + kq) < (unsigned)g.Ws ? v : 0.f;
+                        xv[t][u] = rowok ? v : 0.f;
+                    }
+                }
+            }
+#pragma unroll
+            for (int u = 0; u < 4; ++u) {
+#pragma unroll
+                for (int t = 0; t < NTAPS; ++t) acc[t] = __builtin_amdgcn_mfma_f32_16x16x4f32(xv[t][u], gv[u], acc[t], 0, 0, 0);
+                bsum += gv[u];
+            }
+        }
+        f32x4 dacc;
+#pragma unroll
+        for (int t = 0; t < NTAPS; ++t) {
+            f32x4 x3 = *(lds_f32x4_p)(epi_lane + t * B16_TILE);
+            if constexpr (BNF) {
+                const f32x4 t3 = *(lds_f32x4_p)(epi_lane + (Cfg::T_BNT + t) * B16_TILE);
+                const int dh = t == 0 ? tdh0 : t == 1 ? tdh1 : tdh2, dw = t == 0 ? tdw0 : t == 1 ? tdw1 : tdw2;
+                const bool in = (unsigned)(ci + dh) < (unsigned)g.Hs && (unsigned)(cj + dw + pl) < (unsigned)g.Ws && pl < left;
+#pragma unroll
+                for (int e = 0; e < 4; ++e) {
+                    const float v = bn_fold_dt(x3[e], t3[e], bd_gr[e], bd_rs[e], bd_sh[e], bd_c1[e], bd_c2[e]);
+                    x3[e] = in ? v : 0.f;
+                }
+            }
+            f32x4 part;
+#pragma unroll
+            for (int s4 = 0; s4 < 4; ++s4) part = __builtin_amdgcn_mfma_f32_16x16x4f32(w3[t][s4], x3[s4], s4 ? part : zero4(), 0, 0, 0);
+            dacc = t ? dacc + part : part;
+        }
+        {
+            const int pn[1] = {cn}, pi[1] = {ci}, pj[1] = {cj + pl};
+            const bool pv[1] = {true};
+            LF_EPI_TILE(0)
+        }
+        if constexpr (Cfg::SUMS) {
+            if (wave_rows && ((it & 3) == 3 || it == niter - 1)) {
+                f32x4 q1, q2;
+                q1.x = sum16(s1[0].x); q1.y = sum16(s1[0].y); q1.z = sum16(s1[0].z); q1.w = sum16(s1[0].w);
+                q2.x = sum16(s2[0].x); q2.y = sum16(s2[0].y); q2.z = sum16(s2[0].z); q2.w = sum16(s2[0].w);
+                const bool first = (it & 15) < 4;
+                row1 = first ? q1 : row1 + q1;
+                row2 = first ? q2 : row2 + q2;
+                s1[0] = zero4(); s2[0] = zero4();
+                if (((it & 15) == 15 || it == niter - 1) && pl == 0) {
+                    const long row = (p_begin >> 8) + (it >> 4);
+#pragma unroll
+                    for (int e = 0; e < 4; ++e) {
+                        a.stats[(long)(kq * 4 + e) * a.stats_ld + row] = row1[e];
+                        a.stats[(long)(g.Cd + kq * 4 + e) * a.stats_ld + row] = row2[e];
+                    }
+                }
+            }
+        }
+        cj += 16;
+        if (cj >= g.Wl) { cj = 0; if (++ci >= g.Hl) { ci = 0; ++cn; } }
+    }
+    asm volatile("s_waitcnt vmcnt(0)" ::: "memory");
+    if (!wave_rows) {
+        const int pn[1] = {0};
+        LF_EPI_TAIL
+    }
+#undef LF_EPI_ACC
+#define LF_EPI_ACC(n, m) acc[n][m]
+#undef LF_EPI_LDADD
+#define LF_EPI_LDADD(o) epi_ld<S16>(r_add, o)
+#undef LF_EPI_LDMSK
+#define LF_EPI_LDMSK(o) epi_ld<S16>(r_msk, o)
+#undef LF_EPI_LDAUX
+#define LF_EPI_LDAUX(o) epi_ld<S16>(r_aux, o)
+#undef LF_EPI_HOIST_ALL
+#define LF_EPI_HOIST_ALL false
+#undef LF_EPI_ROW1
+#define LF_EPI_ROW1 false
+    float* const red = reinterpret_cast<float*>(lf_tap_lds);
+    constexpr int RW = Cfg::WAVE_LDS / 4;
+    if (wave > 0) {
+#pragma unroll
+        for (int t = 0; t < NTAPS; ++t)
+#pragma unroll
+            for (int e = 0; e < 4; ++e) red[wave * RW + (t * 4 + e) * 64 + lane] = acc[t][e];
+    }
+    red[wave * RW + 12 * 64 + lane] = bsum;
+    __syncthreads();
+    if (wave == 0) {
+#pragma unroll
+        for (int t = 0; t < NTAPS; ++t) {
+            float* out = wa.partial + ((long)blockIdx.x * NTAPS + t) * g.Cs * g.Cd;
+#pragma unroll
+            for (int e = 0; e < 4; ++e) {
+                float v = acc[t][e];
+#pragma unroll
+                for (int w = 1; w < WG_WAVES; ++w) v += red[w * RW + (t * 4 + e) * 64 + lane];
+                out[(long)(4 * kq + e) * g.Cd + pl] = v;
+            }
+        }
+        if (write_bias && wa.bias_partial) {
+            float v = red[12 * 64 + lane] + red[RW + 12 * 64 + lane] + red[2 * RW + 12 * 64 + lane] + red[3 * RW + 12 * 64 + lane];
+            v += __shfl_xor(v, 16, 64);
+            v += __shfl_xor(v, 32, 64);
+            if (kq == 0) wa.bias_partial[(long)blockIdx.x * g.Cd + pl] = v;
+        }
+    }
diff --git a/lanedetection_end2end_amd/csrc/lf_conv.h b/lanedetection_end2end_amd/csrc/lf_conv.h
--- a/lanedetection_end2end_amd/csrc/lf_conv.h
+++ b/lanedetection_end2end_amd/csrc/lf_conv.h
@@ -95,10 +95,22 @@
 int lf_tapwgrad_splits_for(const LfTapGeom& g, const LfWgradArgs& a, int pro);
 int lf_tapwgrad_launch(const LfTapGeom& g, const LfWgradArgs& a, int pro, hipStream_t st);
 
-bool lf_tapbwd16_ok(const LfTapGeom& gf, const LfTapGeom& gd, const LfWgradArgs& w, const LfTapArgs& a, int pro, int epi);
-int lf_tapbwd16_launch(const LfTapGeom& gf, const LfTapGeom& gd, const LfWgradArgs& w, const LfTapArgs& a, int pro, int epi, hipStream_t st);
+struct LfBnFold {
+    const float* t;
+    const float* asc;
+    const float* ash;
+    const float* gamma;
+    const float* c1;
+    const float* c2;
+};
+bool lf_tapbwd16_ok(const LfTapGeom& gf, const LfTapGeom& gd, const LfWgradArgs& w, const LfTapArgs& a, int pro, int epi,
+                    const LfBnFold* bn = nullptr);
+int lf_tapbwd16_launch(const LfTapGeom& gf, const LfTapGeom& gd, const LfWgradArgs& w, const LfTapArgs& a, int pro, int epi, hipStream_t st,
+                       const LfBnFold* bn = nullptr);
 void lf_tapbwd16_set(int mode);
-bool lf_tapbwd16_routed(int pro, int epi);
+bool lf_tapbwd16_routed(int pro, int epi, bool bnfold = false);
+long lf_tapbwd16_bn_launches();
+bool lf_tapbwd16_reduce_gz();
 
 bool lf_tapwgrad_ro_ok(const LfTapGeom& g, int s16);
 int lf_tapwgrad_ro_rows_bound(const LfTapGeom& g);
diff --git a/lanedetection_end2end_amd/csrc/lf_debug.h b/lanedetection_end2end_amd/csrc/lf_debug.h
--- a/lanedetection_end2end_amd/csrc/lf_debug.h
+++ b/lanedetection_end2end_amd/csrc/lf_debug.h
@@ -20,10 +20,15 @@
                              const float* sh, float* t, float* y, float* stats, int N, int H, int W, int C, int dilation, float* scratch,
                              void* stream);
 void lf_debug_set_bwd16_fused(int mode);
+long lf_debug_bn_bwd_launches(int which);
 long lf_debug_conv1d_bwd_pair_scratch_floats(int N, int H, int W, int C);
 int lf_debug_conv1d_bwd_pair(const float* x, const float* gy, const float* w, int epi, const float* add_src, const float* aux,
                              const float* msc, const float* msh, const float* pro_sc, const float* pro_sh, float* gx, float* gw, float* gb,
                              float* stats, int N, int H, int W, int C, int axis, int dilation, float* scratch, void* stream);
+int lf_debug_conv1d_bwd_pair_bn(const float* x, const float* gy, const float* w, int epi, const float* add_src, const float* aux,
+                                const float* msc, const float* msh, const float* pro_sc, const float* pro_sh, float* gx, float* gw, float* gb,
+                                float* stats, int N, int H, int W, int C, int axis, int dilation, float* scratch, void* stream, const float* t,
+                                const float* asc, const float* ash, const float* gamma, const float* c1, const float* c2, const float* dm);
 int lf_debug_conv1d_wgrad_pro(const float* x, const float* gy, const float* sc, const float* sh, float* gw, float* gb, int N, int H, int W,
                               int C, int axis, int dilation, float* scratch, void* stream);
 int lf_debug_conv1d_bwd_data_epi3(const float* gy, const float* w, const float* mask_src, const float* add_src, const float* aux,
@@ -55,6 +60,8 @@
                     long pix_per_image, int s16, void* stream);
 int lf_debug_bn_bwd_reduce(const float* g, const float* y, const float* t, const float* asc, const float* ash, const float* dm, float* rows,
                            int ld, long npix, int C, long pix_per_image, int s16, void* stream);
+int lf_debug_bn_bwd_reduce_gz(const float* g, const float* y, const float* t, const float* asc, const float* ash, const float* dm,
+                              float* rows, int ld, long npix, int C, long pix_per_image, int s16, void* stream, float* g_z);
 int lf_debug_bn_bwd_apply(const float* g, const float* y, const float* t, const float* asc, const float* ash, const float* gamma,
                           const float* c1, const float* c2, const float* dm, float* g_t, float* g_z, long npix, int C, long pix_per_image,
                           int s16, void* stream);
diff --git a/lanedetection_end2end_amd/csrc/lf_eltwise.h b/lanedetection_end2end_amd/csrc/lf_eltwise.h
--- a/lanedetection_end2end_amd/csrc/lf_eltwise.h
+++ b/lanedetection_end2end_amd/csrc/lf_eltwise.h
@@ -19,12 +19,14 @@
               long npix, int C, long pix_per_image, int s16, hipStream_t st);
 int lf_bn_bwd_reduce_rows(long npix);
 int lf_bn_bwd_reduce(const float* g, const float* y, const float* t, const float* asc, const float* ash, const float* dm,
-                     float* rows, int ld, long npix, int C, long pix_per_image, int s16, hipStream_t st);
+                     float* rows, int ld, long npix, int C, long pix_per_image, int s16, hipStream_t st, float* g_z = nullptr);
 int lf_bn_bwd_finalize(const LfStatPart* parts, int nparts, int C, double count, const float* asc, const float* ash, float* c1,
                        float* c2, float* ggamma, float* gbeta, int training, hipStream_t st);
 int lf_bn_bwd_apply(const float* g, const float* y, const float* t, const float* asc, const float* ash, const float* gamma,
                     const float* c1, const float* c2, const float* dm, float* g_t, float* g_z, long npix, int C,
                     long pix_per_image, int s16, hipStream_t st);
+
+long lf_bn_bwd_launches(int which);
 
 int lf_pool_rows(long npix_out);
 int lf_pool_concat_fwd(const float* x, int N, int H, int W, int Cin, float* cat, int cat_pix, int choff, float* rows, int ld,
diff --git a/lanedetection_end2end_amd/csrc/lf_eltwise.hip b/lanedetection_end2end_amd/csrc/lf_eltwise.hip
--- a/lanedetection_end2end_amd/csrc/lf_eltwise.hip
+++ b/lanedetection_end2end_amd/csrc/lf_eltwise.hip
@@ -155,7 +155,8 @@
 __global__ __launch_bounds__(256) void bn_bwd_reduce_kernel(const T* __restrict__ g, const T* __restrict__ y,
                                                            const T* __restrict__ t, const float* __restrict__ asc,
                                                            const float* __restrict__ ash, const float* __restrict__ dm,
-                                                           float* __restrict__ rows, int ld, long npix, int U, long pix_per_image) {
+                                                           float* __restrict__ rows, int ld, long npix, int U, long pix_per_image,
+                                                           T* __restrict__ g_z) {
     constexpr int V = 4 * NQ;
     const int C = U * V, ppi = 256 / U;
     const int cq = threadIdx.x % U, pr = threadIdx.x / U;
@@ -179,6 +180,7 @@
 #pragma unroll
             for (int q = 0; q < NQ; ++q) gm[q] = pos4(gm[q], yv[q]);
         }
+        if (g_z) lf_stq<T, NQ>(g_z + off, gm);
         if (dm) {
             const float* d = dm + (p / pix_per_image) * C + c;
 #pragma unroll
@@ -486,17 +488,22 @@
 
 int lf_bn_bwd_reduce_rows(long npix) { return grid_for(npix * 4, 1024); }
 
+static std::atomic<long> g_bn_bwd_launches[2];
+long lf_bn_bwd_launches(int which) { return which == 0 || which == 1 ? g_bn_bwd_launches[which].load() : -1; }
+
 int lf_bn_bwd_reduce(const float* g, const float* y, const float* t, const float* asc, const float* ash, const float* dm,
-                     float* rows, int ld, long npix, int C, long pix_per_image, int s16, hipStream_t st) {
+                     float* rows, int ld, long npix, int C, long pix_per_image, int s16, hipStream_t st, float* g_z) {
     LF_REQUIRE(quad_ok(C), "bn_bwd_reduce: unsupported channel count %d", C);
+    LF_REQUIRE(!g_z || (g_z != g && g_z != y && g_z != t), "bn_bwd_reduce: g_z aliases an input");
     const dim3 grid(lf_bn_bwd_reduce_rows(npix));
     const bool oct = oct_ok(s16, C);
     const int V = oct ? 8 : 4;
     LF_BY_STORAGE3(s16, oct,
-        hipLaunchKernelGGL((bn_bwd_reduce_kernel<lf_bf16, 2>), grid, dim3(256), 0, st, as<lf_bf16>(g), as<lf_bf16>(y), as<lf_bf16>(t), asc, ash, dm, rows, ld, npix, C / V, pix_per_image),
-        hipLaunchKernelGGL((bn_bwd_reduce_kernel<lf_bf16, 1>), grid, dim3(256), 0, st, as<lf_bf16>(g), as<lf_bf16>(y), as<lf_bf16>(t), asc, ash, dm, rows, ld, npix, C / V, pix_per_image),
-        hipLaunchKernelGGL((bn_bwd_reduce_kernel<float, 1>), grid, dim3(256), 0, st, g, y, t, asc, ash, dm, rows, ld, npix, C / V, pix_per_image));
+        hipLaunchKernelGGL((bn_bwd_reduce_kernel<lf_bf16, 2>), grid, dim3(256), 0, st, as<lf_bf16>(g), as<lf_bf16>(y), as<lf_bf16>(t), asc, ash, dm, rows, ld, npix, C / V, pix_per_image, as<lf_bf16>(g_z)),
+        hipLaunchKernelGGL((bn_bwd_reduce_kernel<lf_bf16, 1>), grid, dim3(256), 0, st, as<lf_bf16>(g), as<lf_bf16>(y), as<lf_bf16>(t), asc, ash, dm, rows, ld, npix, C / V, pix_per_image, as<lf_bf16>(g_z)),
+        hipLaunchKernelGGL((bn_bwd_reduce_kernel<float, 1>), grid, dim3(256), 0, st, g, y, t, asc, ash, dm, rows, ld, npix, C / V, pix_per_image, g_z));
     LF_CHECK_LAUNCH("bn_bwd_reduce");
+    ++g_bn_bwd_launches[0];
     return 0;
 }
 
@@ -529,6 +536,7 @@
         hipLaunchKernelGGL((bn_bwd_apply_kernel<lf_bf16, 1>), grid, dim3(256), 0, st, as<lf_bf16>(g), as<lf_bf16>(y), as<lf_bf16>(t), asc, ash, gamma, c1, c2, dm, as<lf_bf16>(g_t), as<lf_bf16>(g_z), units, C / V, pix_per_image),
         hipLaunchKernelGGL((bn_bwd_apply_kernel<float, 1>), grid, dim3(256), 0, st, g, y, t, asc, ash, gamma, c1, c2, dm, g_t, g_z, units, C / V, pix_per_image));
     LF_CHECK_LAUNCH("bn_bwd_apply");
+    ++g_bn_bwd_launches[1];
     return 0;
 }
 
diff --git a/lanedetection_end2end_amd/csrc/lf_erfnet.hip b/lanedetection_end2end_amd/csrc/lf_erfnet.hip
--- a/lanedetection_end2end_amd/csrc/lf_erfnet.hip
+++ b/lanedetection_end2end_amd/csrc/lf_erfnet.hip
@@ -551,7 +551,7 @@
 
 typedef LfBiasChain BiasChain;
 
-struct PairDg { const GemmOp* op; float* dst; int epi; LfTapArgs extra; };
+struct PairDg { const GemmOp* op; float* dst; int epi; LfTapArgs extra; const LfBnFold* bn = nullptr; };
 
 int run_wgrad(const Ctx& c, const GemmOp& op, const ConvRef& cv, const float* x, const float* g, const float* pro_sc,
               const float* pro_sh, int bias_accumulate, bool batch_off = false, BiasChain* chain = nullptr, const PairDg* pair = nullptr) {
@@ -575,16 +575,17 @@
         if (a.bias_partial) a.bias_partial = rows;
     }
     const int wpro = pro_sc ? LF_PRO_BNRELU : LF_PRO_NONE;
-    if (pair && !chain && !c.s16 && (P->precision == 0 || P->precision == 3) && lf_tapbwd16_routed(wpro, pair->epi)) {
+    if (pair && !chain && !c.s16 && (P->precision == 0 || P->precision == 3) && lf_tapbwd16_routed(wpro, pair->epi, pair->bn != nullptr)) {
         LfTapArgs d = pair->extra;
         d.src = g; d.dst = pair->dst; d.bias = nullptr; d.wp = c.packed(pair->op->pack); d.s16 = 0;
-        if (lf_tapbwd16_ok(op.geom, pair->op->geom, a, d, wpro, pair->epi)) {
+        if (lf_tapbwd16_ok(op.geom, pair->op->geom, a, d, wpro, pair->epi, pair->bn)) {
             c.last_rows = lf_tapgemm_stat_rows_for(pair->op->geom, d);
             ProfScope ps(c, 0, pair->op->geom, pair->epi, ws, 2);
-            LF_TRY(lf_tapbwd16_launch(op.geom, pair->op->geom, a, d, wpro, pair->epi, ws));
+            LF_TRY(lf_tapbwd16_launch(op.geom, pair->op->geom, a, d, wpro, pair->epi, ws, pair->bn));
             c.pair_fused = true;
         }
     }
+    if (pair && pair->bn && !c.pair_fused) return 0;
     if (!c.pair_fused) {
         ProfScope ps(c, 1, op.geom, 0, ws);
         LF_TRY(lf_tapwgrad_launch(op.geom, a, wpro, ws));
@@ -605,8 +606,24 @@
     return 0;
 }
 
+struct BnOp { const float* t; const BNRef* bn; const float* dm; float* dt; float* dst_apply; long npix; int C; long ppi; };
 int run_bwd_pair(const Ctx& c, const ConvRef& cv, const float* x, const float* g, const float* pro_sc, const float* pro_sh, float* dst,
-                 int epi, const LfTapArgs& extra) {
+                 int epi, const LfTapArgs& extra, const BnOp* bnop = nullptr, float** landed = nullptr) {
+    if (landed) *landed = dst;
+    if (bnop) {
+        const BNRef& b = *bnop->bn;
+        if (!bnop->dm) {
+            const LfBnFold f = {bnop->t, c.at(b.asc), c.at(b.ash), c.params[b.p_g], c.at(b.c1), c.at(b.c2)};
+            const PairDg pair = {&cv.dg[0], dst, epi, extra, &f};
+            LF_TRY(run_wgrad(c, cv.fwd, cv, x, g, pro_sc, pro_sh, 0, false, nullptr, &pair));
+            if (c.pair_fused) return 0;
+        }
+        LF_TRY(lf_bn_bwd_apply(g, nullptr, bnop->t, c.at(b.asc), c.at(b.ash), c.params[b.p_g], c.at(b.c1), c.at(b.c2), bnop->dm, bnop->dt,
+                               nullptr, bnop->npix, bnop->C, bnop->ppi, c.s16, c.st));
+        g = bnop->dt;
+        dst = bnop->dst_apply;
+        if (landed) *landed = dst;
+    }
     const PairDg pair = {&cv.dg[0], dst, epi, extra};
     LF_TRY(run_wgrad(c, cv.fwd, cv, x, g, pro_sc, pro_sh, 0, false, nullptr, &pair));
     if (c.pair_fused) return 0;
@@ -691,21 +708,29 @@
         const float* prelast = c.at(L.kind == K_NB ? L.b[3] : L.b[0]);
         const float* dm = (L.kind == K_NB && L.drop_idx >= 0 && c.dropmask) ? c.dropmask + P->drop_off[L.drop_idx] : nullptr;
         const float* gz;
+        const float* gbn = nullptr;
         if (!prepped) {
+            const bool feeds_fold = L.kind == K_NB && L.Cout == 16 && L.Wout % 64 == 0 && !dm && !c.s16 && (P->precision == 0 || P->precision == 3) &&
+                                    c.grads[L.cv[3].p_w] && lf_tapbwd16_routed(LF_PRO_NONE, LF_EPI_MASK, true);
+            const bool store_gz = feeds_fold || lf_tapbwd16_reduce_gz();
             const int rrows = lf_bn_bwd_reduce_rows(npo);
-            LF_TRY(lf_bn_bwd_reduce(in, ylast, prelast, c.at(blast.asc), c.at(blast.ash), dm, stat0, lf_stat_ld(rrows), npo, L.Cout, ppi, c.s16, c.st));
+            LF_TRY(lf_bn_bwd_reduce(in, ylast, prelast, c.at(blast.asc), c.at(blast.ash), dm, stat0, lf_stat_ld(rrows), npo, L.Cout, ppi, c.s16, c.st,
+                                    store_gz ? Y : nullptr));
             LfStatPart rp = {stat0, rrows, L.Cout, 0, lf_stat_ld(rrows)};
             LF_TRY(bn_bwd_finalize(c, blast, &rp, 1, (double)npo));
-            LF_TRY(lf_bn_bwd_apply(in, ylast, prelast, c.at(blast.asc), c.at(blast.ash), c.params[blast.p_g], c.at(blast.c1),
-                                   c.at(blast.c2), dm, X, L.kind == K_NB ? Y : nullptr, npo, L.Cout, ppi, c.s16, c.st));
+            if (store_gz) gbn = Y;
+            else
+                LF_TRY(lf_bn_bwd_apply(in, ylast, prelast, c.at(blast.asc), c.at(blast.ash), c.params[blast.p_g], c.at(blast.c1),
+                                       c.at(blast.c2), dm, X, L.kind == K_NB ? Y : nullptr, npo, L.Cout, ppi, c.s16, c.st));
             gz = Y;
         } else {
             LfStatPart rp = {stat0, prep_rows, L.Cout, 0, prep_ld};
             LF_TRY(bn_bwd_finalize(c, blast, &rp, 1, (double)npo));
-            LF_TRY(lf_bn_bwd_apply(in, nullptr, prelast, c.at(blast.asc), c.at(blast.ash), c.params[blast.p_g], c.at(blast.c1),
+            gz = gbn = in;
+        }
+        if (gbn && L.kind != K_NB)
+            LF_TRY(lf_bn_bwd_apply(gbn, nullptr, prelast, c.at(blast.asc), c.at(blast.ash), c.params[blast.p_g], c.at(blast.c1),
                                    c.at(blast.c2), dm, X, nullptr, npo, L.Cout, ppi, c.s16, c.st));
-            gz = in;
-        }
         float* F = prepped ? Y : in;
         float* out = nullptr;
         prepped = false;
@@ -715,24 +740,26 @@
             const BNRef& b1 = L.bn[0];
             LfTapArgs a = lf_no_args();
             a.mask_src = t3;
-            LF_TRY(run_bwd_pair(c, L.cv[3], t3, X, nullptr, nullptr, F, LF_EPI_MASK, a));
+            const BnOp bo_last = {prelast, &blast, dm, X, F, npo, L.Cout, ppi};
+            LF_TRY(run_bwd_pair(c, L.cv[3], t3, gbn ? gbn : X, nullptr, nullptr, F, LF_EPI_MASK, a, gbn ? &bo_last : nullptr));
             a = lf_no_args();
             a.aux = t2; a.msc = c.at(b1.sc); a.msh = c.at(b1.sh); a.asc = c.at(b1.asc); a.ash = c.at(b1.ash);
             a.stats = stat0; a.stats_ld = lf_stat_ld(lf_tapgemm_stat_rows(L.cv[2].dg[0].geom));
             LF_TRY(run_bwd_pair(c, L.cv[2], t2, F, c.at(b1.sc), c.at(b1.sh), X, LF_EPI_MASKBN | LF_EPI_STATS_XHAT, a));
             LfStatPart sp = {stat0, c.last_rows, L.Cout, 0, a.stats_ld};
             LF_TRY(bn_bwd_finalize(c, b1, &sp, 1, (double)npo));
-            LF_TRY(lf_bn_bwd_apply(X, nullptr, t2, c.at(b1.asc), c.at(b1.ash), c.params[b1.p_g], c.at(b1.c1), c.at(b1.c2),
-                                   nullptr, F , nullptr, npo, L.Cout, ppi, c.s16, c.st));
             a = lf_no_args();
             a.mask_src = t1;
-            LF_TRY(run_bwd_pair(c, L.cv[1], t1, F, nullptr, nullptr, X, LF_EPI_MASK, a));
+            const BnOp bo_1 = {t2, &b1, nullptr, F , X, npo, L.Cout, ppi};
+            float* gt1 = nullptr;
+            LF_TRY(run_bwd_pair(c, L.cv[1], t1, X, nullptr, nullptr, F, LF_EPI_MASK, a, &bo_1, &gt1));
+            float* const other = gt1 == F ? X : F;
             a = lf_no_args();
             a.add_src = gz;
             int epi = LF_EPI_ADD;
             add_prep(a, epi, L.cv[0].dg[0].geom);
-            LF_TRY(run_bwd_pair(c, L.cv[0], x, X, nullptr, nullptr, F, epi, a));
-            out = F;
+            LF_TRY(run_bwd_pair(c, L.cv[0], x, gt1, nullptr, nullptr, other, epi, a));
+            out = other;
             if (can_prep) { prepped = true; prep_rows = c.last_rows; prep_ld = a.stats_ld; }
         } else if (L.kind == K_UP) {
             long wsum = 0, bsum = 0;
diff --git a/lanedetection_end2end_amd/csrc/lf_ops.hip b/lanedetection_end2end_amd/csrc/lf_ops.hip
--- a/lanedetection_end2end_amd/csrc/lf_ops.hip
+++ b/lanedetection_end2end_amd/csrc/lf_ops.hip
@@ -104,6 +104,7 @@
 void lf_debug_set_wgrad_ro(int mode, int cap64, int cap128) { lf_tapwgrad_ro_set(mode, cap64, cap128); }
 void lf_debug_set_fp32_stream(int mode, int max_workgroups) { lf_tapgemm_set_fp32_stream(mode, max_workgroups); }
 void lf_debug_set_bwd16_fused(int mode) { lf_tapbwd16_set(mode); }
+long lf_debug_bn_bwd_launches(int which) { return which == 2 ? lf_tapbwd16_bn_launches() : lf_bn_bwd_launches(which); }
 void lf_debug_set_fwd_pair(int mode, int max_workgroups) { lf_tappair_set(mode, max_workgroups); }
 long lf_debug_bias_residual_launches(void) { return lf_tapgemm_bias_residual_launches(); }
 void lf_debug_set_thin(int mode, int nt) { lf_tapgemm_set_thin(mode, nt); }
@@ -495,6 +496,18 @@
     return lf_bn_bwd_reduce(g, y, t, asc, ash, dm, rows, ld, npix, C, pix_per_image, s16 != 0, (hipStream_t)stream) ? -1 : nrows;
 }
 
+int lf_debug_bn_bwd_reduce_gz(const float* g, const float* y, const float* t, const float* asc, const float* ash, const float* dm,
+                              float* rows, int ld, long npix, int C, long pix_per_image, int s16, void* stream, float* g_z) {
+    if (!g_z) return lf_debug_bn_bwd_reduce(g, y, t, asc, ash, dm, rows, ld, npix, C, pix_per_image, s16, stream);
+    if (!(g && t && asc && ash && rows)) { lf_fail("lf_debug_bn_bwd_reduce_gz: null pointer"); return -1; }
+    if (!(al16(g) && al16(y) && al16(t) && al16(dm) && al16(g_z))) { lf_fail("lf_debug_bn_bwd_reduce_gz: pointers must be 16-byte aligned"); return -1; }
+    if (!stream_ok("lf_debug_bn_bwd_reduce_gz", npix, C, pix_per_image, dm)) return -1;
+    if (!quads_ok(C)) { lf_fail("lf_debug_bn_bwd_reduce_gz: unsupported channel count %d", C); return -1; }
+    const int nrows = lf_bn_bwd_reduce_rows(npix);
+    if (ld < nrows) { lf_fail("lf_debug_bn_bwd_reduce_gz: ld %d below the %d rows of the launch", ld, nrows); return -1; }
+    return lf_bn_bwd_reduce(g, y, t, asc, ash, dm, rows, ld, npix, C, pix_per_image, s16 != 0, (hipStream_t)stream, g_z) ? -1 : nrows;
+}
+
 int lf_debug_bn_bwd_apply(const float* g, const float* y, const float* t, const float* asc, const float* ash, const float* gamma,
                           const float* c1, const float* c2, const float* dm, float* g_t, float* g_z, long npix, int C, long pix_per_image,
                           int s16, void* stream) {
@@ -586,9 +599,32 @@
     return 3L * C * C + rows * (3L * C * C + C);
 }
 
+namespace {
+int conv1d_bwd_pair(const float* x, const float* gy, const float* w, int epi, const float* add_src, const float* aux, const float* msc,
+                    const float* msh, const float* pro_sc, const float* pro_sh, float* gx, float* gw, float* gb, float* stats, int N, int H,
+                    int W, int C, int axis, int dilation, float* scratch, void* stream, const LfBnFold* bn, const float* dm);
+}
 int lf_debug_conv1d_bwd_pair(const float* x, const float* gy, const float* w, int epi, const float* add_src, const float* aux,
                              const float* msc, const float* msh, const float* pro_sc, const float* pro_sh, float* gx, float* gw, float* gb,
                              float* stats, int N, int H, int W, int C, int axis, int dilation, float* scratch, void* stream) {
+    return conv1d_bwd_pair(x, gy, w, epi, add_src, aux, msc, msh, pro_sc, pro_sh, gx, gw, gb, stats, N, H, W, C, axis, dilation, scratch, stream,
+                           nullptr, nullptr);
+}
+int lf_debug_conv1d_bwd_pair_bn(const float* x, const float* gy, const float* w, int epi, const float* add_src, const float* aux,
+                                const float* msc, const float* msh, const float* pro_sc, const float* pro_sh, float* gx, float* gw, float* gb,
+                                float* stats, int N, int H, int W, int C, int axis, int dilation, float* scratch, void* stream, const float* t,
+                                const float* asc, const float* ash, const float* gamma, const float* c1, const float* c2, const float* dm) {
+    if (!(t && asc && ash && gamma && c1 && c2)) { lf_fail("lf_debug_conv1d_bwd_pair_bn: null pointer"); return -1; }
+    const LfBnFold bn = {t, asc, ash, gamma, c1, c2};
+    return conv1d_bwd_pair(x, gy, w, epi, add_src, aux, msc, msh, pro_sc, pro_sh, gx, gw, gb, stats, N, H, W, C, axis, dilation, scratch, stream,
+                           &bn, dm);
+}
+}
+
+namespace {
+int conv1d_bwd_pair(const float* x, const float* gy, const float* w, int epi, const float* add_src, const float* aux, const float* msc,
+                    const float* msh, const float* pro_sc, const float* pro_sh, float* gx, float* gw, float* gb, float* stats, int N, int H,
+                    int W, int C, int axis, int dilation, float* scratch, void* stream, const LfBnFold* bn, const float* dm) {
     if (!(x && gy && w && gx && gw && gb && scratch)) { lf_fail("lf_debug_conv1d_bwd_pair: null pointer"); return -1; }
     if (N < 1 || H < 1 || W < 1 || C < 1 || dilation < 1 || (axis != 0 && axis != 1)) { lf_fail("lf_debug_conv1d_bwd_pair: bad arguments"); return -1; }
     if (g_ops_bf16 == 2) { lf_fail("lf_debug_conv1d_bwd_pair: fp32 tensors only"); return -1; }
@@ -606,18 +642,22 @@
     a.mask_src = (epi & LF_EPI_MASK) ? x : nullptr;
     a.aux = (epi & LF_EPI_MASKBN) ? x : aux;
     a.stats_ld = lf_tapgemm_stat_rows(g);
+    a.dm = dm;
     const int pro = pro_sc ? LF_PRO_BNRELU : LF_PRO_NONE;
-    if (!lf_tapbwd16_ok(g, g, wa, a, pro, epi)) {
+    if (!lf_tapbwd16_ok(g, g, wa, a, pro, epi, bn)) {
         lf_fail("lf_debug_conv1d_bwd_pair: the fused kernel does not take this launch (epi %d, prologue %d, %d x %d x %d x %d)", epi, pro, N, H, W, C);
         return -1;
     }
     hipLaunchKernelGGL(pack_one_kernel, dim3(64), dim3(256), 0, st, w, scratch, C, C, 3, 3L * C, 3L, conv1d_taps(1));
-    if (lf_tapbwd16_launch(g, g, wa, a, pro, epi, st)) return -1;
+    if (lf_tapbwd16_launch(g, g, wa, a, pro, epi, st, bn)) return -1;
     const int idx[3] = {0, 1, 2};
     const int nsplit = lf_tapwgrad_splits_for(g, wa, pro);
     if (lf_wgrad_reduce_launch(wa.partial, nsplit, 3, C, C, gw, 3L, 3L * C, idx, wa.bias_partial, nsplit, gb, 0, st)) return -1;
     return (epi & LF_EPI_STATS_XHAT) ? lf_tapgemm_stat_rows_for(g, a) : 0;
 }
+}
+
+extern "C" {
 
 int lf_debug_conv1d_wgrad_pro(const float* x, const float* gy, const float* sc, const float* sh, float* gw, float* gb, int N, int H, int W,
                               int C, int axis, int dilation, float* scratch, void* stream) {
```
